# Acly/dlimgedit

Hardware: AMD Instinct MI355X
Metric: images/sec encode+mask @1024x1024 (higher is better)
Workload: dtype f16; 1 GPU; SAM vit_b encoder + 1 point prompt, 1 image(s)/GPU/step, 1024x1024 RGBA, inputs and masks resident in HBM; timed through the extension entry point dlimg_amd_encode_and_mask (device pointers in and out) -- the drop-in table itself, host buffers in and out, is `abi_path`; weights=seeded synthetic, lanes_per_gpu=4, lanes_fed_by_the_step_queue=3, requests_coalesced_per_pass=4, passes_queued_per_lane=2

## Files before the change

__graft_entry__.py:

```python
from __future__ import annotations

import sys
import tempfile
from pathlib import Path

ROOT = Path(__file__).resolve().parent
if str(ROOT) not in sys.path:
    sys.path.insert(0, str(ROOT))


def build() -> None:
    from dlimgedit_amd.build import build as build_lib
    lib = build_lib(verbose=True)
    import dlimgedit_amd
    from dlimgedit_amd import api
    handle = api.library()
    assert handle.dlimg_init() is not None
    for name in api.ext.EXPORTS:
        getattr(handle, name)
    hooks = api.hooks_library()
    assert hooks.dlimg_init() is not None
    for name in api.ext.HOOK_EXPORTS:
        getattr(hooks, name)
    from oracle import sam_oracle
    from oracle.build_ref import build_abi_consumer
    ref = build_abi_consumer()
    print(f"ok: {lib}; oracle/_ref: {ref if ref else 'reference tree absent, nothing prebuilt'}")


def smoke() -> None:
    import numpy as np
    from dlimgedit_amd import api, weights as W
    from dlimgedit_amd.sam_config import get_config
    from oracle import sam_oracle as O

    assert api.Environment.is_supported(api.Backend.gpu), "no gfx950 device: the HIP path cannot run"
    cfg = get_config("vit_test")
    with tempfile.TemporaryDirectory() as d:
        params = W.write_synthetic_model_dir(d, cfg, seed=7)
        env = api.Environment(api.Options(api.Backend.gpu, d))
        rng = np.random.default_rng(0)
        yy, xx = np.mgrid[0:1024, 0:1024].astype(np.float32)
        img = np.zeros((1024, 1024, 4), np.uint8)
        for c in range(3):
            img[:, :, c] = np.clip(128 + 60 * np.sin(xx * 0.01 * (c + 1)) * np.cos(yy * 0.013) +
                                   rng.uniform(-8, 8, (1024, 1024)), 0, 255).astype(np.uint8)
        img[:, :, 3] = 255
        seg = api.Segmentation.process(api.ImageView(img, api.Channels.rgba), env)
        mask = seg.compute_mask(api.Point(512, 512))
        ora = O.OracleSegmentation(params, cfg).process(img, O.CH_RGBA)
        want = ora.compute_mask(point=(512, 512))
        inter = np.logical_and(mask > 0, want > 0).sum()
        union = np.logical_or(mask > 0, want > 0).sum()
        iou = 1.0 if union == 0 else inter / union
        emb_err = float(np.abs(api.ext.get_embedding(seg) - ora.embedding).max())
        print(f"smoke: embedding max-abs err {emb_err:.4f}, mask IoU vs oracle {iou:.4f}")
        assert emb_err < 0.05 and iou >= 0.98
        seg.close()
        env.close()


if __name__ == "__main__":
    build()
    if "--smoke" in sys.argv:
        smoke()
```

dlimgedit_amd/api.py:

```python
from __future__ import annotations

import ctypes as C
import os
import enum
from dataclasses import dataclass, field
from pathlib import Path
from typing import Optional, Sequence, Tuple

import numpy as np

LIB_PATH = Path(__file__).resolve().parent / "lib" / "libdlimgedit.so"
HOOKS_LIB_PATH = LIB_PATH.with_name("libdlimgedit_test.so")
if os.environ.get("DLIMGEDIT_TUNING_LIB") == "1":
    LIB_PATH = HOOKS_LIB_PATH = LIB_PATH.with_name("libdlimgedit_tuning.so")
elif os.environ.get("DLIMGEDIT_TUNING_LIB"):
    LIB_PATH = HOOKS_LIB_PATH = LIB_PATH.with_name(os.environ["DLIMGEDIT_TUNING_LIB"])


class Error(RuntimeError):
    """dlimg::Exception."""


class Backend(enum.IntEnum):
    cpu = 0
    gpu = 1


class Channels(enum.IntEnum):
    mask = 1
    rgb = 3
    rgba = 4
    bgra = 5
    argb = 6


def count(channels: Channels) -> int:
    return 4 if int(channels) > 4 else int(channels)


@dataclass(frozen=True)
class Extent:
    width: int = 0
    height: int = 0


@dataclass(frozen=True)
class Point:
    x: int = 0
    y: int = 0


@dataclass(frozen=True)
class Region:
    top_left: Point = Point()
    bottom_right: Point = Point()

    @staticmethod
    def from_origin(origin: Point, extent: Extent) -> "Region":
        return Region(origin, Point(origin.x + extent.width, origin.y + extent.height))



class _ImageView(C.Structure):
    _fields_ = [("width", C.c_int), ("height", C.c_int), ("channels", C.c_int), ("stride", C.c_int),
                ("pixels", C.c_void_p)]


class _Options(C.Structure):
    _fields_ = [("backend", C.c_int), ("model_directory", C.c_char_p)]


_u8pp = C.POINTER(C.c_void_p)

_API_FIELDS = [
    ("is_backend_supported", C.CFUNCTYPE(C.c_int, C.c_int)),
    ("create_environment", C.CFUNCTYPE(C.c_int, C.POINTER(C.c_void_p), C.POINTER(_Options))),
    ("destroy_environment", C.CFUNCTYPE(None, C.c_void_p)),
    ("process_image_for_segmentation", C.CFUNCTYPE(C.c_int, C.POINTER(C.c_void_p), C.POINTER(_ImageView), C.c_void_p)),
    ("get_segmentation_mask", C.CFUNCTYPE(C.c_int, C.c_void_p, C.POINTER(C.c_int), C.POINTER(C.c_int), _u8pp,
                                          C.POINTER(C.c_float))),
    ("get_segmentation_extent", C.CFUNCTYPE(None, C.c_void_p, C.POINTER(C.c_int))),
    ("destroy_segmentation", C.CFUNCTYPE(None, C.c_void_p)),
    ("segment_objects", C.CFUNCTYPE(C.c_int, C.POINTER(_ImageView), C.c_void_p, C.c_void_p)),
    ("load_image", C.CFUNCTYPE(C.c_int, C.c_char_p, C.POINTER(C.c_int), C.POINTER(C.c_int), _u8pp)),
    ("save_image", C.CFUNCTYPE(C.c_int, C.POINTER(_ImageView), C.c_char_p)),
    ("create_image", C.CFUNCTYPE(C.c_void_p, C.c_int, C.c_int, C.c_int)),
    ("destroy_image", C.CFUNCTYPE(None, C.c_void_p)),
    ("last_error", C.CFUNCTYPE(C.c_char_p)),
    ("process_images_for_segmentation", C.CFUNCTYPE(C.c_int, C.POINTER(C.c_void_p), C.POINTER(_ImageView), C.c_int,
                                                    C.c_void_p)),
    ("get_segmentation_masks", C.CFUNCTYPE(C.c_int, C.POINTER(C.c_void_p), C.c_int, C.POINTER(C.c_int),
                                           C.POINTER(C.c_int), _u8pp)),
]

REFERENCE_SLOTS = 13


class _Api(C.Structure):
    _fields_ = _API_FIELDS


_lib = None
_api = None


def library() -> C.CDLL:
    global _lib
    if _lib is None:
        if not LIB_PATH.exists():
            raise Error(f"{LIB_PATH} not found: build it with `python -m dlimgedit_amd.build` "
                        "(the HIP library is the product; there is no Python fallback)")
        _lib = C.CDLL(str(LIB_PATH))
        _lib.dlimg_init.restype = C.POINTER(_Api)
        _lib.dlimg_init.argtypes = []
    return _lib


_hooks_lib = None


def hooks_library() -> C.CDLL:
    global _hooks_lib
    if _hooks_lib is None:
        if HOOKS_LIB_PATH == LIB_PATH:
            _hooks_lib = library()
        else:
            if not HOOKS_LIB_PATH.exists():
                raise Error(f"{HOOKS_LIB_PATH} not found: build it with `python -m dlimgedit_amd.build`")
            _hooks_lib = C.CDLL(str(HOOKS_LIB_PATH))
            _hooks_lib.dlimg_init.restype = C.POINTER(_Api)
            _hooks_lib.dlimg_init.argtypes = []
    return _hooks_lib


def _check_hook(result: int) -> None:
    if result != 0:
        msg = hooks_library().dlimg_init().contents.last_error()
        raise Error(msg.decode("utf-8", "replace") if msg else "Unknown error")


def api() -> _Api:
    global _api
    if _api is None:
        _api = library().dlimg_init().contents
    return _api


def _check(result: int) -> None:
    if result != 0:
        msg = api().last_error()
        raise Error(msg.decode("utf-8", "replace") if msg else "Unknown error")



class ImageView:

    def __init__(self, pixels: np.ndarray, channels: Channels = Channels.rgba, stride: Optional[int] = None):
        if pixels.dtype != np.uint8:
            raise TypeError("pixels must be uint8")
        if pixels.ndim == 2:
            pixels = pixels[:, :, None]
        h, w, c = pixels.shape
        if c != count(channels):
            raise ValueError(f"array has {c} channels, {channels!r} needs {count(channels)}")
        if stride is None:
            pixels = np.ascontiguousarray(pixels)
            stride = w * c
        self._array = pixels
        self.extent = Extent(w, h)
        self.channels = Channels(channels)
        self.stride = int(stride)

    def _c(self) -> _ImageView:
        return _ImageView(self.extent.width, self.extent.height, int(self.channels), self.stride,
                          self._array.ctypes.data)


class Image:

    def __init__(self, extent: Extent, channels: Channels = Channels.rgba):
        self._extent, self._channels = extent, Channels(channels)
        self._ptr = api().create_image(extent.width, extent.height, count(channels))
        if not self._ptr:
            raise Error("create_image failed")

    def extent(self) -> Extent:
        return self._extent

    def channels(self) -> Channels:
        return self._channels

    def size(self) -> int:
        return self._extent.width * self._extent.height * count(self._channels)

    def pixels(self) -> np.ndarray:
        buf = (C.c_uint8 * self.size()).from_address(self._ptr)
        buf._owner = self
        return np.frombuffer(buf, dtype=np.uint8).reshape(self._extent.height, self._extent.width, count(self._channels))

    def view(self) -> ImageView:
        return ImageView(self.pixels(), self._channels)

    @staticmethod
    def load(filepath) -> "Image":
        ext = (C.c_int * 2)()
        ch = C.c_int()
        px = C.c_void_p()
        _check(api().load_image(str(filepath).encode(), ext, C.byref(ch), C.byref(px)))
        img = Image.__new__(Image)
        img._extent, img._channels, img._ptr = Extent(ext[0], ext[1]), Channels(ch.value), px.value
        return img

    @staticmethod
    def save(img: ImageView, filepath) -> None:
        v = img._c()
        _check(api().save_image(C.byref(v), str(filepath).encode()))

    def __del__(self):
        ptr, self._ptr = getattr(self, "_ptr", None), None
        if ptr and _api is not None:
            _api.destroy_image(ptr)


def _mask_image(extent: Extent) -> np.ndarray:
    return Image(extent, Channels.mask).pixels().reshape(extent.height, extent.width)



@dataclass
class Options:
    backend: Backend = Backend.cpu
    model_directory: str = "models"


class Environment:

    @staticmethod
    def is_supported(backend: Backend) -> bool:
        return api().is_backend_supported(int(backend)) != 0

    def __init__(self, options: Options = Options()):
        self._handle = C.c_void_p()
        self._dir = str(options.model_directory).encode()
        opts = _Options(int(options.backend), self._dir)
        _check(api().create_environment(C.byref(self._handle), C.byref(opts)))

    def handle(self) -> C.c_void_p:
        return self._handle

    def close(self) -> None:
        h, self._handle = self._handle, C.c_void_p()
        if h and _api is not None:
            _api.destroy_environment(h)

    def __del__(self):
        self.close()

    def __enter__(self):
        return self

    def __exit__(self, *exc):
        self.close()


@dataclass
class Mask:
    image: np.ndarray
    accuracy: float = 0.0


MAX_CLICKS = 8
TOKEN_ROWS_MAX = 112
EMPTY_REGION = (0, 0, -1, -1)
REFINE_MARK = 4


@dataclass
class ClickEntries:
    heads: list
    points: list
    regions: list
    prompt_heads: list
    token_rows: list
    stage_clicks: list = field(default_factory=list)

    def _staged(self, j) -> bool:
        return j < len(self.stage_clicks) and len(self.stage_clicks[j]) > 1

    @property
    def launches(self) -> list:
        out = []
        plain = [j for j in range(len(self.token_rows)) if not self._staged(j)]
        for t in dict.fromkeys(self.token_rows[j] for j in plain):
            group = [j for j in plain if self.token_rows[j] == t]
            cut = TOKEN_ROWS_MAX // t
            out += [(t, group[k:k + cut]) for k in range(0, len(group), cut)]
        for j in range(len(self.token_rows)):
            if self._staged(j):
                box_rows = self.token_rows[j] - self.stage_clicks[j][-1]
                out += [(box_rows + k, [j]) for k in self.stage_clicks[j]]
        return out


def pack_clicks(clicks, labels, region=None):
    clicks, labels = _checked_clicks(clicks, labels)
    pts = [(c.x, c.y) for c in clicks]
    labs = list(labels)
    if region is not None:
        pts += [(region.top_left.x, region.top_left.y), (region.bottom_right.x, region.bottom_right.y)]
        labs += [2, 3]
    else:
        pts.append((0, 0))
        labs.append(-1)
    return pts, labs


def _checked_clicks(clicks, labels):
    clicks = list(clicks)
    labels = [1] * len(clicks) if labels is None else [int(v) for v in labels]
    if not clicks:
        raise Error("a prompt needs at least one click")
    if len(clicks) > MAX_CLICKS:
        raise Error(f"a prompt takes at most {MAX_CLICKS} clicks, not {len(clicks)}")
    if len(labels) != len(clicks):
        raise Error(f"{len(clicks)} clicks but {len(labels)} labels")
    if any(v not in (0, 1) for v in labels):
        raise Error("the label of a click is 1 (foreground) or 0 (background)")
    if labels[0] != 1:
        raise Error("the first click of a prompt is a foreground click: it travels in the head entry, which has no label")
    return clicks, labels


def _checked_marks(n_clicks: int, refine_after) -> list:
    if refine_after is None:
        return []
    if isinstance(refine_after, str):
        if refine_after != "each":
            raise Error('refine_after is a sequence of click counts or "each"')
        return list(range(1, n_clicks))
    ks = [int(k) for k in refine_after]
    if any(k < 1 or k >= n_clicks for k in ks):
        raise Error(f"refine_after: a mark goes behind the first k clicks, 1 <= k < {n_clicks} (every stage adds at least one click)")
    if any(b <= a for a, b in zip(ks, ks[1:])):
        raise Error("refine_after: the click counts are strictly increasing (no mark directly after another)")
    return ks


def click_entries(clicks, labels=None, regions=None, refine_after=None) -> ClickEntries:
    n = len(clicks)
    labels = [None] * n if labels is None else list(labels)
    regions = [None] * n if regions is None else list(regions)
    refine_after = [refine_after] * n if refine_after is None or isinstance(refine_after, str) else list(refine_after)
    if len(labels) != n or len(regions) != n or len(refine_after) != n:
        raise Error("one list of labels, one region (or None) and one refine_after (or None) per prompt")
    out = ClickEntries([], [], [], [], [])
    for j in range(n):
        cs, ls = _checked_clicks(clicks[j], labels[j])
        marks = _checked_marks(len(cs), refine_after[j])
        r = regions[j]
        out.prompt_heads.append(len(out.heads))
        out.token_rows.append(5 + len(cs) + (2 if r is not None else 1))
        out.stage_clicks.append(marks + [len(cs)])
        for k, (c, lab) in enumerate(zip(cs, ls)):
            if k in marks:
                out.heads.append(None)
                out.points.append((0, 0))
                out.regions.append((REFINE_MARK, 0, 0, 0))
            out.heads.append(j if k == 0 else None)
            out.points.append((c.x, c.y))
            if k:
                out.regions.append((lab, 0, 0, 0))
            else:
                out.regions.append(EMPTY_REGION if r is None else (r.top_left.x, r.top_left.y, r.bottom_right.x, r.bottom_right.y))
    return out


def _entry_calls(entries: ClickEntries) -> list:
    n = len(entries.heads)
    if any(h is None for h in entries.heads):
        return [(list(range(n)), True)]
    plain = [i for i in range(n) if entries.regions[i] == EMPTY_REGION]
    boxed = [i for i in range(n) if entries.regions[i] != EMPTY_REGION]
    return [(sel, given) for sel, given in ((plain, False), (boxed, True)) if sel]


def _entry_arrays(segs, entries: ClickEntries, sel, regions_given: bool):
    n = len(sel)
    handles = (C.c_void_p * n)(*[None if entries.heads[i] is None else segs[entries.heads[i]]._handle for i in sel])
    p = (C.c_int * (2 * n))(*[v for i in sel for v in entries.points[i]])
    r = (C.c_int * (4 * n))(*[v for i in sel for v in entries.regions[i]]) if regions_given else None
    return n, handles, p, r


class Segmentation:

    def __init__(self, handle: C.c_void_p, env: Environment):
        self._handle, self._env = handle, env

    @staticmethod
    def process(img: ImageView, env: Environment) -> "Segmentation":
        seg = Segmentation(C.c_void_p(), env)
        v = img._c()
        _check(api().process_image_for_segmentation(C.byref(seg._handle), C.byref(v), env.handle()))
        return seg

    @staticmethod
    def process_batch(imgs: Sequence[ImageView], env: Environment) -> list:
        n = len(imgs)
        handles = (C.c_void_p * n)()
        views = (_ImageView * n)(*[i._c() for i in imgs])
        segs = []
        try:
            _check(api().process_images_for_segmentation(handles, views, n, env.handle()))
        finally:
            segs = [Segmentation(C.c_void_p(h), env) for h in handles if h]
        return segs

    def extent(self) -> Extent:
        out = (C.c_int * 2)()
        api().get_segmentation_extent(self._handle, out)
        return Extent(out[0], out[1])

    def _query(self, point, region, n_masks, out=None):
        e = self.extent()
        masks = [_mask_image(e) for _ in range(n_masks)] if out is None else list(out)
        assert len(masks) == n_masks and all(m.shape == (e.height, e.width) and m.dtype == np.uint8 and
                                              m.flags.c_contiguous for m in masks)
        ptrs = (C.c_void_p * 3)(*([m.ctypes.data for m in masks] + [None] * (3 - n_masks)))
        acc = (C.c_float * 3)(0.0, 0.0, 0.0)
        p = (C.c_int * 2)(point.x, point.y) if point is not None else None
        r = (C.c_int * 4)(region.top_left.x, region.top_left.y, region.bottom_right.x, region.bottom_right.y) \
            if region is not None else None
        _check(api().get_segmentation_mask(self._handle, p, r, ptrs, acc))
        return masks, list(acc)

# ... 170 lines not shown
               "dlimg_amd_bench_gemm_stamps")

    @staticmethod
    def _ptr(a: Optional[np.ndarray]):
        return None if a is None else a.ctypes.data

    @classmethod
    def device_count(cls) -> int:
        return cls._l().dlimg_amd_device_count()

    @classmethod
    def model_geometry(cls, env: Environment) -> Tuple[int, int, int, int]:
        out = (C.c_int * 4)()
        _check(cls._l().dlimg_amd_model_geometry(env.handle(), out))
        return tuple(out)

    @classmethod
    def get_embedding(cls, seg: Segmentation) -> np.ndarray:
        out = np.empty((4096, 256), dtype=np.float32)
        _check(cls._l().dlimg_amd_get_embedding(seg._handle, out.ctypes.data))
        return out

    @classmethod
    def get_logits(cls, seg: Segmentation, point: Optional[Point] = None, region: Optional[Region] = None):
        logits = np.empty((4, 256, 256), dtype=np.float32)
        iou = np.empty(4, dtype=np.float32)
        p = (C.c_int * 2)(point.x, point.y) if point is not None else None
        r = (C.c_int * 4)(region.top_left.x, region.top_left.y, region.bottom_right.x, region.bottom_right.y) \
            if region is not None else None
        _check(cls._l().dlimg_amd_get_logits(seg._handle, p, r, logits.ctypes.data, iou.ctypes.data))
        return logits, iou

    @classmethod
    def decoder_state(cls, seg: Segmentation, point: Point):
        buf = C.create_string_buffer(1024)
        _check(cls._l().dlimg_amd_decoder_state(seg._handle, (C.c_int * 2)(point.x, point.y), None, 0, buf, 1024))
        parts = [(n, int(c)) for n, c in (item.split(":") for item in buf.value.decode().strip(",").split(","))]
        out = np.empty(sum(c for _, c in parts), dtype=np.float32)
        _check(cls._l().dlimg_amd_decoder_state(seg._handle, (C.c_int * 2)(point.x, point.y), out.ctypes.data, out.size, None, 0))
        res, off = {}, 0
        for n, c in parts:
            res[n] = out[off:off + c]
            off += c
        return res

    @classmethod
    def mask_pieces(cls, mask_bytes, extra_bytes: int = 0):
        n = len(mask_bytes)
        sizes = (C.c_longlong * max(1, n))(*mask_bytes)
        ends = (C.c_longlong * 8)()
        cap = 8 * (n + 1)
        copies = (C.c_longlong * (5 * cap))()
        pieces = C.c_int(0)
        got = cls._h().dlimg_amd_test_mask_pieces(n, sizes, extra_bytes, ends, 8, copies, cap, C.byref(pieces))
        if got < 0:
            _check_hook(1)
        return [ends[i] for i in range(pieces.value)], [tuple(copies[5 * k + j] for j in range(5)) for k in range(got)]

    @classmethod
    def plan_steps(cls, passes_in_flight, images_in_flight, cursor: int, pending: int, width: int, depth: int, all_: bool):
        lanes = len(passes_in_flight)
        p = (C.c_int * lanes)(*passes_in_flight)
        i = (C.c_int * lanes)(*images_in_flight)
        cur = C.c_int(cursor)
        cap = pending + lanes + 1
        out_lane, out_images = (C.c_int * cap)(), (C.c_int * cap)()
        n = cls._h().dlimg_amd_test_plan_steps(lanes, p, i, C.byref(cur), pending, width, depth, int(all_), out_lane, out_images, cap)
        if n < 0:
            _check_hook(1)
        return [(out_lane[k], out_images[k]) for k in range(n)], list(p), list(i), cur.value

    @classmethod
    def parse_cpu_list(cls, text: str) -> list:
        out = (C.c_int * 4096)()
        n = cls._h().dlimg_amd_test_parse_cpu_list(text.encode(), out, 4096)
        if n < 0:
            _check_hook(1)
        return list(out[:n])

    @classmethod
    def device_alloc(cls, env, nbytes: int) -> int:
        out = C.c_void_p()
        _check(cls._l().dlimg_amd_device_alloc(env.handle(), nbytes, C.byref(out)))
        return out.value

    @classmethod
    def device_free(cls, env, ptr: int) -> None:
        _check(cls._l().dlimg_amd_device_free(env.handle(), ptr))

    @classmethod
    def copy_to_device(cls, env, dst: int, src: np.ndarray) -> None:
        src = np.ascontiguousarray(src)
        _check(cls._l().dlimg_amd_copy_to_device(env.handle(), dst, src.ctypes.data, src.nbytes))

    @classmethod
    def copy_to_host(cls, env, dst: np.ndarray, src: int) -> None:
        _check(cls._l().dlimg_amd_copy_to_host(env.handle(), dst.ctypes.data, src, dst.nbytes))

    @staticmethod
    def device_views(ptrs, width, height, channels=Channels.rgba, stride=None):
        n = len(ptrs)

        def per_view(value):
            return list(value) if isinstance(value, (list, tuple)) else [value] * n

        ws, hs, cs, ss = per_view(width), per_view(height), per_view(channels), per_view(stride)
        return (_ImageView * n)(*[_ImageView(ws[i], hs[i], int(cs[i]), ws[i] * count(cs[i]) if ss[i] is None else ss[i], ptrs[i])
                                  for i in range(n)])

    @classmethod
    def encode_and_mask(cls, env, views, points, mask_ptrs) -> None:
        n = len(views)
        p = (C.c_int * (2 * n))(*[v for q in points for v in (q.x, q.y)])
        m = (C.c_void_p * n)(*mask_ptrs)
        _check(cls._l().dlimg_amd_encode_and_mask(env.handle(), views, n, p, m))

    @classmethod
    def encode_only(cls, env, views) -> None:
        _check(cls._l().dlimg_amd_encode_only(env.handle(), views, len(views)))

    @classmethod
    def synchronize(cls, env) -> None:
        _check(cls._l().dlimg_amd_synchronize(env.handle()))

    @classmethod
    def lane_count(cls, env) -> int:
        return cls._l().dlimg_amd_lane_count(env.handle())

    @classmethod
    def queue_config(cls, env) -> dict:
        out = (C.c_int * 6)()
        _check(cls._l().dlimg_amd_queue_config(env.handle(), out))
        return {"coalesce": out[0], "step_depth": out[1], "lanes": out[2], "lanes_in_use": out[3],
                "one_image_passes": out[4], "one_image_passes_alone": out[5]}

    @classmethod
    def image_memory_is_pinned(cls, array: np.ndarray) -> bool:
        out = C.c_int(0)
        _check(cls._l().dlimg_amd_image_memory(array.ctypes.data, array.nbytes, C.byref(out)))
        return bool(out.value)

    @classmethod
    def replica_count(cls, env) -> int:
        return cls._l().dlimg_amd_replica_count(env.handle())

    @classmethod
    def segmentation_device(cls, seg) -> Tuple[int, int]:
        r, d = C.c_int(), C.c_int()
        _check(cls._l().dlimg_amd_segmentation_device(seg._handle, C.byref(r), C.byref(d)))
        return r.value, d.value

    @classmethod
    def compute_mask_batch_device(cls, segs, dev_out: int, points=None, regions=None, root_device: int = 0, clicks=None,
                                  labels=None, refine_after=None) -> list:
        if refine_after is not None and clicks is None:
            raise Error("compute_mask_batch_device: refine_after goes with `clicks`")
        if clicks is not None:
            if points is not None:
                raise Error("compute_mask_batch_device: `points` or `clicks`, not both")
            if len(clicks) != len(segs):
                raise Error("compute_mask_batch_device: one list of clicks per segmentation")
            entries = click_entries(clicks, labels, regions, refine_after)
            calls = _entry_calls(entries)
            if len(calls) > 1:
                calls = [([i], entries.regions[i] != EMPTY_REGION) for i in range(len(entries.heads))]
            result, base = [], 0
            for sel, given in calls:
                n, handles, p, r = _entry_arrays(segs, entries, sel, given)
                offsets = (C.c_size_t * n)()
                _check(cls._l().dlimg_amd_get_segmentation_masks_device(handles, n, p, r, root_device, dev_out + base, offsets))
                result += [base + offsets[k] for k, i in enumerate(sel) if entries.heads[i] is not None]
                e = segs[entries.heads[sel[0]]].extent()
                base += e.width * e.height if len(calls) > 1 else 0
            return result
        n = len(segs)
        handles = (C.c_void_p * n)(*[s._handle for s in segs])
        p = r = None
        if points is not None:
            p = (C.c_int * (2 * n))(*[v for q in points for v in (q.x, q.y)])
        if regions is not None:
            r = (C.c_int * (4 * n))(*[v for q in regions for v in (q.top_left.x, q.top_left.y, q.bottom_right.x,
                                                                  q.bottom_right.y)])
        offsets = (C.c_size_t * n)()
        _check(cls._l().dlimg_amd_get_segmentation_masks_device(handles, n, p, r, root_device, dev_out, offsets))
        return list(offsets)

    @classmethod
    def set_profiling(cls, env, on: bool) -> None:
        _check(cls._l().dlimg_amd_set_profiling(env.handle(), int(on)))

    @classmethod
    def take_stage_stats(cls, env) -> dict:
        n = len(STAGES)
        ms, work, launches = (C.c_double * n)(), (C.c_double * n)(), (C.c_long * n)()
        _check(cls._l().dlimg_amd_take_stage_stats(env.handle(), ms, work, launches))
        return {s: {"ms": ms[i], "work": work[i], "launches": launches[i]} for i, s in enumerate(STAGES)}

    @classmethod
    def test_preprocess(cls, pixels: np.ndarray, channels: Channels, stride: Optional[int] = None) -> np.ndarray:
        h, w = pixels.shape[:2]
        if stride is None:
            pixels = np.ascontiguousarray(pixels)
            stride = w * count(channels)
        out = np.empty((4096, 768), dtype=np.float16)
        _check_hook(cls._h().dlimg_amd_test_preprocess(pixels.ctypes.data, w, h, stride, int(channels), out.ctypes.data))
        return out

    @classmethod
    def test_postprocess(cls, planes: np.ndarray, out_w: int, out_h: int, iou: Optional[np.ndarray] = None) -> np.ndarray:
        planes = np.ascontiguousarray(planes, dtype=np.float32).reshape(-1, 256, 256)
        out = np.empty((out_h, out_w), dtype=np.uint8)
        iou = None if iou is None else np.ascontiguousarray(iou, dtype=np.float32)
        _check_hook(cls._h().dlimg_amd_test_postprocess(planes.ctypes.data, planes.shape[0], cls._ptr(iou), out_w, out_h,
                                                   out.ctypes.data))
        return out

    @classmethod
    def test_postprocess_batch(cls, planes: np.ndarray, out_w: int, out_h: int) -> np.ndarray:
        planes = np.ascontiguousarray(planes, dtype=np.float32).reshape(-1, 256, 256)
        out = np.empty((planes.shape[0], out_h, out_w), dtype=np.uint8)
        _check_hook(cls._h().dlimg_amd_test_postprocess_batch(planes.ctypes.data, planes.shape[0], out_w, out_h, out.ctypes.data))
        return out

    @classmethod
    def force_gemm_tile(cls, tile: int = -1, consumer_tile: int = -1) -> None:
        _check_hook(cls._h().dlimg_amd_test_force_gemm_tile(int(tile)))
        _check_hook(cls._h().dlimg_amd_test_force_gemm_consumer_tile(int(consumer_tile)))

    @classmethod
    def test_gemm(cls, A: np.ndarray, W: np.ndarray, bias=None, resid=None, act: int = 0, want_f16: bool = False):
        A = np.ascontiguousarray(A, dtype=np.float16)
        W = np.ascontiguousarray(W, dtype=np.float16)
        M, K = A.shape
        N = W.shape[0]
        bias = None if bias is None else np.ascontiguousarray(bias, dtype=np.float32)
        resid = None if resid is None else np.ascontiguousarray(resid, dtype=np.float32)
        out32 = np.empty((M, N), dtype=np.float32)
        out16 = np.empty((M, N), dtype=np.float16) if want_f16 else None
        _check_hook(cls._h().dlimg_amd_test_gemm(M, N, K, A.ctypes.data, W.ctypes.data, cls._ptr(bias), cls._ptr(resid),
                                            0 if resid is None else resid.shape[0], act, out32.ctypes.data,
                                            cls._ptr(out16)))
        return (out32, out16) if want_f16 else out32

    @classmethod
    def test_gemm_ln(cls, A1, W1, bias1, resid, W2, gamma, beta, bias2, eps: float, act: int = 0):
        A1 = np.ascontiguousarray(A1, dtype=np.float16)
        W1 = np.ascontiguousarray(W1, dtype=np.float16)
        M, K1 = A1.shape
        D = W1.shape[0]
        W2 = np.asarray(W2, dtype=np.float32)
        N = W2.shape[0]
        wg = np.ascontiguousarray((W2 * np.asarray(gamma, np.float32)[None, :]).astype(np.float16))
        colsum = np.ascontiguousarray(wg.astype(np.float64).sum(axis=1).astype(np.float32))
        b2 = np.ascontiguousarray((np.asarray(bias2, np.float64) + W2.astype(np.float64) @ np.asarray(beta, np.float64))
                                  .astype(np.float32))
        bias1 = None if bias1 is None else np.ascontiguousarray(bias1, dtype=np.float32)
        resid = None if resid is None else np.ascontiguousarray(resid, dtype=np.float32)
        x = np.empty((M, D), dtype=np.float32)
        xh = np.empty((M, D), dtype=np.float16)
        y = np.empty((M, N), dtype=np.float32)
        _check_hook(cls._h().dlimg_amd_test_gemm_ln(M, D, K1, N, A1.ctypes.data, W1.ctypes.data, cls._ptr(bias1),
                                               cls._ptr(resid), wg.ctypes.data, colsum.ctypes.data, b2.ctypes.data,
                                               eps, act, x.ctypes.data, xh.ctypes.data, y.ctypes.data))
        return x, xh, y

    @classmethod
    def test_lane_worker(cls, tasks: int, sleep_us: int = 0):
        order = np.full(tasks + 1, -1, dtype=np.int32)
        ran = cls._h().dlimg_amd_test_lane_worker(tasks, sleep_us, order.ctypes.data)
        if ran < 0:
            _check_hook(1)
        return order[:ran].tolist()

    @classmethod
    def test_gemm_stream(cls, A, W, bias, resid_hi, resid_lo, pair: bool):
        A = np.ascontiguousarray(A, dtype=np.float16)
        W = np.ascontiguousarray(W, dtype=np.float16)
        M, K = A.shape
        D = W.shape[0]
        bias = None if bias is None else np.ascontiguousarray(bias, dtype=np.float32)
        resid_hi = None if resid_hi is None else np.ascontiguousarray(resid_hi, dtype=np.float16)
        resid_lo = None if resid_lo is None else np.ascontiguousarray(resid_lo, dtype=np.float16)
        x = None if pair else np.empty((M, D), dtype=np.float32)
        hi = np.empty((M, D), dtype=np.float16)
        lo = np.empty((M, D), dtype=np.float16) if pair else None
        stats = np.empty((M * 48,), dtype=np.float32)
        _check_hook(cls._h().dlimg_amd_test_gemm_stream(M, D, K, A.ctypes.data, W.ctypes.data, cls._ptr(bias), cls._ptr(resid_hi),
                                                   cls._ptr(resid_lo), int(pair), cls._ptr(x), hi.ctypes.data,
                                                   cls._ptr(lo), stats.ctypes.data))
        return x, hi, lo, stats

    @classmethod
    def test_layernorm(cls, x, w, b, eps: float, act: int = 0):
        x = np.ascontiguousarray(x, dtype=np.float32)
        w = np.ascontiguousarray(w, dtype=np.float32)
        b = np.ascontiguousarray(b, dtype=np.float32)
        rows, dim = x.shape
        o32 = np.empty_like(x)
        o16 = np.empty(x.shape, dtype=np.float16)
        _check_hook(cls._h().dlimg_amd_test_layernorm(x.ctypes.data, w.ctypes.data, b.ctypes.data, eps, rows, dim, act,
                                                 o32.ctypes.data, o16.ctypes.data))
        return o32, o16

    @classmethod
    def test_attention(cls, is_global: bool, qkv, qkv_bias, rel_h, rel_w, batch: int, heads: int, hd: int):
        qkv = np.ascontiguousarray(qkv, dtype=np.float16)
        rel_h = np.ascontiguousarray(rel_h, dtype=np.float32)
        rel_w = np.ascontiguousarray(rel_w, dtype=np.float32)
        qkv_bias = None if qkv_bias is None else np.ascontiguousarray(qkv_bias, dtype=np.float32)
        out = np.empty((batch * 4096, heads * hd), dtype=np.float16)
        _check_hook(cls._h().dlimg_amd_test_attention(int(is_global), qkv.ctypes.data, cls._ptr(qkv_bias), rel_h.ctypes.data,
                                                 rel_w.ctypes.data, batch, heads, hd, out.ctypes.data))
        return out

    @classmethod
    def test_decode(cls, env: Environment, embeddings: np.ndarray, emb_index, coords, labels):
        emb = np.ascontiguousarray(embeddings, dtype=np.float32).reshape(-1, 4096, 256)
        idx = np.ascontiguousarray(emb_index, dtype=np.int32).reshape(-1)
        count = idx.size
        c = np.ascontiguousarray(coords, dtype=np.float32).reshape(count, 4)
        l = np.ascontiguousarray(labels, dtype=np.float32).reshape(count, 2)
        logits = np.empty((count, 4, 256, 256), dtype=np.float32)
        iou = np.empty((count, 4), dtype=np.float32)
        _check_hook(cls._h().dlimg_amd_test_decode(env.handle(), emb.shape[0], emb.ctypes.data, count, idx.ctypes.data,
                                                   c.ctypes.data, l.ctypes.data, logits.ctypes.data, iou.ctypes.data))
        return logits, iou

    @classmethod
    def test_decode_prompts(cls, env: Environment, embeddings: np.ndarray, emb_index, coords, labels, mask_planes=None,
                            mask_iou=None, want_state: bool = False):
        emb = np.ascontiguousarray(embeddings, dtype=np.float32).reshape(-1, 4096, 256)
        idx = np.ascontiguousarray(emb_index, dtype=np.int32).reshape(-1)
        count = idx.size
        l = np.ascontiguousarray(labels, dtype=np.float32).reshape(count, -1)
        points = l.shape[1]
        c = np.ascontiguousarray(coords, dtype=np.float32).reshape(count, points, 2)
        planes = None if mask_planes is None else np.ascontiguousarray(mask_planes, dtype=np.float32).reshape(count, 4, 256, 256)
        iou4 = None if mask_iou is None else np.ascontiguousarray(mask_iou, dtype=np.float32).reshape(count, 4)
        logits = np.empty((count, 4, 256, 256), dtype=np.float32)
        iou = np.empty((count, 4), dtype=np.float32)
        state = np.empty(1 << 18, dtype=np.float32) if want_state else None
        layout = C.create_string_buffer(1024)
        _check_hook(cls._h().dlimg_amd_test_decode_prompts(
            env.handle(), emb.shape[0], emb.ctypes.data, count, idx.ctypes.data, points, c.ctypes.data, l.ctypes.data,
            cls._ptr(planes), cls._ptr(iou4), logits.ctypes.data, iou.ctypes.data, cls._ptr(state),
            0 if state is None else state.size, layout, 1024))
        if not want_state:
            return logits, iou
        res, off = {}, 0
        for n, cnt in ((n, int(cnt)) for n, cnt in (item.split(":") for item in layout.value.decode().strip(",").split(","))):
            res[n] = state[off:off + cnt].copy()
            off += cnt
        return logits, iou, res

    @classmethod
    def test_resize(cls, pixels: np.ndarray, channels: Channels, out_w: int, out_h: int) -> np.ndarray:
        pixels = np.ascontiguousarray(pixels)
        h, w = pixels.shape[:2]
        c = count(channels)
        out = np.empty((out_h, out_w, c), dtype=np.uint8)
        _check_hook(cls._h().dlimg_amd_test_resize(pixels.ctypes.data, w, h, w * c, int(channels), out_w, out_h,
                                              out.ctypes.data))
        return out

    @classmethod
    def birefnet_prepare_image(cls, image: np.ndarray, channels: "Channels", mean, std) -> np.ndarray:
        image = np.ascontiguousarray(image, dtype=np.uint8)
        h, w = image.shape[:2]
        mean = np.ascontiguousarray(mean, dtype=np.float32)
        std = np.ascontiguousarray(std, dtype=np.float32)
        out = np.empty((1, 3, h, w), dtype=np.float32)
        _check(cls._l().dlimg_amd_birefnet_prepare_image(image.ctypes.data, w, h, image.strides[0], int(channels),
                                                         mean.ctypes.data, std.ctypes.data, out.ctypes.data))
        return out

    @classmethod
    def birefnet_process_mask(cls, logits: np.ndarray) -> np.ndarray:
        logits = np.ascontiguousarray(logits, dtype=np.float32)
        h, w = logits.shape
        out = np.empty((h, w), dtype=np.uint8)
        _check(cls._l().dlimg_amd_birefnet_process_mask(logits.ctypes.data, w, h, out.ctypes.data))
        return out

    @classmethod
    def resize_mask(cls, mask: np.ndarray, out_w: int, out_h: int) -> np.ndarray:
        mask = np.ascontiguousarray(mask, dtype=np.uint8)
        h, w = mask.shape
        out = np.empty((out_h, out_w), dtype=np.uint8)
        _check(cls._l().dlimg_amd_resize_mask(mask.ctypes.data, w, h, mask.strides[0], out_w, out_h, out.ctypes.data))
        return out

    @classmethod
    def bench_prepost(cls, batch: int = 16, iters: int = 50, working_set_mb: int = 768) -> Tuple[float, float]:
        pre, post = C.c_double(), C.c_double()
        _check_hook(cls._h().dlimg_amd_bench_prepost(batch, iters, working_set_mb, C.byref(pre), C.byref(post)))
        return pre.value, post.value

    @classmethod
    def bench_attention(cls, is_global: bool, heads: int = 12, hd: int = 64, batch: int = 1, iters: int = 50) -> float:
        ms = C.c_double()
        _check_hook(cls._h().dlimg_amd_bench_attention(int(is_global), batch, heads, hd, iters, C.byref(ms)))
        return ms.value

    @classmethod
    def bench_gemm(cls, M: int, N: int, K: int, act: int = 0, iters: int = 20, flavour: int = 0, tile: int = -1,
                   shared: bool = False, streams: int = 1) -> float:
        ms = C.c_double()
        _check_hook(cls._h().dlimg_amd_bench_gemm_streams(M, N, K, act, flavour, tile, int(shared), streams, iters,
                                                     C.byref(ms)))
        return ms.value

    @classmethod
    def bench_gemm_stamps(cls, M: int, N: int, K: int, act: int = 0, iters: int = 20, flavour: int = 0, tile: int = 9,
                          streams: int = 1, groups: int = 4096):
        ms = C.c_double()
        st = np.zeros((groups, 4), np.uint64)
        _check_hook(cls._h().dlimg_amd_bench_gemm_stamps(M, N, K, act, flavour, tile, 0, streams, iters, C.byref(ms),
                                                    st.ctypes.data, groups))
        return ms.value, st
```

dlimgedit_amd/build.py:

```python
from __future__ import annotations

import os
import shutil
import subprocess
import sys
from concurrent.futures import ThreadPoolExecutor
from pathlib import Path

PKG = Path(__file__).resolve().parent
ROOT = PKG.parent
CSRC = PKG / "csrc"
OBJ = CSRC / "_obj"
OBJ_TUNING = CSRC / "_obj_tuning"
LIB = PKG / "lib" / "libdlimgedit.so"
LIB_TEST = PKG / "lib" / "libdlimgedit_test.so"
LIB_TUNING = PKG / "lib" / "libdlimgedit_tuning.so"
ARCH = "gfx950"
SONAME = "libdlimgedit.so.1"
EXPORTS_MAP = CSRC / "exports.map"
EXPORTS_TEST_MAP = CSRC / "exports_test.map"
HOOK_SOURCES = ["test_hooks.cpp"]

SOURCES = [
    "kernels/gemm.hip",
    "kernels/elementwise.hip",
    "kernels/attention_window.hip",
    "kernels/attention_global.hip",
    "kernels/decoder.hip",
    "kernels/decoder_image.hip",
    "kernels/decoder_hq.hip",
    "kernels/postprocess.hip",
    "kernels/resize.hip",
    "kernels/objects.hip",
    "resize_tables.cpp",
    "gemm_plan.cpp",
    "image_io.cpp",
    "image_memory.cpp",
    "jpeg_decode.cpp",
    "weights.cpp",
    "lane_board.cpp",
    "stage_clock.cpp",
    "mask_transport.cpp",
    "sam_weights.cpp",
    "sam_model.cpp",
    "environment.cpp",
    "segmentation.cpp",
    "dlimgedit.cpp",
    "ext_api.cpp",
]


EXTRA_FLAGS = {
    "kernels/postprocess.hip": ["-ffp-contract=off"],
    "kernels/resize.hip": ["-ffp-contract=off"],
    "kernels/objects.hip": ["-ffp-contract=off"],
    "resize_tables.cpp": ["-ffp-contract=off"],
}


def hipcc() -> str:
    exe = shutil.which("hipcc") or "/opt/rocm/bin/hipcc"
    if not Path(exe).exists():
        raise RuntimeError("hipcc not found; the MI355X build of dlimgedit needs the ROCm toolchain")
    return exe


def _flags() -> list:
    return [f"--offload-arch={ARCH}", "-O3", "-std=c++17", "-fPIC", "-fvisibility=hidden", "-DDLIMGEDIT_EXPORTS",
            "-fno-slp-vectorize", "-Wall", "-Wno-unused-function", "-Wno-unused-result", f"-I{ROOT / 'include'}", f"-I{CSRC}"]


def _deps_mtime() -> float:
    hdrs = list(CSRC.rglob("*.hpp")) + list(CSRC.rglob("*.inc")) + list((ROOT / "include").rglob("*.h"))
    return max(p.stat().st_mtime for p in hdrs)


def _compile(src: str, force: bool, hdr_mtime: float, tuning: bool = False) -> Path:
    s = CSRC / src
    if not s.exists():
        raise FileNotFoundError(s)
    o = (OBJ_TUNING if tuning else OBJ) / (src.replace("/", "_") + ".o")
    if not force and o.exists() and o.stat().st_mtime > max(s.stat().st_mtime, hdr_mtime):
        return o
    cmd = [hipcc(), *_flags(), *(["-DDLIMG_TUNING", *os.environ.get("DLIMG_TUNING_DEFS", "").split()] if tuning else []), *EXTRA_FLAGS.get(src, []), "-x", "hip", "-c",
           str(s), "-o", str(o)]
    r = subprocess.run(cmd, capture_output=True, text=True)
    if r.returncode != 0:
        raise RuntimeError(f"hipcc failed for {src}:\n{r.stdout}\n{r.stderr}")
    if r.stderr.strip():
        sys.stderr.write(r.stderr)
    return o


LLVM_OBJDUMP = "/opt/rocm/lib/llvm/bin/llvm-objdump"
VALIDATED_HIPCC = "HIP 7.2.26015 / AMD clang 22.0.0git roc-7.2.0 (7b800a19)"


def disassemble_device_code(obj: Path) -> str:
    import tempfile
    with tempfile.TemporaryDirectory() as d:
        tmp = Path(d) / obj.name
        shutil.copy(obj, tmp)
        subprocess.run([LLVM_OBJDUMP, "--offloading", str(tmp)], capture_output=True, text=True, check=True)
        code = [f for f in Path(d).iterdir() if f.name.startswith(obj.name + ".") and "amdgcn" in f.name]
        if not code:
            raise RuntimeError(f"no gfx950 code object found in {obj}")
        return subprocess.run([LLVM_OBJDUMP, "-d", str(code[0])], capture_output=True, text=True, check=True).stdout


def check_packed_select_erratum(obj: Path) -> dict:
    import re
    counts, bad, name = {}, [], None
    for line in disassemble_device_code(obj).splitlines():
        m = re.match(r"^[0-9a-f]+ <(.+)>:$", line)
        if m:
            name = m.group(1)
            continue
        m = re.search(r"\b(v_pk_\w+)\s", line)
        if not (name and m):
            continue
        if m.group(1).endswith("_f32"):
            counts[name] = counts.get(name, 0) + 1
        sel = re.search(r"op_sel:\[([01]),([01])", line)
        if sel and sel.group(2) == "1":
            bad.append((name, line.strip().split("//")[0].strip()))
    if bad:
        listing = "\n".join(f"  {n}: {i}" for n, i in bad[:8])
        raise RuntimeError(f"{obj.name}: packed instruction with a src1 low-lane select (op_sel:[_,1,..]) -- reads 0.0 beside another "
                           f"wave's MFMA on gfx950 (DESIGN.md section 6; validated toolchain: {VALIDATED_HIPCC}):\n{listing}")
    return counts


def _link(out: Path, objs: list, exports: Path, soname: str = "") -> None:
    cmd = [hipcc(), f"--offload-arch={ARCH}", "-shared", "-fPIC", "-o", str(out), *map(str, objs),
           "-Wl,-rpath,/opt/rocm/lib", "-Wl,--no-undefined", *([f"-Wl,-soname,{soname}"] if soname else []),
           f"-Wl,--version-script={exports}", "-ldl", "-lz"]
    r = subprocess.run(cmd, capture_output=True, text=True)
    if r.returncode != 0:
        raise RuntimeError(f"link failed:\n{r.stdout}\n{r.stderr}")


def _stale(lib: Path, objs: list, force: bool) -> bool:
    return force or not lib.exists() or lib.stat().st_mtime < max(o.stat().st_mtime for o in objs)


def build(force: bool = False, verbose: bool = False, tuning: bool = False) -> Path:
    (OBJ_TUNING if tuning else OBJ).mkdir(parents=True, exist_ok=True)
    LIB.parent.mkdir(parents=True, exist_ok=True)
    hdr = _deps_mtime()
    workers = min(6, os.cpu_count() or 1)
    with ThreadPoolExecutor(workers) as ex:
        objs = list(ex.map(lambda s: _compile(s, force, hdr, tuning), SOURCES))
        hooks = list(ex.map(lambda s: _compile(s, force, hdr, tuning), HOOK_SOURCES))
    if tuning:
        if _stale(LIB_TUNING, objs + hooks, force):
            _link(LIB_TUNING, objs + hooks, EXPORTS_TEST_MAP)
        if verbose:
            print(f"built {LIB_TUNING} ({LIB_TUNING.stat().st_size / 1e6:.1f} MB)")
        return LIB_TUNING
    if _stale(LIB, objs, force) or _stale(LIB_TEST, objs + hooks, force):
        for o in objs:
            if o.name.startswith("kernels_"):
                check_packed_select_erratum(o)
        if _stale(LIB, objs, force):
            _link(LIB, objs, EXPORTS_MAP, SONAME)
        _link(LIB_TEST, objs + hooks, EXPORTS_TEST_MAP)
    link = LIB.parent / SONAME
    if not link.is_symlink() and not link.exists():
        link.symlink_to(LIB.name)
    if verbose:
        print(f"built {LIB} ({LIB.stat().st_size / 1e6:.1f} MB) and {LIB_TEST.name}")
    return LIB


if __name__ == "__main__":
    build(force="--force" in sys.argv, verbose=True, tuning="--tuning" in sys.argv)
```

dlimgedit_amd/csrc/kernels/gemm.hip:

```cpp
#include "device_common.hpp"
#include "kernels.hpp"
#include "gemm_plan.hpp"

#include <hip/hip_ext.h>

#include <mutex>
#include <cstdlib>
#include <type_traits>

namespace dlimg {
namespace {

#ifdef DLIMG_TUNING
#define DLIMG_STAMPS(a) ((a).stamps)
#else
#define DLIMG_STAMPS(a) (static_cast<unsigned long long*>(nullptr))
#endif

#if defined(DLIMG_TUNING) && defined(DLIMG_NO_RESID_READ)
constexpr bool kNoResidRead = true;
#else
constexpr bool kNoResidRead = false;
#endif
#if defined(DLIMG_TUNING) && defined(DLIMG_NO_COPY_WRITE)
constexpr bool kNoCopyWrite = true;
#else
constexpr bool kNoCopyWrite = false;
#endif

#if defined(DLIMG_TUNING) && defined(DLIMG_NO_STATS_MATH)
constexpr bool kNoStatsMath = true;
#else
constexpr bool kNoStatsMath = false;
#endif
#if defined(DLIMG_TUNING) && defined(DLIMG_NO_STREAM_STORE)
constexpr bool kNoStreamStore = true;
#else
constexpr bool kNoStreamStore = false;
#endif

#include "gemm_f16_tile.inc"

typedef float float4v __attribute__((ext_vector_type(4)));

template <int BM, int BN, int WGM, int WGN, int NSTAGE, int MINW, int ACT, int EPI>
__global__ __launch_bounds__(64 * WGM * WGN, MINW) void gemm16_f16_kernel(k::GemmArgs a) {
    constexpr int BKT = 32;
    constexpr int NW = WGM * WGN;
    constexpr int ROW_BYTES = BKT * 2;
    constexpr int WM = BM / WGM, WN = BN / WGN;
    constexpr int TM = WM / 16, TN = WN / 16;
    constexpr int A_BYTES = BM * ROW_BYTES, B_BYTES = BN * ROW_BYTES;
    constexpr int STAGE_BYTES = A_BYTES + B_BYTES;
    constexpr int LOADS = (BM + BN) * ROW_BYTES / 1024 / NW;
    constexpr int JG = ((WN / 32) % 3 == 0) ? 3 : (((WN / 32) % 2 == 0) ? 2 : 1);
    constexpr int CHUNKS = JG * 8;
    constexpr int OUT_BYTES = 32 * CHUNKS * 16;
    static_assert(NW * OUT_BYTES <= NSTAGE * STAGE_BYTES, "output staging must fit in the operand buffers");
    static_assert(TM % 2 == 0 && TN % 2 == 0, "wave tile must be a multiple of 32x32");
    extern __shared__ __attribute__((aligned(16))) char smem[];

    const int lane = lane_id();
    const int wave = wave_id();
    const int wr = wave / WGN, wc = wave % WGN;
    const int l15 = lane & 15, quad = lane >> 4;

    const int ntn = a.N / BN;
    const int tile = xcd_remap(blockIdx.x, gridDim.x);
    const int m0 = (tile / ntn) * BM;
    const int n0 = (tile % ntn) * BN;

    float4v acc[TM][TN];
#pragma unroll
    for (int i = 0; i < TM; ++i)
#pragma unroll
        for (int j = 0; j < TN; ++j) acc[i][j] = float4v{0.f, 0.f, 0.f, 0.f};

    float* rowstat = reinterpret_cast<float*>(smem + NSTAGE * STAGE_BYTES);
    float* colvec = rowstat + 2 * BM;
    const int nk = a.K / BKT;
    auto stage = [&](int kt) {
        char* dst = smem + (kt % NSTAGE) * STAGE_BYTES;
        stage_tile<BM, BKT, NW, 1>(a.A, a.lda, m0, kt * BKT, dst, wave, lane);
        stage_tile<BN, BKT, NW, 1>(a.W, a.ldw, n0, kt * BKT, dst + A_BYTES, wave, lane);
    };
    auto frag = [&](const char* lds, int row) {
        return *reinterpret_cast<const half8_t*>(lds + row * ROW_BYTES + ((quad ^ swz16(row)) << 4));
    };
    ColumnVectors<BM, BN, 64 * NW, EPI> column_vectors;
    RowStats<BM, 64 * NW, EPI> row_stats;
    column_vectors.issue(a, n0);
    row_stats.issue(a, m0);
#pragma unroll
    for (int t = 0; t < NSTAGE - 1; ++t)
        if (t < nk) stage(t);
    column_vectors.store(colvec);
    row_stats.finish(a, rowstat);

    static_assert(NSTAGE >= 3, "a tile is read one step before it is multiplied");
    constexpr int TH = TM / 2;
    half8_t fb[2][TN], fal[2][TH], fah[TH];
    auto wait_tile = [&](int newer) {
        static_assert((NSTAGE - 2) * LOADS < 64 && NSTAGE <= 8, "vmcnt is a 6-bit counter");
        if (newer >= 6) wait_dma<6 * LOADS>();
        else if (newer == 5) wait_dma<5 * LOADS>();
        else if (newer == 4) wait_dma<4 * LOADS>();
        else if (newer == 3) wait_dma<3 * LOADS>();
        else if (newer == 2) wait_dma<2 * LOADS>();
        else if (newer == 1) wait_dma<LOADS>();
        else wait_dma<0>();
    };
    auto read_next = [&](int buf, int kt) {
        const char* la = smem + (kt % NSTAGE) * STAGE_BYTES;
        const char* lb = la + A_BYTES;
#pragma unroll
        for (int j = 0; j < TN; ++j) fb[buf][j] = frag(lb, wc * WN + j * 16 + l15);
#pragma unroll
        for (int i = 0; i < TH; ++i) fal[buf][i] = frag(la, wr * WM + i * 16 + l15);
    };
    auto step = [&](int kt, auto cur_tag, auto steady_tag) {
        constexpr int cur = decltype(cur_tag)::value;
        constexpr bool STEADY = decltype(steady_tag)::value;
        const char* la = smem + (kt % NSTAGE) * STAGE_BYTES;
#pragma unroll
        for (int i = 0; i < TH; ++i) fah[i] = frag(la, wr * WM + (TH + i) * 16 + l15);
        if (STEADY) {
            wait_dma<(NSTAGE - 3) * LOADS>();
            __builtin_amdgcn_s_barrier();
            read_next(cur ^ 1, kt + 1);
            stage(kt + NSTAGE - 1);
        } else if (kt + 1 < nk) {
            wait_tile(min(NSTAGE - 3, nk - 2 - kt));
            __builtin_amdgcn_s_barrier();
            read_next(cur ^ 1, kt + 1);
            if (kt + NSTAGE - 1 < nk) stage(kt + NSTAGE - 1);
        }
        __builtin_amdgcn_sched_barrier(0);
#pragma unroll
        for (int i = 0; i < TH; ++i)
#pragma unroll
            for (int j = 0; j < TN; ++j)
                acc[i][j] = __builtin_amdgcn_mfma_f32_16x16x32_f16(fb[cur][j], fal[cur][i], acc[i][j], 0, 0, 0);
#pragma unroll
        for (int i = 0; i < TH; ++i)
#pragma unroll
            for (int j = 0; j < TN; ++j)
                acc[TH + i][j] = __builtin_amdgcn_mfma_f32_16x16x32_f16(fb[cur][j], fah[i], acc[TH + i][j], 0, 0, 0);
    };
    wait_tile(min(NSTAGE - 2, nk - 1));
    __builtin_amdgcn_s_barrier();
    read_next(0, 0);
    __builtin_amdgcn_s_waitcnt(0xC07F);
    using Even = std::integral_constant<int, 0>;
    using Odd = std::integral_constant<int, 1>;
    int kt = 0;
    for (; kt + 2 + (NSTAGE - 1) <= nk; kt += 2) {
        step(kt, Even{}, std::true_type{});
        step(kt + 1, Odd{}, std::true_type{});
    }
    for (; kt < nk; kt += 2) {
        step(kt, Even{}, std::false_type{});
        if (kt + 1 < nk) step(kt + 1, Odd{}, std::false_type{});
    }

    __syncthreads();
    char* slab = smem + wave * OUT_BYTES;
    float2_t* rowpart = reinterpret_cast<float2_t*>(smem + NW * OUT_BYTES);
    static_assert(NW * OUT_BYTES + BM * (BN / 32) * 8 <= NSTAGE * STAGE_BYTES, "tile statistics must fit behind the slabs");
    const int resid_row0 = a.resid ? m0 % a.resid_mod : 0;
    constexpr int NIT = 32 * CHUNKS / 64;
    constexpr int NJ = (WN / 32) / JG, NSLAB = (TM / 2) * NJ;
    constexpr int RV_BUFS = (MINW >= 4 && NIT > 4) ? 1 : 2;
    float4_t rv[RV_BUFS][NIT];
    if (RV_BUFS == 2) {
        const int pf_row_base = wr * WM, pf_col_base = wc * WN;
        float4_t(&pf_dst)[NIT] = rv[0];
#include "gemm_epilogue_prefetch.inc"
    }
#pragma unroll
    for (int band = 0; band < TM / 2; ++band) {
#pragma unroll
        for (int jg = 0; jg < NJ; ++jg) {
            const int sl = band * NJ + jg;
#pragma unroll
            for (int ii = 0; ii < 2; ++ii) {
                const int row = ii * 16 + l15;
#pragma unroll
                for (int jj = 0; jj < JG * 2; ++jj) {
                    const int chunk = jj * 4 + quad;
                    *reinterpret_cast<float4v*>(slab + (row * CHUNKS + (chunk ^ (row & 7))) * 16) =
                        acc[band * 2 + ii][jg * JG * 2 + jj];
                }
            }
            if (sl + RV_BUFS - 1 < NSLAB) {
                constexpr int AHEAD = RV_BUFS - 1;
                const int pf_row_base = wr * WM + ((sl + AHEAD) / NJ) * 32;
                const int pf_col_base = wc * WN + ((sl + AHEAD) % NJ) * JG * 32;
                float4_t(&pf_dst)[NIT] = rv[(sl + AHEAD) % RV_BUFS];
#include "gemm_epilogue_prefetch.inc"
            }
            const int row_local_base = wr * WM + band * 32, col_local_base = wc * WN + jg * JG * 32;
            float4_t(&rv_cur)[NIT] = rv[sl % RV_BUFS];
#include "gemm_epilogue.inc"
        }
    }
    if (EPI == EPI_STATS) {
        __syncthreads();
        write_tile_stats<BM, BN>(a, rowpart, m0, n0);
    }
}


constexpr int kPPHalfBytes = 128 * 128;
constexpr int kPPBufBytes = 4 * kPPHalfBytes;
constexpr int pp_aux_bytes(int bm) { return bm * 8 + 2 * 256 * 4 + (bm * 4 * 8 > kPPStatGroups * bm * 8 ? bm * 4 * 8 : kPPStatGroups * bm * 8); }
constexpr int kPPAuxBytes = pp_aux_bytes(256);
constexpr int kPPLds = 2 * kPPBufBytes + kPPAuxBytes;
static_assert(kPPLds <= 160 * 1024, "gemm_pp_kernel: LDS");

DLIMG_DEVICE void pp_barrier_after_reads() {
    __builtin_amdgcn_sched_barrier(0);
    asm volatile("s_waitcnt lgkmcnt(0)\n\ts_barrier" ::: "memory");
    __builtin_amdgcn_sched_barrier(0);
}
DLIMG_DEVICE void pp_barrier() {
    __builtin_amdgcn_sched_barrier(0);
    asm volatile("s_barrier" ::: "memory");
    __builtin_amdgcn_sched_barrier(0);
}

struct HiLo4 { half4_t h, l; };
DLIMG_DEVICE float4_t hilo_pack(half4_t h, half4_t l) { return __builtin_bit_cast(float4_t, HiLo4{h, l}); }
template <bool HIGH> DLIMG_DEVICE float mix_sum(uint32_t hi, uint32_t lo) {
    float r;
    if (HIGH) asm("v_fma_mix_f32 %0, %1, 1.0, %2 op_sel:[1,0,1] op_sel_hi:[1,0,1]" : "=v"(r) : "v"(hi), "v"(lo));
    else asm("v_fma_mix_f32 %0, %1, 1.0, %2 op_sel:[0,0,0] op_sel_hi:[1,0,1]" : "=v"(r) : "v"(hi), "v"(lo));
    return r;
}
template <bool HIGH> DLIMG_DEVICE float mix_rest(float v, uint32_t hi) {
    float r;
    if (HIGH) asm("v_fma_mix_f32 %0, %1, -1.0, %2 op_sel:[1,0,0] op_sel_hi:[1,0,0]" : "=v"(r) : "v"(hi), "v"(v));
    else asm("v_fma_mix_f32 %0, %1, -1.0, %2 op_sel:[0,0,0] op_sel_hi:[1,0,0]" : "=v"(r) : "v"(hi), "v"(v));
    return r;
}
DLIMG_DEVICE float4_t hilo_value(float4_t packed) {
    const uint4_t x = __builtin_bit_cast(uint4_t, packed);
    return float4_t{mix_sum<false>(x[0], x[2]), mix_sum<true>(x[0], x[2]), mix_sum<false>(x[1], x[3]), mix_sum<true>(x[1], x[3])};
}
DLIMG_DEVICE HiLo4 hilo_split(float4_t v) {
    HiLo4 out;
    out.h = __builtin_convertvector(v, half4_t);
    const uint2_t hb = __builtin_bit_cast(uint2_t, out.h);
    const float4_t rest = {mix_rest<false>(v[0], hb[0]), mix_rest<true>(v[1], hb[0]), mix_rest<false>(v[2], hb[1]), mix_rest<true>(v[3], hb[1])};
    out.l = __builtin_convertvector(rest, half4_t);
    return out;
}
DLIMG_DEVICE float4_t hilo_load(const half_t* hi, const half_t* lo, size_t offset) {
    return hilo_pack(*reinterpret_cast<const half4_t*>(hi + offset), *reinterpret_cast<const half4_t*>(lo + offset));
}

template <int BM, int EPI>
struct PPAux {
    static constexpr int BN = 256;
    static constexpr int TPR = 512 / BM;
    static constexpr int GP = BM * 8 > 1024 ? BM * 8 / 1024 : 1;
    static DLIMG_DEVICE void issue(const k::GemmArgs& a, int m0, int n0, float* colvec, float2_t* raw, int wave, int lane) {
        if (wave == 0) {
            if (a.bias) glds16(a.bias + n0 + lane * 4, colvec);
            else *reinterpret_cast<float4_t*>(colvec + lane * 4) = float4_t{0.f, 0.f, 0.f, 0.f};
        }
        if (EPI != EPI_NORM) return;
        if (wave == 1) glds16(a.ln_colsum + n0 + lane * 4, colvec + BN);
        const int pieces = a.ln_groups * GP;
        for (int p = wave; p < pieces + 2; p += 8) {
            if (p < 2) continue;
            const int g = (p - 2) / GP, h = (p - 2) % GP;
            const float2_t* src = reinterpret_cast<const float2_t*>(a.ln_stats) + (size_t)g * a.M + m0 + h * 128 + lane * 2;
            if (BM * 8 >= 1024 || lane < BM / 2) glds16(src, raw + g * BM + h * 128);
        }
    }
    static DLIMG_DEVICE void merge(const k::GemmArgs& a, const float2_t* raw, float* rowstat) {
        if (EPI != EPI_NORM) return;
        const int r = threadIdx.x / TPR, sub = threadIdx.x % TPR;
        float s1 = 0.f;
        for (int g = sub; g < a.ln_groups; g += TPR) s1 += raw[g * BM + r][0];
#pragma unroll
        for (int o = 1; o < TPR; o <<= 1) s1 += __shfl_xor(s1, o, 64);
        const float n_g = (float)(a.K / a.ln_groups), inv_n_g = 1.0f / n_g;
        const float mean = s1 / (float)a.K;
        float m2 = 0.f;
        for (int g = sub; g < a.ln_groups; g += TPR) {
            const float2_t q = raw[g * BM + r];
            const float dm = q[0] * inv_n_g - mean;
            m2 += q[1] + n_g * dm * dm;
        }
#pragma unroll
        for (int o = 1; o < TPR; o <<= 1) m2 += __shfl_xor(m2, o, 64);
        if (sub == 0) reinterpret_cast<float2_t*>(rowstat)[r] = float2_t{mean, rsqrtf(m2 / (float)a.K + a.ln_eps)};
        __syncthreads();
    }
};

template <int NI, int ACT, int EPI, bool PRE = false>
DLIMG_DEVICE void pp_epilogue(const k::GemmArgs& a, float4v (&acc)[NI][4], char* smem, const float* rowstat, const float* colvec,
                              float2_t* rowpart, int m0, int n0, int row_base, int wc, int wave, int lane,
                              float4_t (*pre)[4] = nullptr) {
    constexpr int BN = 256;
    const int l15 = lane & 15, quad = lane >> 4;
    const int col_base = wc * 64 + quad * 4;
    float4_t bias4[4], csum4[4];
#pragma unroll
    for (int j = 0; j < 4; ++j) {
        bias4[j] = *reinterpret_cast<const float4_t*>(colvec + col_base + j * 16);
        if (EPI == EPI_NORM) csum4[j] = *reinterpret_cast<const float4_t*>(colvec + BN + col_base + j * 16);
    }
    char* slab = smem + wave * 8192;
    const int resid_row0 = (a.resid || a.resid_h) ? m0 % a.resid_mod : 0;
    if (a.out_f32 == nullptr && a.out_l == nullptr) {
        const int rd_row = lane >> 3, rd_chunk = lane & 7;
#pragma unroll
        for (int i = 0; i < NI; ++i) {
            char* sl = slab + (i & 1) * 4096;
            float2_t st = float2_t{0.f, 1.f};
            if (EPI == EPI_NORM) st = reinterpret_cast<const float2_t*>(rowstat)[row_base + i * 16 + l15];
#pragma unroll
            for (int j = 0; j < 4; ++j) {
                float4_t v = float4_t{acc[i][j][0], acc[i][j][1], acc[i][j][2], acc[i][j][3]};
                if (EPI == EPI_NORM) v = (v - csum4[j] * st[0]) * st[1];
                v += bias4[j];
                if (ACT == k::ACT_GELU) v = gelu4(v);
                const half4_t h = {(half_t)v[0], (half_t)v[1], (half_t)v[2], (half_t)v[3]};
                const int piece = (j * 4 + quad) ^ ((l15 & 7) << 1);
                *reinterpret_cast<half4_t*>(sl + l15 * 128 + piece * 8) = h;
            }
            asm volatile("s_waitcnt lgkmcnt(0)" ::: "memory");
#pragma unroll
            for (int kk = 0; kk < 2; ++kk) {
                const int r = kk * 8 + rd_row;
                const float4_t piece16 = *reinterpret_cast<const float4_t*>(sl + r * 128 + ((rd_chunk ^ (r & 7)) << 4));
                const size_t m = (size_t)(m0 + row_base + i * 16 + r);
                half_t* const dst = a.out_h + m * a.ldc16 + n0 + wc * 64 + rd_chunk * 8;
                store16_result(dst, piece16);
            }
        }
    } else {
        auto fp32_bands = [&](auto resid_tag, auto h_tag) {
            constexpr int RESID = decltype(resid_tag)::value;
            constexpr int OUT = decltype(h_tag)::value;
            constexpr bool HAS_H = OUT == 1;
            const int rd_row = lane >> 3, rd_col = (lane & 7) * 8;
            float4_t rv[2][4];
            auto request_residual = [&](int i, float4_t (&dst)[4]) {
    #pragma unroll
                for (int kk = 0; kk < 2; ++kk) {
                    dst[kk * 2] = dst[kk * 2 + 1] = float4_t{0.f, 0.f, 0.f, 0.f};
                    const int r = kk * 8 + rd_row;
                    if (RESID == 1 && !kNoResidRead) {
                        const float* src = a.resid + (size_t)(resid_row0 + row_base + i * 16 + r) * a.ldr + n0 + wc * 64 + rd_col;
                        dst[kk * 2] = *reinterpret_cast<const float4_t*>(src);
                        dst[kk * 2 + 1] = *reinterpret_cast<const float4_t*>(src + 4);
                    }
                    if (RESID == 2 && !kNoResidRead) {
                        const size_t off = (size_t)(resid_row0 + row_base + i * 16 + r) * a.ldrs + n0 + wc * 64 + rd_col;
                        dst[kk * 2] = *reinterpret_cast<const float4_t*>(a.resid_h + off);
                        dst[kk * 2 + 1] = *reinterpret_cast<const float4_t*>(a.resid_l + off);
                    }
                }
            };
            if (!PRE) request_residual(0, rv[0]);
    #pragma unroll
            for (int i = 0; i < NI; ++i) {
                char* sl = slab + (i & 1) * 4096;
                float2_t st = float2_t{0.f, 1.f};
                if (EPI == EPI_NORM) st = reinterpret_cast<const float2_t*>(rowstat)[row_base + i * 16 + l15];
    #pragma unroll
                for (int j = 0; j < 4; ++j) {
                    float4_t v = float4_t{acc[i][j][0], acc[i][j][1], acc[i][j][2], acc[i][j][3]};
                    if (EPI == EPI_NORM) v = (v - csum4[j] * st[0]) * st[1];
                    v += bias4[j];
                    if (ACT == k::ACT_GELU) v = gelu4(v);
                    *reinterpret_cast<float4_t*>(sl + l15 * 256 + (((j * 4 + quad) ^ (l15 & 7)) << 4)) = v;
                }
                if (!PRE && i + 1 < NI) request_residual(i + 1, rv[(i + 1) & 1]);
                asm volatile("s_waitcnt lgkmcnt(0)" ::: "memory");
    #pragma unroll
                for (int kk = 0; kk < 2; ++kk) {
                    const int r = kk * 8 + rd_row;
                    const int slot = (lane & 7) * 2;
                    float4_t v0 = *reinterpret_cast<const float4_t*>(sl + r * 256 + ((slot ^ (r & 7)) << 4));
                    float4_t v1 = *reinterpret_cast<const float4_t*>(sl + r * 256 + (((slot + 1) ^ (r & 7)) << 4));
                    const float4_t ra = PRE ? pre[i][kk * 2] : rv[i & 1][kk * 2], rb = PRE ? pre[i][kk * 2 + 1] : rv[i & 1][kk * 2 + 1];
                    if (RESID == 1) {
                        v0 += ra;
                        v1 += rb;
                    } else if (RESID == 2) {
                        const uint4_t xa = __builtin_bit_cast(uint4_t, ra), xb = __builtin_bit_cast(uint4_t, rb);
                        v0 += hilo_value(__builtin_bit_cast(float4_t, uint4_t{xa[0], xa[1], xb[0], xb[1]}));
                        v1 += hilo_value(__builtin_bit_cast(float4_t, uint4_t{xa[2], xa[3], xb[2], xb[3]}));
                    }
                    const size_t m = (size_t)(m0 + row_base + i * 16 + r);
                    const int col = n0 + wc * 64 + rd_col;
                    if (kNoStreamStore) {
                        if (v0[0] + v1[3] == 123.456f) a.out_h[0] = (half_t)1.f;
                    } else if (OUT == 2) {
                        const HiLo4 p0 = hilo_split(v0), p1 = hilo_split(v1);
                        const uint2_t h0 = __builtin_bit_cast(uint2_t, p0.h), h1 = __builtin_bit_cast(uint2_t, p1.h);
                        const uint2_t l0 = __builtin_bit_cast(uint2_t, p0.l), l1 = __builtin_bit_cast(uint2_t, p1.l);
                        store16_result(a.out_h + m * a.ldc16 + col, uint4_t{h0[0], h0[1], h1[0], h1[1]});
                        store16_result(a.out_l + m * a.ldc16 + col, uint4_t{l0[0], l0[1], l1[0], l1[1]});
                    } else {
                        store16_result(a.out_f32 + m * a.ldc32 + col, v0);
                        store16_result(a.out_f32 + m * a.ldc32 + col + 4, v1);
                    }
                    if (HAS_H && !kNoCopyWrite) {
                        const half8_t h = {(half_t)v0[0], (half_t)v0[1], (half_t)v0[2], (half_t)v0[3],
                                           (half_t)v1[0], (half_t)v1[1], (half_t)v1[2], (half_t)v1[3]};
                        store16_result(a.out_h + m * a.ldc16 + col, h);
                    }
                    if (EPI == EPI_STATS) {
                        float s1 = ((v0[0] + v0[1]) + (v0[2] + v0[3])) + ((v1[0] + v1[1]) + (v1[2] + v1[3]));
                        if (kNoStatsMath) { if ((lane & 7) == 0) rowpart[(row_base + i * 16 + r) * 4 + wc] = float2_t{s1, s1}; continue; }
                        s1 = sum_over_8_lanes(s1);
                        const float4_t d0 = v0 - s1 * (1.0f / 64.0f), d1 = v1 - s1 * (1.0f / 64.0f);
                        float m2 = ((d0[0] * d0[0] + d0[1] * d0[1]) + (d0[2] * d0[2] + d0[3] * d0[3])) +
                                   ((d1[0] * d1[0] + d1[1] * d1[1]) + (d1[2] * d1[2] + d1[3] * d1[3]));
                        m2 = sum_over_8_lanes(m2);
                        if ((lane & 7) == 0) rowpart[(row_base + i * 16 + r) * 4 + wc] = float2_t{s1, m2};
                    }
                }
            }

        };
        using I0 = std::integral_constant<int, 0>;
        using I1 = std::integral_constant<int, 1>;
        using I2 = std::integral_constant<int, 2>;
        if (a.out_l) {
            if (a.resid_h) fp32_bands(I2{}, I2{});
            else if (a.resid) fp32_bands(I1{}, I2{});
            else fp32_bands(I0{}, I2{});
        } else if (a.resid) {
            if (a.out_h) fp32_bands(I1{}, I1{});
            else fp32_bands(I1{}, I0{});
        } else {
            if (a.out_h) fp32_bands(I0{}, I1{});
            else fp32_bands(I0{}, I0{});
        }
    }
    if (EPI == EPI_STATS) {
        __syncthreads();
        for (int r = threadIdx.x; r < NI * 32; r += 512) {
            float s1 = 0.f;
#pragma unroll
            for (int g = 0; g < 4; ++g) s1 += rowpart[r * 4 + g][0];
            const float mean = s1 * (1.0f / (float)BN);
            float m2 = 0.f;
#pragma unroll
            for (int g = 0; g < 4; ++g) {
                const float dm = rowpart[r * 4 + g][0] * (1.0f / 64.0f) - mean;
                m2 += rowpart[r * 4 + g][1] + 64.0f * dm * dm;
            }
            reinterpret_cast<float2_t*>(a.stats_out)[(size_t)(n0 / BN) * a.M + m0 + r] = float2_t{s1, m2};
        }
    }
}

template <int ACT, int EPI>
__global__ __launch_bounds__(512, 2) void gemm_pp_kernel(k::GemmArgs a) {
    constexpr int BM = 256, BN = 256;
    extern __shared__ __attribute__((aligned(16))) char smem[];
    const int lane = lane_id();
    const int wave = wave_id();
    const int wr = wave >> 2, wc = wave & 3;
    const int l15 = lane & 15, quad = lane >> 4;

    const int ntn = a.N / BN;
    const int tile = xcd_remap(blockIdx.x, gridDim.x);
    const int m0 = (tile / ntn) * BM;
    const int n0 = (tile % ntn) * BN;
    const int nk = a.K / 64;

    float* rowstat = reinterpret_cast<float*>(smem + 2 * kPPBufBytes);
    float* colvec = rowstat + 2 * BM;
    float2_t* rowpart = reinterpret_cast<float2_t*>(colvec + 2 * BN);

    float4v acc[8][4];
#pragma unroll
    for (int i = 0; i < 8; ++i)
#pragma unroll
        for (int j = 0; j < 4; ++j) acc[i][j] = float4v{0.f, 0.f, 0.f, 0.f};

    const half_t* src_a[2];
    const half_t* src_w[2];
#pragma unroll
    for (int q = 0; q < 2; ++q) {
        const int row = (wave * 2 + q) * 8 + (lane >> 3);
        const int chunk = (lane & 7) ^ ((row >> 1) & 7);
        src_a[q] = a.A + (size_t)(m0 + row) * a.lda + chunk * 8;
        src_w[q] = a.W + (size_t)(n0 + row) * a.ldw + chunk * 8;
    }
    const size_t a_half = (size_t)128 * a.lda, w_half = (size_t)128 * a.ldw;
    auto stage = [&](int t, int H) {
        char* dst = smem + (t & 1) * kPPBufBytes + H * kPPHalfBytes + wave * 2048;
#pragma unroll
        for (int q = 0; q < 2; ++q) {
            const half_t* g = (H < 2 ? src_a[q] + (H & 1) * a_half : src_w[q] + (H & 1) * w_half) + (size_t)t * 64;
            glds16(g, dst + q * 1024);
        }
    };

    const int sw = (l15 >> 1) & 7;
    const int off0 = l15 * 128 + ((quad ^ sw) << 4);
    const int off1 = l15 * 128 + (((quad ^ sw) ^ 4) << 4);
    const char* a_base = smem + wr * kPPHalfBytes;
    const char* w_base = smem + (2 + (wc >> 1)) * kPPHalfBytes + (wc & 1) * 64 * 128;
    auto frag = [&](const char* p) { return *reinterpret_cast<const half8_t*>(p); };

    const unsigned long long t_start = DLIMG_STAMPS(a) ? __builtin_amdgcn_s_memtime() : 0ull;
    const unsigned long long r_start = DLIMG_STAMPS(a) ? __builtin_amdgcn_s_memrealtime() : 0ull;
    PPAux<BM, EPI>::issue(a, m0, n0, colvec, rowpart, wave, lane);
    stage(0, 0); stage(0, 1); stage(0, 2); stage(0, 3);
    if (nk > 1) { stage(1, 2); stage(1, 3); }
    if (nk > 1) wait_dma<4>(); else wait_dma<0>();
    pp_barrier();
    if (wr == 1) pp_barrier();

    half8_t fa[4][2], fw[2][2][2];
    auto mfma_quadrant = [&](int mh, int nh) {
        __builtin_amdgcn_s_setprio(1);
#pragma unroll
        for (int ks = 0; ks < 2; ++ks)
#pragma unroll
            for (int i = 0; i < 4; ++i)
#pragma unroll
                for (int j = 0; j < 2; ++j)
                    acc[mh * 4 + i][nh * 2 + j] =
                        __builtin_amdgcn_mfma_f32_16x16x32_f16(fw[nh][j][ks], fa[i][ks], acc[mh * 4 + i][nh * 2 + j], 0, 0, 0);
        __builtin_amdgcn_s_setprio(0);
    };
    auto read_a = [&](int buf, int mh) {
        const char* p = a_base + buf * kPPBufBytes + mh * 64 * 128;
#pragma unroll
        for (int i = 0; i < 4; ++i) {
            fa[i][0] = frag(p + i * 2048 + off0);
            fa[i][1] = frag(p + i * 2048 + off1);
        }
    };
    auto read_w = [&](int buf, int nh) {
        const char* p = w_base + buf * kPPBufBytes + nh * 32 * 128;
#pragma unroll
        for (int j = 0; j < 2; ++j) {
            fw[nh][j][0] = frag(p + j * 2048 + off0);
            fw[nh][j][1] = frag(p + j * 2048 + off1);
        }
    };
    auto step = [&](int t, auto buf_tag, auto steady_tag) {
        constexpr int buf = decltype(buf_tag)::value;
        constexpr bool STEADY = decltype(steady_tag)::value;
        read_w(buf, 0);
        read_w(buf, 1);
        read_a(buf, 0);
        if (STEADY || t + 1 < nk) { stage(t + 1, 0); stage(t + 1, 1); }
        pp_barrier_after_reads();
        mfma_quadrant(0, 0);
        mfma_quadrant(0, 1);
        pp_barrier();
        read_a(buf, 1);
        if (STEADY || t + 2 < nk) {
            stage(t + 2, 2);
            stage(t + 2, 3);
            wait_dma<4>();
        } else {
            wait_dma<0>();
        }
        pp_barrier_after_reads();
        mfma_quadrant(1, 1);
        mfma_quadrant(1, 0);
        pp_barrier();
    };
    using Even = std::integral_constant<int, 0>;
    using Odd = std::integral_constant<int, 1>;
    const unsigned long long t_loop = DLIMG_STAMPS(a) ? __builtin_amdgcn_s_memtime() : 0ull;
    const unsigned long long r_loop = DLIMG_STAMPS(a) ? __builtin_amdgcn_s_memrealtime() : 0ull;
    int t = 0;
    for (; t + 3 < nk; t += 2) {
        step(t, Even{}, std::true_type{});
        step(t + 1, Odd{}, std::true_type{});
    }
    for (; t < nk; t += 2) {
        step(t, Even{}, std::false_type{});
        if (t + 1 < nk) step(t + 1, Odd{}, std::false_type{});
    }
    if (wr == 0) pp_barrier();
    const unsigned long long t_loop_end = DLIMG_STAMPS(a) ? __builtin_amdgcn_s_memtime() : 0ull;
    const unsigned long long r_loop_end = DLIMG_STAMPS(a) ? __builtin_amdgcn_s_memrealtime() : 0ull;

    PPAux<BM, EPI>::merge(a, rowpart, rowstat);
    pp_epilogue<8, ACT, EPI>(a, acc, smem, rowstat, colvec, rowpart, m0, n0, wr * 128, wc, wave, lane);
    if (DLIMG_STAMPS(a) && threadIdx.x == 0) {
        asm volatile("s_waitcnt vmcnt(0)" ::: "memory");
        unsigned long long* d = DLIMG_STAMPS(a) + (size_t)blockIdx.x * 4;
        d[0] = t_loop_end - t_loop;
        d[1] = r_loop_end - r_loop;
        d[2] = ((t_loop - t_start) << 32) | ((__builtin_amdgcn_s_memtime() - t_loop_end) & 0xffffffffull);
        d[3] = __builtin_amdgcn_s_memrealtime() - r_start;
    }
}


constexpr int pp128_a_bytes(int bm) { return bm * 128; }
constexpr int pp128_w_base(int bm) { return 3 * pp128_a_bytes(bm); }
constexpr int pp128_operands(int bm) { return 3 * pp128_a_bytes(bm) + 3 * 2 * kPPHalfBytes; }
constexpr int pp128_lds(int bm) { return pp128_operands(bm) + pp_aux_bytes(bm); }
static_assert(pp128_lds(128) <= 160 * 1024 && pp128_lds(64) <= 160 * 1024, "gemm_pp128_kernel: LDS");

template <int BM, int ACT, int EPI>
__global__ __launch_bounds__(512, 2) void gemm_pp128_kernel(k::GemmArgs a) {
    static_assert(BM == 128 || BM == 64, "128 or 64 rows per tile");
    constexpr int BN = 256;
    constexpr int NI = BM / 32;
    constexpr int APIECES = BM / 64;
    constexpr int LOADS = 4 + APIECES;
    extern __shared__ __attribute__((aligned(16))) char smem[];
    const int lane = lane_id();
    const int wave = wave_id();
    const int wr = wave >> 2, wc = wave & 3;
    const int l15 = lane & 15, quad = lane >> 4;

    const int ntn = a.N / BN;
    const int tile = xcd_remap(blockIdx.x, gridDim.x);
    const int m0 = (tile / ntn) * BM;
    const int n0 = (tile % ntn) * BN;
    const int nk = a.K / 64;

    float* rowstat = reinterpret_cast<float*>(smem + pp128_operands(BM));
    float* colvec = rowstat + 2 * BM;
    float2_t* rowpart = reinterpret_cast<float2_t*>(colvec + 2 * BN);

    float4v acc[NI][4];
#pragma unroll
    for (int i = 0; i < NI; ++i)
#pragma unroll
        for (int j = 0; j < 4; ++j) acc[i][j] = float4v{0.f, 0.f, 0.f, 0.f};

    const half_t* src_a[APIECES];
    const half_t* src_w[2];
#pragma unroll
    for (int q = 0; q < 2; ++q) {
        const int row = (wave * 2 + q) * 8 + (lane >> 3);
        const int chunk = (lane & 7) ^ ((row >> 1) & 7);
        src_w[q] = a.W + (size_t)(n0 + row) * a.ldw + chunk * 8;
    }
#pragma unroll
    for (int q = 0; q < APIECES; ++q) {
        const int row = (wave * APIECES + q) * 8 + (lane >> 3);
        const int chunk = (lane & 7) ^ ((row >> 1) & 7);
        src_a[q] = a.A + (size_t)(m0 + row) * a.lda + chunk * 8;
    }
    const size_t w_half = (size_t)128 * a.ldw;
    auto stage_a = [&](int t, int abuf) {
        char* dst = smem + abuf * pp128_a_bytes(BM) + wave * (APIECES * 1024);
#pragma unroll
        for (int q = 0; q < APIECES; ++q) glds16(src_a[q] + (size_t)t * 64, dst + q * 1024);
    };
    auto stage_w = [&](int t, int wbuf, int h) {
        char* dst = smem + pp128_w_base(BM) + (wbuf * 2 + h) * kPPHalfBytes + wave * 2048;
#pragma unroll
        for (int q = 0; q < 2; ++q) glds16(src_w[q] + h * w_half + (size_t)t * 64, dst + q * 1024);
    };

    const int sw = (l15 >> 1) & 7;
    const int off0 = l15 * 128 + ((quad ^ sw) << 4);
    const int off1 = l15 * 128 + (((quad ^ sw) ^ 4) << 4);
    const char* a_base = smem + wr * (BM / 2) * 128;
    const char* w_base = smem + pp128_w_base(BM) + (wc >> 1) * kPPHalfBytes + (wc & 1) * 64 * 128;
    auto frag = [&](const char* p) { return *reinterpret_cast<const half8_t*>(p); };

    PPAux<BM, EPI>::issue(a, m0, n0, colvec, rowpart, wave, lane);
    stage_a(0, 0); stage_w(0, 0, 0); stage_w(0, 0, 1);
    if (nk > 1) { stage_a(1, 1); stage_w(1, 1, 0); stage_w(1, 1, 1); }
    if (nk > 1) wait_dma<LOADS>(); else wait_dma<0>();
    constexpr bool PRE = EPI == EPI_STATS;
    float4_t rpre[NI][4];
    if (PRE) {
#pragma unroll
        for (int i = 0; i < NI; ++i)
#pragma unroll
            for (int kk = 0; kk < 4; ++kk) rpre[i][kk] = float4_t{0.f, 0.f, 0.f, 0.f};
        if (a.resid && !kNoResidRead) {
            const int resid_row0 = m0 % a.resid_mod;
#pragma unroll
            for (int i = 0; i < NI; ++i)
#pragma unroll
                for (int kk = 0; kk < 2; ++kk) {
                    const float* src = a.resid + (size_t)(resid_row0 + wr * (BM / 2) + i * 16 + kk * 8 + (lane >> 3)) * a.ldr + n0 + wc * 64 + (lane & 7) * 8;
                    rpre[i][kk * 2] = *reinterpret_cast<const float4_t*>(src);
                    rpre[i][kk * 2 + 1] = *reinterpret_cast<const float4_t*>(src + 4);
                }
        } else if (a.resid_h) {
            const int resid_row0 = m0 % a.resid_mod;
#pragma unroll
            for (int i = 0; i < NI; ++i)
#pragma unroll
                for (int kk = 0; kk < 2; ++kk) {
                    const size_t off = (size_t)(resid_row0 + wr * (BM / 2) + i * 16 + kk * 8 + (lane >> 3)) * a.ldrs + n0 + wc * 64 + (lane & 7) * 8;
                    rpre[i][kk * 2] = *reinterpret_cast<const float4_t*>(a.resid_h + off);
                    rpre[i][kk * 2 + 1] = *reinterpret_cast<const float4_t*>(a.resid_l + off);
                }
        }
    }
    pp_barrier();
    if (wr == 1) pp_barrier();

    half8_t fa[NI][2], fw[4][2];
    auto mfma_tile = [&] {
        __builtin_amdgcn_s_setprio(1);
#pragma unroll
        for (int ks = 0; ks < 2; ++ks)
#pragma unroll
            for (int i = 0; i < NI; ++i)
#pragma unroll
                for (int j = 0; j < 4; ++j)
                    acc[i][j] = __builtin_amdgcn_mfma_f32_16x16x32_f16(fw[j][ks], fa[i][ks], acc[i][j], 0, 0, 0);
        __builtin_amdgcn_s_setprio(0);
    };
    int buf3 = 0;
    auto step = [&](int t, auto steady_tag) {
        constexpr bool STEADY = decltype(steady_tag)::value;
        const char* ab = a_base + buf3 * pp128_a_bytes(BM);
        const char* wb = w_base + buf3 * 2 * kPPHalfBytes;
        const int next2 = buf3 == 0 ? 2 : buf3 - 1;
#pragma unroll
        for (int j = 0; j < 4; ++j) {
            fw[j][0] = frag(wb + j * 2048 + off0);
            fw[j][1] = frag(wb + j * 2048 + off1);
        }
#pragma unroll
        for (int i = 0; i < NI; ++i) {
            fa[i][0] = frag(ab + i * 2048 + off0);
            fa[i][1] = frag(ab + i * 2048 + off1);
        }
        if (STEADY || t + 2 < nk) {
            stage_w(t + 2, next2, 0);
            stage_w(t + 2, next2, 1);
            stage_a(t + 2, next2);
            __builtin_amdgcn_sched_barrier(0);
            asm volatile("s_waitcnt lgkmcnt(0) vmcnt(%0)\n\ts_barrier" ::"n"(LOADS) : "memory");
        } else {
            __builtin_amdgcn_sched_barrier(0);
            asm volatile("s_waitcnt lgkmcnt(0) vmcnt(0)\n\ts_barrier" ::: "memory");
        }
        __builtin_amdgcn_sched_barrier(0);
        mfma_tile();
        pp_barrier();
        buf3 = buf3 == 2 ? 0 : buf3 + 1;
    };
    const unsigned long long t_loop = DLIMG_STAMPS(a) ? __builtin_amdgcn_s_memtime() : 0ull;
    const unsigned long long r_loop = DLIMG_STAMPS(a) ? __builtin_amdgcn_s_memrealtime() : 0ull;
    int t = 0;
    for (; t + 2 < nk; ++t) step(t, std::true_type{});
    for (; t < nk; ++t) step(t, std::false_type{});
    if (wr == 0) pp_barrier();
    const unsigned long long t_loop_end = DLIMG_STAMPS(a) ? __builtin_amdgcn_s_memtime() : 0ull;
    const unsigned long long r_loop_end = DLIMG_STAMPS(a) ? __builtin_amdgcn_s_memrealtime() : 0ull;

    PPAux<BM, EPI>::merge(a, rowpart, rowstat);
    pp_epilogue<NI, ACT, EPI, PRE>(a, acc, smem, rowstat, colvec, rowpart, m0, n0, wr * (BM / 2), wc, wave, lane, PRE ? rpre : nullptr);
    if (DLIMG_STAMPS(a) && threadIdx.x == 0) {
        asm volatile("s_waitcnt vmcnt(0)" ::: "memory");
        unsigned long long* d = DLIMG_STAMPS(a) + (size_t)blockIdx.x * 4;
        d[0] = t_loop_end - t_loop;
        d[1] = r_loop_end - r_loop;
        d[2] = (__builtin_amdgcn_s_memtime() - t_loop_end) & 0xffffffffull;
        d[3] = 0;
    }
}

typedef void (*GemmKernel)(k::GemmArgs);

struct Timing { hipEvent_t start = nullptr, stop = nullptr; };

void launch_flavour(GemmKernel const (&kernels)[5], k::LdsOptIn (&opt_in)[5], const k::GemmArgs& a, int grid,
                    int threads, size_t lds, hipStream_t s, Timing t) {
    const int index = a.stats_out ? 4 : (a.ln_stats ? 2 : 0) + (a.act == k::ACT_GELU ? 1 : 0);
    if (lds > 48 * 1024)
        opt_in[index].ensure((const void*)kernels[index], lds, "gemm: the device refuses the LDS size of this tile configuration");
    if (t.start && t.stop)
        hipExtLaunchKernelGGL(kernels[index], dim3(grid), dim3(threads), lds, s, t.start, t.stop, 0, a);
    else
        hipLaunchKernelGGL(kernels[index], dim3(grid), dim3(threads), lds, s, a);
}

template <int TILE>
constexpr bool tile_row_is(int bm, int bn, int threads, size_t lds, k::TileFamily family, int stat_capacity) {
    constexpr k::GemmTile row = k::kGemmTiles[TILE];
    return row.bm == bm && row.bn == bn && row.threads == threads && (size_t)row.lds == lds && row.family == family &&
           row.pair_stream == (family == k::TileFamily::pingpong) && row.stat_groups <= stat_capacity &&
           row.lds * row.per_cu <= 160 * 1024;
}
template <int TILE>
void launch_tile(GemmKernel const (&kernels)[5], k::LdsOptIn (&opt_in)[5], const k::GemmArgs& a, hipStream_t s, Timing t) {
    constexpr k::GemmTile row = k::kGemmTiles[TILE];
    launch_flavour(kernels, opt_in, a, (a.M / row.bm) * (a.N / row.bn), row.threads, row.lds, s, t);
}

template <int TILE, int BM, int BN, int WGM, int WGN, int NSTAGE, int MINW>
void launch16(const k::GemmArgs& a, hipStream_t s, Timing t) {
    static_assert(tile_row_is<TILE>(BM, BN, 64 * WGM * WGN, (size_t)NSTAGE * (BM + BN) * 64 + aux_bytes(BM, BN), k::TileFamily::ring16,
                                    kStatRegs * (64 * WGM * WGN / BM)), "gemm16_f16_kernel: the kernel and its row of k::kGemmTiles disagree");
    static const GemmKernel kernels[5] = {
        gemm16_f16_kernel<BM, BN, WGM, WGN, NSTAGE, MINW, k::ACT_NONE, EPI_PLAIN>,
        gemm16_f16_kernel<BM, BN, WGM, WGN, NSTAGE, MINW, k::ACT_GELU, EPI_PLAIN>,
        gemm16_f16_kernel<BM, BN, WGM, WGN, NSTAGE, MINW, k::ACT_NONE, EPI_NORM>,
        gemm16_f16_kernel<BM, BN, WGM, WGN, NSTAGE, MINW, k::ACT_GELU, EPI_NORM>,
        gemm16_f16_kernel<BM, BN, WGM, WGN, NSTAGE, MINW, k::ACT_NONE, EPI_STATS>,
    };
    static k::LdsOptIn attr_once[5];
    launch_tile<TILE>(kernels, attr_once, a, s, t);
}

template <int TILE, int BM, int BN, int WGM, int WGN, int BKT, int NSTAGE, int MINW>
void launch(const k::GemmArgs& a, hipStream_t s, Timing t) {
    static_assert(tile_row_is<TILE>(BM, BN, 64 * WGM * WGN, (size_t)NSTAGE * (BM + BN) * BKT * 2 + aux_bytes(BM, BN), k::TileFamily::ring32,
                                    kStatRegs * (64 * WGM * WGN / BM)), "gemm_f16_kernel: the kernel and its row of k::kGemmTiles disagree");
#ifdef DLIMG_TUNING
    static const int ablate = [] { const char* e = std::getenv("DLIMGEDIT_GEMM_ABLATE"); return e ? std::atoi(e) : 0; }();
#endif
    static const GemmKernel kernels[5] = {
#ifdef DLIMG_TUNING
        ablate == 1   ? gemm_f16_kernel<BM, BN, WGM, WGN, BKT, NSTAGE, MINW, k::ACT_NONE, EPI_PLAIN, 1>
        : ablate == 2 ? gemm_f16_kernel<BM, BN, WGM, WGN, BKT, NSTAGE, MINW, k::ACT_NONE, EPI_PLAIN, 2> :
#endif
        gemm_f16_kernel<BM, BN, WGM, WGN, BKT, NSTAGE, MINW, k::ACT_NONE, EPI_PLAIN>,
        gemm_f16_kernel<BM, BN, WGM, WGN, BKT, NSTAGE, MINW, k::ACT_GELU, EPI_PLAIN>,
        gemm_f16_kernel<BM, BN, WGM, WGN, BKT, NSTAGE, MINW, k::ACT_NONE, EPI_NORM>,
        gemm_f16_kernel<BM, BN, WGM, WGN, BKT, NSTAGE, MINW, k::ACT_GELU, EPI_NORM>,
        gemm_f16_kernel<BM, BN, WGM, WGN, BKT, NSTAGE, MINW, k::ACT_NONE, EPI_STATS>,
    };
    static k::LdsOptIn attr_once[5];
    launch_tile<TILE>(kernels, attr_once, a, s, t);
}

template <int TILE>
void launch_pp(const k::GemmArgs& a, hipStream_t s, Timing t) {
    static_assert(tile_row_is<TILE>(256, 256, 512, kPPLds, k::TileFamily::pingpong, kPPStatGroups), "gemm_pp_kernel: the kernel and its row of k::kGemmTiles disagree");
    static const GemmKernel kernels[5] = {
        gemm_pp_kernel<k::ACT_NONE, EPI_PLAIN>, gemm_pp_kernel<k::ACT_GELU, EPI_PLAIN>, gemm_pp_kernel<k::ACT_NONE, EPI_NORM>,
        gemm_pp_kernel<k::ACT_GELU, EPI_NORM>,  gemm_pp_kernel<k::ACT_NONE, EPI_STATS>,
    };
    static k::LdsOptIn attr_once[5];
    launch_tile<TILE>(kernels, attr_once, a, s, t);
}

template <int TILE, int BM>
void launch_pp128(const k::GemmArgs& a, hipStream_t s, Timing t) {
    static_assert(tile_row_is<TILE>(BM, 256, 512, pp128_lds(BM), k::TileFamily::pingpong, kPPStatGroups), "gemm_pp128_kernel: the kernel and its row of k::kGemmTiles disagree");
    static const GemmKernel kernels[5] = {
        gemm_pp128_kernel<BM, k::ACT_NONE, EPI_PLAIN>, gemm_pp128_kernel<BM, k::ACT_GELU, EPI_PLAIN>,
        gemm_pp128_kernel<BM, k::ACT_NONE, EPI_NORM>,  gemm_pp128_kernel<BM, k::ACT_GELU, EPI_NORM>,
        gemm_pp128_kernel<BM, k::ACT_NONE, EPI_STATS>,
    };
    static k::LdsOptIn attr_once[5];
    launch_tile<TILE>(kernels, attr_once, a, s, t);
}

typedef void (*TileLauncher)(const k::GemmArgs&, hipStream_t, Timing);
constexpr TileLauncher kLaunchers[k::kGemmNumTiles] = {
    launch<0, 128, 384, 2, 2, 64, 2, 1>, launch<1, 128, 288, 4, 1, 64, 3, 1>, launch<2, 128, 128, 2, 2, 64, 2, 4>,
    launch<3, 128, 96, 4, 1, 64, 4, 1>,  launch<4, 128, 64, 2, 2, 64, 2, 3>,  launch<5, 64, 64, 2, 2, 64, 2, 4>,
    launch<6, 256, 256, 2, 4, 32, 4, 2>, launch16<7, 256, 256, 2, 4, 4, 2>,   launch16<8, 128, 128, 2, 2, 4, 2>,
    launch_pp<9>,                        launch_pp128<10, 128>,               launch_pp128<11, 64>,
};

}

namespace k {

void gemm(const GemmArgs& a, hipStream_t s, hipEvent_t start, hipEvent_t stop) {
    if (const char* err = gemm_check(a)) throw_error(err);
    const int tile = gemm_pick_tile(a);
    if (tile < 0) gemm_no_tile(a);
    kLaunchers[tile](a, s, Timing{start, stop});
}

}
}
```

dlimgedit_amd/csrc/kernels/kernels.hpp:

```cpp
#pragma once

#include <hip/hip_runtime.h>
#include <stdint.h>

namespace dlimg {

typedef _Float16 half_t;

[[noreturn]] void throw_error(const char* msg);

namespace k {

class LdsOptIn {
  public:
    static constexpr int kMaxDevices = 64;
    void ensure(const void* kernel, size_t bytes, const char* refused_message) {
        int dev = 0;
        if (hipGetDevice(&dev) != hipSuccess || dev < 0 || dev >= kMaxDevices) throw_error("kernel launch: no current HIP device");
        int st = __atomic_load_n(&state_[dev], __ATOMIC_ACQUIRE);
        if (st == 0) {
            st = hipFuncSetAttribute(kernel, hipFuncAttributeMaxDynamicSharedMemorySize, (int)bytes) == hipSuccess ? 1 : -1;
            if (st < 0) (void)hipGetLastError();
            __atomic_store_n(&state_[dev], st, __ATOMIC_RELEASE);
        }
        if (st < 0) throw_error(refused_message);
    }

  private:
    int state_[kMaxDevices] = {};
};

enum Act { ACT_NONE = 0, ACT_GELU = 1 };

struct GemmArgs {
    const half_t* A = nullptr;  int lda = 0;
    const half_t* W = nullptr;  int ldw = 0;
    const float* bias = nullptr;
    const float* resid = nullptr; int ldr = 0; int resid_mod = 1;
    float* out_f32 = nullptr;   int ldc32 = 0;
    half_t* out_h = nullptr;    int ldc16 = 0;
    const half_t* resid_h = nullptr; const half_t* resid_l = nullptr; int ldrs = 0;
    half_t* out_l = nullptr;
    int M = 0, N = 0, K = 0;
    int act = ACT_NONE;
    float* stats_out = nullptr;
    const float* ln_stats = nullptr;
    int ln_groups = 0;
    const float* ln_colsum = nullptr;
    float ln_eps = 0.f;
    bool shared_gpu = false;
    bool alone = false;
    int tile = -1;
    int unit_rows = 0;
    unsigned long long* stamps = nullptr;
};
const char* gemm_check(const GemmArgs&);
bool gemm_tile_fits(const GemmArgs&, int tile);
int gemm_pick_tile(const GemmArgs&);
int gemm_choose_tile(GemmArgs&);
void gemm(const GemmArgs&, hipStream_t, hipEvent_t start = nullptr, hipEvent_t stop = nullptr);

void layernorm(const float* x, const float* w, const float* b, float eps, int rows, int D, int act,
               float* out_f32, half_t* out_h, hipStream_t, int* nonfinite = nullptr);

void preprocess(const uint8_t* img, int w, int h, int stride, int channels, half_t* patches, hipStream_t);
struct PreImage { const uint8_t* img; int w, h, stride, channels; half_t* patches; };
void preprocess_batch(const PreImage* images, int count, hipStream_t);

struct ResizeAxis { const int* first; const int* count; const float* coef; int taps; int out; };
void resize_srgb(const uint8_t* src, int w, int h, int stride, int C, const ResizeAxis& ax, const ResizeAxis& ay,
                 const float* decode_lut, const uint32_t* encode_tab, float* tmp, uint8_t* dst, hipStream_t);

struct ResizeJob { const uint8_t* src; int w, h, stride, channels; ResizeAxis ax, ay; float* tmp; half_t* patches; };
size_t resize_preprocess_tmp_floats(int h, int rw, int channels);
void resize_preprocess_batch(const ResizeJob* jobs, int count, const float* decode_lut, const uint32_t* encode_tab,
                             hipStream_t);

void add_cast(const float* a, const float* b, size_t b_mod, size_t n, float* out_f32, half_t* out_h, hipStream_t);
void im2col3x3(const half_t* in, int B, int C, half_t* out, hipStream_t);
void cast_f16(const float* in, half_t* out, size_t n, hipStream_t);

void attention_window(const half_t* qkv, const half_t* qkv_pad, const half_t* rel_h, const half_t* rel_w,
                      half_t* out, int B, int heads, int hd, hipStream_t);
float attention_global_q_scale(int hd);
float attention_global_rel_scale(int hd);
void attention_global(const half_t* qkv, const half_t* rel_h, const half_t* rel_w, half_t* out, int B,
                      int heads, int hd, hipStream_t);

constexpr int kDecoderMaxRows = 112;
constexpr int kDecoderMaxPoints = 10;
constexpr int kDecoderMaxTokens = 5 + kDecoderMaxPoints;
constexpr bool decoder_tokens_supported(int T) { return T >= 7 && T <= kDecoderMaxTokens; }
constexpr int decoder_max_prompts(int T) { return kDecoderMaxRows / T; }
constexpr int decoder_prompt_slice(int T) { return T <= 8 ? 2 : 1; }
size_t token_to_image_scratch_floats(int P, int T);
struct TokenRows {
    const float* x = nullptr;
    const float* ln_w = nullptr;
    const float* ln_b = nullptr;
    float eps = 0.f;
    const float* add = nullptr;
};
struct TokenLinear {
    TokenRows in;
    int K = 0;
    const float* W = nullptr;
    const float* b = nullptr;
    TokenRows resid;
    float* Y = nullptr;
    int N = 0;
    int relu = 0;
};
constexpr int kDecoderMaxPrompts = 16;
struct DecoderPrompts {
    float coords[kDecoderMaxPrompts * kDecoderMaxPoints * 2];
    float labels[kDecoderMaxPrompts * kDecoderMaxPoints];
    const float* emb[kDecoderMaxPrompts];
};
constexpr int kMaskHidden = 16;
struct MaskBranch {
    const float* w1 = nullptr; const float* b1 = nullptr; const float* ln1_w = nullptr; const float* ln1_b = nullptr;
    const float* w2 = nullptr; const float* b2 = nullptr; const float* ln2_w = nullptr; const float* ln2_b = nullptr;
    const float* proj_w = nullptr; const float* proj_b = nullptr;
};
struct MaskSource { const float* logits4; const float* iou4; };
void mask_embed(const MaskSource* src, const MaskBranch& branch, float* h , int P, hipStream_t);
constexpr float kDecoderHqLabel = -1024.0f;
struct PromptEncoderWeights {
    const float* gauss = nullptr; const float* point_embed = nullptr; const float* not_a_point = nullptr;
    const float* iou_token = nullptr; const float* mask_tokens = nullptr;
};
struct DecoderStartInputs {
    DecoderPrompts prompts{};
    PromptEncoderWeights pe;
    float* tokens = nullptr;
    const TokenLinear* first = nullptr;
    int n_first = 0;
    float* keys = nullptr;
    half_t* keys_h = nullptr;
    const float* no_mask = nullptr;
    const float* const* mask_h = nullptr;
    const MaskBranch* mask = nullptr;
    const float* hq_token = nullptr;
};
void decoder_start(const DecoderStartInputs& in, int P, int T, hipStream_t s);
void token_linears(const TokenLinear* ops, int count, int rows, int T, hipStream_t);
void token_self_attention_out(const float* q, const float* k, const float* v, const TokenLinear& out, int P, int T, hipStream_t);
bool token_self_attention_out_with_gemm(const float* q, const float* k, const float* v, const TokenLinear& out, int P, int T,
                                        const GemmArgs& g, hipStream_t);
void token_to_image_partials(const float* q, const TokenLinear* q_proj, const half_t* K, int ldk, const half_t* V, int ldv,
                             float* scratch, int P, int T, hipStream_t);
void token_merge_linear(const float* scratch, const TokenLinear& out, const float* out_wt, const TokenLinear& next, int P,
                        int T, hipStream_t);
void image_update(const half_t* q, int ldq, const float* tk, const float* tv, const half_t* W, const float* bias,
                  const float* ln_w, const float* ln_b, float eps, float* keys, half_t* keys_h, int P, int T, hipStream_t);
void upscale_logits(const half_t* keys_h, const half_t* W1, const float* b1, const float* ln_w, const float* ln_b, float eps,
                    const half_t* W2, const float* b2, const float* hyper, float* logits, int P, hipStream_t, half_t* u_out = nullptr);
struct HeadWeights { const float* w[5][3]; const float* b[5][3]; };
struct HqHead { const float* w[3]; const float* b[3]; float* hyper_hq; };
void output_heads(const float* scratch, const TokenLinear& out, const float* out_wt, const TokenRows& norm ,
                  const HeadWeights& hw, float* hyper , float* iou , int P, int T, hipStream_t,
                  const HqHead* hq = nullptr);

void hq_features_finish(const float* vit, const float* emb, const float* b_vit, const float* b_emb, float* out, hipStream_t);
struct HqMaskWeights {
    const half_t* conv1_w = nullptr; const float* conv1_b = nullptr; const float* ln_w = nullptr; const float* ln_b = nullptr;
    const half_t* conv2_w = nullptr; const float* conv2_b = nullptr;
};
void hq_mask_path(const half_t* U, const HqMaskWeights& w, float eps, half_t* H, const float* const* features,
                  const float* hyper_hq, float* logits, int P, hipStream_t);

void birefnet_prepare_image(const uint8_t* pixels, int w, int h, int stride, int bytes_pp, const float mean[3],
                            const float std[3], float* out, hipStream_t s);
void birefnet_process_mask(const float* logits, int w, int h, uint8_t* out, hipStream_t s);

struct PostJob { const float* src; const float* select_iou; uint8_t* dst; int out_w, out_h, pre_w, pre_h; };
void postprocess_masks(const PostJob* jobs_host, int count, hipStream_t);

}
}
```

dlimgedit_amd/csrc/sam_model.cpp:

```cpp
#include "sam_model.hpp"
#include "gemm_plan.hpp"
#include "image_memory.hpp"

#include <algorithm>
#include <cmath>
#include <cstdlib>
#include <cstring>

namespace dlimg {

namespace {

constexpr float kLnEps = 1e-6f;
constexpr float kDecLnEps = 1e-5f;

hipStream_t make_lane_stream(int device, int lane_index) {
    HIP_CHECK(hipSetDevice(device));
    hipStream_t stream = nullptr;
    static const bool plain = [] {
        if (const char* e = std::getenv("DLIMGEDIT_PLAIN_STREAMS")) return std::atoi(e) != 0;
        return hardware_queues_trusted();
    }();
    if (plain) {
        HIP_CHECK(hipStreamCreateWithFlags(&stream, hipStreamNonBlocking));
    } else {
        int least = 0, greatest = 0;
        HIP_CHECK(hipDeviceGetStreamPriorityRange(&least, &greatest));
        const int prio = least + (greatest - least) * (lane_index % 3) / 2;
        HIP_CHECK(hipStreamCreateWithPriority(&stream, hipStreamNonBlocking, prio));
    }
    return stream;
}

}

SamModel::SamModel(std::shared_ptr<SamWeights const> weights, int lane_index, int lane_count, std::shared_ptr<LaneBoard> board)
    : device_(weights->device), shared_gpu_(lane_count > 1), board_(std::move(board)), lane_index_(lane_index),
      stream_(make_lane_stream(device_, lane_index)), weights_(std::move(weights)), clock_(stream_), done_events_(stream_),
      masks_(device_, stream_, clock_, board_.get(), lane_index_) {
    for (auto& st : stage_) HIP_CHECK(hipEventCreateWithFlags(&st.copied, hipEventDisableTiming));
    HIP_CHECK(hipEventCreateWithFlags(&caller_copied_, hipEventDisableTiming));
}

SamModel::~SamModel() {
    if (stream_) (void)hipStreamSynchronize(stream_);
    for (auto& d : flag_owner_) {
        try {
            if (d) d->settle();
        } catch (...) {
        }
    }
    for (auto& st : stage_)
        if (st.copied) (void)hipEventDestroy(st.copied);
    if (caller_copied_) (void)hipEventDestroy(caller_copied_);
    if (stream_) (void)hipStreamDestroy(stream_);
    if (pass_flags_) (void)hipHostFree(pass_flags_);
}

void SamModel::gemm(k::GemmArgs const& args, Stage shape) {
    k::GemmArgs a = args;
    plan_inputs(a, shared_gpu_, alone_);
    if (!clock_.profiling()) {
        k::gemm(a, stream_);
        return;
    }
    const Stage flavour = a.stats_out ? ST_GEMM_STATS : a.ln_stats ? (a.act == k::ACT_GELU ? ST_GEMM_NORM_GELU : ST_GEMM_NORM) : ST_GEMM_OTHER;
    const StageClock::Pending p = clock_.event_pair(ST_GEMM, 2.0 * a.M * a.N * a.K, flavour, shape);
    k::gemm(a, stream_, p.a, p.b);
    clock_.add(p);
}

void SamModel::synchronize() { HIP_CHECK(hipStreamSynchronize(stream_)); }

std::shared_ptr<SamModel::DeferredPass> SamModel::defer_last_pass() {
    DLIMG_ASSERT(pass_flag_ != nullptr);
    auto d = std::make_shared<DeferredPass>();
    d->lane = this;
    d->done_ = completion();
    d->flag_ = pass_flag_;
    flag_owner_[pass_flag_ - pass_flags_] = d;
    return d;
}

bool SamModel::DeferredPass::settle() {
    std::lock_guard<std::mutex> lock(mutex_);
    if (!settled_) {
        settled_ = true;
        lane->wait_and_recycle(done_);
        overflowed_ = *flag_ != 0;
        *const_cast<volatile int*>(flag_) = 0;
    }
    return overflowed_;
}


void SamModel::reserve_encoder(int batch) {
    SamWeights const& W = *weights_;
    if (batch <= enc_batch_) return;
    HIP_CHECK(hipStreamSynchronize(stream_));
    const size_t M = (size_t)batch * kTokens;
    const size_t D = W.geom_.embed_dim;
    const size_t wide = std::max<size_t>(W.geom_.mlp_dim, 9 * kEmbedDim);
    img_dev_.reserve((size_t)batch * kImageSize * kImageSize * 4);
    patches_.reserve(M * kPatchK);
    split_stream_ = W.fused_ln_ && shared_gpu_ && D % 256 == 0 && split_stream_allowed();
    if (split_stream_) xlo_.reserve(M * D);
    else x_.reserve(M * D);
    xn_.reserve(M * D);
    xstat_.reserve(M * k::kGemmMaxStatGroups * 2);
    qkv_.reserve(M * 3 * D);
    att_.reserve(M * std::max<size_t>(D, kEmbedDim));
    hid_.reserve(M * wide);
    neck_f32_.reserve(M * kEmbedDim);
    emb_.reserve(M * kEmbedDim);
    if (W.has_hq()) {
        hq_a_.reserve(M * 4 * kEmbedDim);
        hq_h_.reserve(M * 4 * kEmbedDim);
        hq_vit_.reserve(M * 4 * 128);
        hq_embf_.reserve(M * 4 * 128);
        emb_h_.reserve(M * kEmbedDim);
        hq_feat_.reserve((size_t)batch * kHqFeatureFloats);
    }
    enc_batch_ = batch;
}

bool SamModel::split_stream_allowed() {
    static const bool on = [] { const char* e = std::getenv("DLIMGEDIT_SPLIT_STREAM"); return !e || std::atoi(e) != 0; }();
    return on;
}

void SamModel::preprocess_device_image(int slot, int batch, uint8_t const* dev_pixels, int w, int h, int stride,
                                       int channels) {
    DLIMG_ASSERT(slot >= 0 && slot < batch);
    reserve_encoder(batch);
    forget_staged_resize(slot);
    const int bytes = channels > 4 ? 4 : channels;
    clock_.timed(ST_PRE, (double)w * h * bytes + (double)kTokens * kPatchK * 2, [&] {
        k::preprocess(dev_pixels, w, h, stride, channels, patches_.get() + (size_t)slot * kTokens * kPatchK, stream_);
    });
}

void SamModel::preprocess_device_images(dlimg_ImageView const* views, int const* resized_wh, int batch) {
    DLIMG_ASSERT(views != nullptr && resized_wh != nullptr && batch > 0);
    reserve_encoder(batch);
    staged_resizes_.clear();
    std::vector<k::PreImage> images;
    std::vector<ResizeRequest> resizes;
    double bytes = 0;
    for (int i = 0; i < batch; ++i) {
        dlimg_ImageView const& v = views[i];
        const int rw = resized_wh[i * 2], rh = resized_wh[i * 2 + 1];
        if (rw == v.width && rh == v.height) {
            const int px = v.channels > 4 ? 4 : v.channels;
            images.push_back(k::PreImage{v.pixels, v.width, v.height, v.stride, v.channels,
                                         patches_.get() + (size_t)i * kTokens * kPatchK});
            bytes += (double)v.width * v.height * px + (double)kTokens * kPatchK * 2;
        } else {
            resizes.push_back(ResizeRequest{v.pixels, v.width, v.height, v.stride, v.channels, rw, rh, i});
        }
    }
    if (!images.empty()) clock_.timed(ST_PRE, bytes, [&] { k::preprocess_batch(images.data(), (int)images.size(), stream_); });
    if (!resizes.empty()) resize_into_patches(resizes.data(), (int)resizes.size());
}

uint8_t* SamModel::stage_rows(uint8_t const* pixels, size_t row_bytes, int rows, int stride, hipEvent_t* copied) {
    ImageStage& st = stage_[stage_seq_++ % kStageRing];
    HIP_CHECK(hipEventSynchronize(st.copied));
    st.pin.reserve(row_bytes * rows);
    uint8_t* pin = static_cast<uint8_t*>(st.pin.get());
    if ((size_t)stride == row_bytes) {
        std::memcpy(pin, pixels, row_bytes * rows);
    } else {
        for (int y = 0; y < rows; ++y) std::memcpy(pin + y * row_bytes, pixels + (size_t)y * stride, row_bytes);
    }
    *copied = st.copied;
    return pin;
}

void SamModel::upload_image(int slot, int batch, uint8_t const* pixels, int w, int h, int stride, int channels) {
    DLIMG_ASSERT(slot >= 0 && slot < batch);
    DLIMG_ASSERT(w > 0 && h > 0 && w <= kImageSize && h <= kImageSize);
    reserve_encoder(batch);
    const int bytes = channels > 4 ? 4 : channels;
    const size_t row = (size_t)w * bytes;
    const size_t slot_bytes = (size_t)kImageSize * kImageSize * 4;
    uint8_t* dev = img_dev_.get() + slot * slot_bytes;
    if ((size_t)stride == row && image_memory_is_pinned(pixels, row * h)) {
        HIP_CHECK(hipMemcpyAsync(dev, pixels, row * h, hipMemcpyHostToDevice, stream_));
        HIP_CHECK(hipEventRecord(caller_copied_, stream_));
        caller_copy_pending_ = true;
        preprocess_device_image(slot, batch, dev, w, h, (int)row, channels);
        return;
    }
    ImageStage& st = stage_[stage_seq_++ % kStageRing];
    HIP_CHECK(hipEventSynchronize(st.copied));
    st.pin.reserve(row * h);
    uint8_t* pin = static_cast<uint8_t*>(st.pin.get());
    const int pieces = (int)std::min<size_t>(8, std::max<size_t>(1, row * h / (1u << 20)));
    for (int p = 0; p < pieces; ++p) {
        const int y0 = (int)((long)h * p / pieces), y1 = (int)((long)h * (p + 1) / pieces);
        if ((size_t)stride == row) {
            std::memcpy(pin + (size_t)y0 * row, pixels + (size_t)y0 * stride, row * (size_t)(y1 - y0));
        } else {
            for (int y = y0; y < y1; ++y) std::memcpy(pin + (size_t)y * row, pixels + (size_t)y * stride, row);
        }
        HIP_CHECK(hipMemcpyAsync(dev + (size_t)y0 * row, pin + (size_t)y0 * row, row * (size_t)(y1 - y0), hipMemcpyHostToDevice, stream_));
    }
    HIP_CHECK(hipEventRecord(st.copied, stream_));
    preprocess_device_image(slot, batch, dev, w, h, (int)row, channels);
}

void SamModel::wait_caller_copies() {
    if (!caller_copy_pending_) return;
    caller_copy_pending_ = false;
    HIP_CHECK(hipEventSynchronize(caller_copied_));
}

std::shared_ptr<SamModel::AxisDev const> SamModel::axis_table(int in_size, int out_size) {
    for (size_t i = 0; i < axis_cache_.size(); ++i)
        if (axis_cache_[i]->in_size == in_size && axis_cache_[i]->out_size == out_size) {
            std::rotate(axis_cache_.begin() + i, axis_cache_.begin() + i + 1, axis_cache_.end());
            return axis_cache_.back();
        }
    AxisTable t = make_axis_table(in_size, out_size);
    auto a = std::make_shared<AxisDev>();
    a->in_size = in_size;
    a->out_size = out_size;
    a->taps = t.taps;
    const size_t n_first = t.first.size() * sizeof(int), n_count = t.count.size() * sizeof(int);
    const size_t n_coef = t.coef.size() * sizeof(float);
    a->host.reserve(n_first + n_count + n_coef);
    a->dev.reserve(n_first + n_count + n_coef);
    uint8_t* host = static_cast<uint8_t*>(a->host.get());
    std::memcpy(host, t.first.data(), n_first);
    std::memcpy(host + n_first, t.count.data(), n_count);
    std::memcpy(host + n_first + n_count, t.coef.data(), n_coef);
    HIP_CHECK(hipMemcpyAsync(a->dev.get(), host, n_first + n_count + n_coef, hipMemcpyHostToDevice, stream_));
    a->first = reinterpret_cast<int const*>(a->dev.get());
    a->count = reinterpret_cast<int const*>(a->dev.get() + n_first);
    a->coef = reinterpret_cast<float const*>(a->dev.get() + n_first + n_count);
    if (axis_cache_.size() >= kAxisCacheEntries) {
        HIP_CHECK(hipStreamSynchronize(stream_));
        axis_cache_.erase(axis_cache_.begin());
    }
    axis_cache_.push_back(a);
    return a;
}

void SamModel::resize_into_patches(ResizeRequest const* requests, int count) {
    constexpr int kGroup = (int)(kAxisCacheEntries / 2);
    if (count > kGroup) {
        for (int base = 0; base < count; base += kGroup) resize_into_patches(requests + base, std::min(kGroup, count - base));
        return;
    }
    if (!srgb_decode_.get()) {
        float lut[256];
        srgb_decode_table(lut);
        srgb_decode_.reserve(256);
        srgb_encode_.reserve(104);
        HIP_CHECK(hipMemcpy(srgb_decode_.get(), lut, sizeof(lut), hipMemcpyHostToDevice));
        HIP_CHECK(hipMemcpy(srgb_encode_.get(), kSrgbEncodeTab4, sizeof(kSrgbEncodeTab4), hipMemcpyHostToDevice));
    }
    std::vector<std::shared_ptr<AxisDev const>> held((size_t)count * 2);
    std::vector<size_t> offset(count);
    size_t floats = 0;
    double bytes = 0;
    for (int i = 0; i < count; ++i) {
        ResizeRequest const& r = requests[i];
        DLIMG_ASSERT(r.slot >= 0 && r.slot < enc_batch_);
        DLIMG_ASSERT(r.w > 0 && r.h > 0 && r.rw > 0 && r.rh > 0 && r.rw <= kImageSize && r.rh <= kImageSize);
        held[i * 2] = axis_table(r.w, r.rw);
        held[i * 2 + 1] = axis_table(r.h, r.rh);
        offset[i] = floats;
        floats += k::resize_preprocess_tmp_floats(r.h, r.rw, r.channels);
        bytes += (double)r.w * r.h * (r.channels > 4 ? 4 : r.channels) + (double)kTokens * kPatchK * 2;
    }
    if (floats > resize_tmp_.capacity()) {
        HIP_CHECK(hipStreamSynchronize(stream_));
        resize_tmp_.reserve(floats);
    }
    std::vector<k::ResizeJob> jobs(count);
    for (int i = 0; i < count; ++i) {
        ResizeRequest const& r = requests[i];
        AxisDev const& ax = *held[i * 2];
        AxisDev const& ay = *held[i * 2 + 1];
        jobs[i] = k::ResizeJob{r.pixels, r.w, r.h, r.stride, r.channels,
                               k::ResizeAxis{ax.first, ax.count, ax.coef, ax.taps, r.rw},
                               k::ResizeAxis{ay.first, ay.count, ay.coef, ay.taps, r.rh},
                               resize_tmp_.get() + offset[i], patches_.get() + (size_t)r.slot * kTokens * kPatchK};
    }
    clock_.timed(ST_PRE, bytes, [&] {
        k::resize_preprocess_batch(jobs.data(), count, srgb_decode_.get(), srgb_encode_.get(), stream_);
    });
}

void SamModel::upload_and_resize_image(int slot, int batch, uint8_t const* pixels, int w, int h, int stride, int channels,
                                       int rw, int rh) {
    DLIMG_ASSERT(slot >= 0 && slot < batch);
    DLIMG_ASSERT(w > 0 && h > 0 && rw > 0 && rh > 0 && rw <= kImageSize && rh <= kImageSize);
    reserve_encoder(batch);
    const int bytes = channels > 4 ? 4 : channels;
    const size_t row = (size_t)w * bytes;
    forget_staged_resize(slot);
    if ((int)resize_src_.size() <= slot) resize_src_.resize(slot + 1);
    DeviceBuffer<uint8_t>& src = resize_src_[slot];
    if (row * h > src.capacity()) {
        HIP_CHECK(hipStreamSynchronize(stream_));
        src.reserve(row * h);
    }
    if ((size_t)stride == row && image_memory_is_pinned(pixels, row * h)) {
        HIP_CHECK(hipMemcpyAsync(src.get(), pixels, row * h, hipMemcpyHostToDevice, stream_));
        HIP_CHECK(hipEventRecord(caller_copied_, stream_));
        caller_copy_pending_ = true;
    } else {
        hipEvent_t copied = nullptr;
        uint8_t* pin = stage_rows(pixels, row, h, stride, &copied);
        HIP_CHECK(hipMemcpyAsync(src.get(), pin, row * h, hipMemcpyHostToDevice, stream_));
        HIP_CHECK(hipEventRecord(copied, stream_));
    }
    staged_resizes_.push_back(ResizeRequest{src.get(), w, h, (int)row, channels, rw, rh, slot});
}

void SamModel::forget_staged_resize(int slot) {
    staged_resizes_.erase(std::remove_if(staged_resizes_.begin(), staged_resizes_.end(),
                                         [slot](ResizeRequest const& r) { return r.slot == slot; }),
                          staged_resizes_.end());
}

void SamModel::run_staged_resizes(int batch) {
    if (staged_resizes_.empty()) return;
    std::vector<ResizeRequest> now;
    now.swap(staged_resizes_);
    now.erase(std::remove_if(now.begin(), now.end(), [batch](ResizeRequest const& r) { return r.slot >= batch; }), now.end());
    if (!now.empty()) resize_into_patches(now.data(), (int)now.size());
}

void SamModel::encode(int batch, float* const* emb_dst) {
    SamWeights const& W = *weights_;
    DLIMG_ASSERT(batch > 0 && batch <= enc_batch_);
    run_staged_resizes(batch);
    alone_ = batch == 1 && shared_gpu_ && board_ && board_->others_idle(lane_index_);
    if (board_ && batch == 1) board_->count_pass(alone_);
    begin_activity();
    struct EndOnExit {
        LaneBoard* board; int lane;
        ~EndOnExit() { if (board) board->end(lane); }
    } end_on_exit{board_.get(), lane_index_};
    const int D = W.geom_.embed_dim, H = W.geom_.num_heads, hd = W.geom_.head_dim(), mlp = W.geom_.mlp_dim;
    const int M = batch * kTokens;

    const bool fused = W.fused_ln_;
    int stat_groups = 0;
    const bool split = split_stream_;
    auto stream_residual = [&](k::GemmArgs& a) {
        if (split) { a.resid_h = xn_.get(); a.resid_l = xlo_.get(); a.ldrs = D; }
        else { a.resid = x_.get(); a.ldr = D; }
        a.resid_mod = M;
    };
    auto writes_stream = [&](k::GemmArgs& a) {
        a.M = M; a.N = D;
        if (split) { a.out_l = xlo_.get(); }
        else { a.out_f32 = x_.get(); a.ldc32 = D; }
        if (fused) {
            a.out_h = xn_.get(); a.ldc16 = D; a.stats_out = xstat_.get();
            plan_inputs(a, shared_gpu_, alone_);
            stat_groups = D / k::gemm_choose_tile(a);
        }
    };
    auto reads_stream = [&](k::GemmArgs& a, LinearH const& lin, NormW const& norm) {
        if (fused) {
            a.ln_stats = xstat_.get(); a.ln_groups = stat_groups; a.ln_colsum = lin.colsum.get(); a.ln_eps = kLnEps;
        } else {
            clock_.timed(ST_LAYERNORM, (double)M * D * 6, [&] {
                k::layernorm(x_.get(), norm.w.get(), norm.b.get(), kLnEps, M, D, k::ACT_NONE, nullptr, xn_.get(), stream_);
            });
        }
        a.A = xn_.get(); a.lda = D; a.W = lin.w.get(); a.ldw = D; a.bias = lin.b.get(); a.M = M; a.N = lin.out; a.K = D;
    };

    k::GemmArgs g;
    g.A = patches_.get(); g.lda = kPatchK; g.W = W.patch_.w.get(); g.ldw = kPatchK; g.bias = W.patch_.b.get();
    g.resid = W.pos_embed_.get(); g.ldr = D; g.resid_mod = kTokens; g.K = kPatchK;
    writes_stream(g);
    gemm(g, ST_GEMM_PATCH);

    int layer_index = 0, first_global = -1;
    for (int gi : W.geom_.global_attn_indexes)
        if (first_global < 0 || gi < first_global) first_global = gi;
    for (EncoderLayer const& L : W.layers_) {
        g = k::GemmArgs{};
        reads_stream(g, L.qkv, L.ln1);
        g.out_h = qkv_.get(); g.ldc16 = 3 * D;
        gemm(g);
        if (L.global) {
            const double fl = (double)batch * (4.0 * kTokens * (double)kTokens * D + 4.0 * kTokens * 64.0 * hd * H);
            clock_.timed(ST_ATTN_GLOBAL, fl, [&] {
                k::attention_global(qkv_.get(), L.rel_h16.get(), L.rel_w16.get(), att_.get(), batch, H, hd, stream_);
            });
        } else {
            const double fl = (double)batch * 25.0 * (4.0 * 196.0 * 196.0 * D + 4.0 * 196.0 * 14.0 * hd * H);
            clock_.timed(ST_ATTN_WINDOW, fl, [&] {
                k::attention_window(qkv_.get(), L.qkv_pad.get(), L.rel_h16.get(), L.rel_w16.get(), att_.get(), batch, H, hd,
                                    stream_);
            });
        }
        g = k::GemmArgs{};
        g.A = att_.get(); g.lda = D; g.W = L.proj.w.get(); g.ldw = D; g.bias = L.proj.b.get(); g.K = D;
        stream_residual(g);
        writes_stream(g);
        gemm(g, ST_GEMM_PROJ);
        g = k::GemmArgs{};
        reads_stream(g, L.fc1, L.ln2);
        g.act = k::ACT_GELU; g.out_h = hid_.get(); g.ldc16 = mlp;
        gemm(g);
        g = k::GemmArgs{};
        g.A = hid_.get(); g.lda = mlp; g.W = L.fc2.w.get(); g.ldw = mlp; g.bias = L.fc2.b.get(); g.K = mlp;
        stream_residual(g);
        writes_stream(g);
        gemm(g, ST_GEMM_FC2);
        if (W.has_hq() && layer_index == first_global) {
            if (!fused) {
                clock_.timed(ST_ENC_OTHER, (double)M * D * 6, [&] {
                    k::add_cast(x_.get(), nullptr, 0, (size_t)M * D, nullptr, xn_.get(), stream_);
                });
            }
            hq_gemm_pair(xn_.get(), D, W.hq_vit1_, W.hq_vit_ln_, W.hq_vit2_, M, hq_vit_.get());
        }
        ++layer_index;
    }

    if (!fused) {
        clock_.timed(ST_ENC_OTHER, (double)M * D * 6, [&] {
            k::add_cast(x_.get(), nullptr, 0, (size_t)M * D, nullptr, xn_.get(), stream_);
        });
    }
    g = k::GemmArgs{};
    g.A = xn_.get(); g.lda = D; g.W = W.neck1_.w.get(); g.ldw = D;
    g.out_f32 = neck_f32_.get(); g.ldc32 = kEmbedDim; g.M = M; g.N = kEmbedDim; g.K = D;
    gemm(g);
    clock_.timed(ST_LAYERNORM, (double)M * kEmbedDim * 6, [&] {
        k::layernorm(neck_f32_.get(), W.neck_ln1_.w.get(), W.neck_ln1_.b.get(), kLnEps, M, kEmbedDim, k::ACT_NONE, nullptr,
                     att_.get(), stream_);
    });
    clock_.timed(ST_ENC_OTHER, (double)M * kEmbedDim * 2 * 10, [&] {
        k::im2col3x3(att_.get(), batch, kEmbedDim, hid_.get(), stream_);
    });
    g = k::GemmArgs{};
    g.A = hid_.get(); g.lda = 9 * kEmbedDim; g.W = W.neck2_.w.get(); g.ldw = 9 * kEmbedDim;
    g.out_f32 = neck_f32_.get(); g.ldc32 = kEmbedDim; g.M = M; g.N = kEmbedDim; g.K = 9 * kEmbedDim;
    gemm(g);
    float* direct = (emb_dst && batch == 1 && emb_dst[0]) ? emb_dst[0] : nullptr;
    if (!pass_flags_) {
        HIP_CHECK(hipHostMalloc(reinterpret_cast<void**>(&pass_flags_), kPassFlags * sizeof(int), hipHostMallocDefault));
        std::memset(pass_flags_, 0, kPassFlags * sizeof(int));
    }
    const unsigned flag_slot = pass_counter_++ % kPassFlags;
    if (flag_owner_[flag_slot]) {
        flag_owner_[flag_slot]->settle();
        flag_owner_[flag_slot].reset();
    }
    pass_flag_ = pass_flags_ + flag_slot;
    *pass_flag_ = 0;
    clock_.timed(ST_LAYERNORM, (double)M * kEmbedDim * 8, [&] {
        k::layernorm(neck_f32_.get(), W.neck_ln2_.w.get(), W.neck_ln2_.b.get(), kLnEps, M, kEmbedDim, k::ACT_NONE,
                     direct ? direct : emb_.get(), W.has_hq() ? emb_h_.get() : nullptr, stream_, pass_flag_);
    });
    if (W.has_hq()) {
        hq_gemm_pair(emb_h_.get(), kEmbedDim, W.hq_emb1_, W.hq_emb_ln_, W.hq_emb2_, M, hq_embf_.get());
        clock_.timed(ST_ENC_OTHER, (double)batch * kHqFeatureFloats * 12, [&] {
            for (int i = 0; i < batch; ++i) {
                float* dst = (emb_dst && emb_dst[i]) ? emb_dst[i] + kEmbeddingFloats : hq_feat_.get() + (size_t)i * kHqFeatureFloats;
                const size_t off = (size_t)i * kTokens * 4 * 128;
                k::hq_features_finish(hq_vit_.get() + off, hq_embf_.get() + off, W.hq_vit2_.b.get(), W.hq_emb2_.b.get(), dst, stream_);
            }
        });
    }
    if (emb_dst && !direct) {
        const size_t n = (size_t)kTokens * kEmbedDim;
        for (int i = 0; i < batch; ++i)
            if (emb_dst[i])
                HIP_CHECK(hipMemcpyAsync(emb_dst[i], emb_.get() + i * n, n * sizeof(float), hipMemcpyDeviceToDevice, stream_));
    }
    HIP_CHECK(hipGetLastError());
    mark_activity();
}

void SamModel::hq_gemm_pair(half_t const* a, int K, LinearH const& conv1, NormW const& ln, LinearH const& conv2, int M, float* out) {
    const int C = conv1.out / 4;
    k::GemmArgs g;
    g.A = a; g.lda = K; g.W = conv1.w.get(); g.ldw = K; g.bias = conv1.b.get();
    g.out_f32 = hq_a_.get(); g.ldc32 = conv1.out; g.M = M; g.N = conv1.out; g.K = K;
    gemm(g);
    clock_.timed(ST_LAYERNORM, (double)M * conv1.out * 6, [&] {
        k::layernorm(hq_a_.get(), ln.w.get(), ln.b.get(), kLnEps, 4 * M, C, k::ACT_GELU, nullptr, hq_h_.get(), stream_);
    });
    g = k::GemmArgs{};
    g.A = hq_h_.get(); g.lda = C; g.W = conv2.w.get(); g.ldw = C;
    g.out_f32 = out; g.ldc32 = conv2.out; g.M = 4 * M; g.N = conv2.out; g.K = C;
    gemm(g);
}


void SamModel::reserve_decoder(int count) {
    if (count <= dec_count_) return;
    HIP_CHECK(hipStreamSynchronize(stream_));
    const size_t P = count, M = P * kTokens;
    keys_.reserve(M * 256);
    keys_h_.reserve(M * 256);
    kqv_h_.reserve(M * 384);
    logits_.reserve(P * 4 * kLowRes * kLowRes);
    iou_.reserve(P * 4);
    hyper_.reserve(P * 4 * 32);
    const size_t T = P * kDecMaxTokens;
    tokens_.reserve(T * 256);
    queries_.reserve(T * 256);
    tk_.reserve(T * 256);
    tv_.reserve(T * 256);
    sq_.reserve(T * 256);
    sk_.reserve(T * 256);
    sv_.reserve(T * 256);
    tsa_.reserve(T * 256);
    tt2i_.reserve(T * 256);
    t2i_part_.reserve(k::token_to_image_scratch_floats((int)P, kDecMaxTokens));
    tmlp_.reserve(T * 2048);
    if (weights_->has_hq()) {
        const size_t L = std::min<size_t>(P, k::decoder_max_prompts(8));
        hyper_hq_.reserve(P * 32);
        hq_u_.reserve(L * kLowRes * kLowRes * 32);
        hq_mid_.reserve(L * kLowRes * kLowRes * 64);
    }
    dec_count_ = count;
}

std::string SamModel::hq_refusal(int points) const {
    if (!has_hq() || points <= kHqMaxPoints) return {};
    return "a prompt of " + std::to_string(points) + " packed points (8 clicks and a box) is more than a SAM-HQ model takes: at most " +
           std::to_string(kHqMaxPoints) + " points, because the HQ token of the model file's dec.hq.* group travels as the 15th and last "
           "token row of the decoder";
}

void SamModel::decode(float const* const* emb, float const* coords, float const* labels, int count, int points,
                      k::MaskSource const* mask_input, bool handles) {
    DLIMG_ASSERT(count > 0);
    if (mask_input && !has_mask_branch()) throw Exception("a mask input needs the prompt encoder's mask branch: the model file has no pe.mask.* tensors");
    DLIMG_ASSERT(points >= 2 && points <= k::kDecoderMaxPoints);
    std::vector<float> hq_coords, hq_labels;
    if (has_hq()) {
        if (!handles)
            throw Exception("a SAM-HQ model (dec.hq.* in the model file) does not decode bare embeddings: the HQ features of the "
                            "image are part of the decode, and only a Segmentation handle holds them");
        const std::string why = hq_refusal(points);
        if (!why.empty()) throw Exception(why);
        const int np = points + 1;
        hq_coords.assign((size_t)count * np * 2, 0.f);
        hq_labels.assign((size_t)count * np, k::kDecoderHqLabel);
        for (int i = 0; i < count; ++i) {
            std::copy_n(coords + (size_t)i * points * 2, points * 2, hq_coords.data() + (size_t)i * np * 2);
            std::copy_n(labels + (size_t)i * points, points, hq_labels.data() + (size_t)i * np);
        }
        coords = hq_coords.data();
        labels = hq_labels.data();
        points = np;
    }
    static_assert(5 + k::kDecoderMaxPoints == kDecMaxTokens && k::decoder_tokens_supported(kDecTokens) &&
                  k::decoder_tokens_supported(kDecMaxTokens), "the kernels are built for these token counts");
    reserve_decoder(count);
    const int chunk = k::decoder_max_prompts(5 + points);
    if (mask_input) {
        DLIMG_ASSERT(count <= chunk);
        const size_t need = (size_t)count * kTokens * k::kMaskHidden;
        if (need > mask_h_.capacity()) {
            HIP_CHECK(hipStreamSynchronize(stream_));
            mask_h_.reserve(need);
        }
    }
    for (int c0 = 0; c0 < count; c0 += chunk)
        decode_chunk(emb + c0, coords + (size_t)c0 * points * 2, labels + (size_t)c0 * points, std::min(chunk, count - c0), c0,
                     points, mask_input ? mask_input + c0 : nullptr);
    mark_activity();
}

void SamModel::decode_chunk(float const* const* emb, float const* coords, float const* labels, int count, int first,
                            int points, k::MaskSource const* mask_input) {
    SamWeights const& W = *weights_;
    const int TOK = 5 + points;
    const bool hq = W.has_hq();
    const int P = count, M = P * kTokens, T = P * TOK;
    hipStream_t s = stream_;
    float* logits_out = logits_.get() + (size_t)first * 4 * kLowRes * kLowRes;
    float* iou_out = iou_.get() + (size_t)first * 4;

    auto body = [&] {
        k::DecoderStartInputs start;
        std::memcpy(start.prompts.coords, coords, (size_t)P * points * 2 * sizeof(float));
        std::memcpy(start.prompts.labels, labels, (size_t)P * points * sizeof(float));
        for (int i = 0; i < P; ++i) start.prompts.emb[i] = emb[i];

        float const* qpe = tokens_.get();
        k::TokenRows cur;
        auto rows_of = [&](k::TokenRows r, bool with_pe) { if (with_pe) r.add = qpe; return r; };
        auto lin = [&](k::TokenRows in, int K, LinearF const& l, k::TokenRows resid, float* Y, int relu) {
            k::TokenLinear op;
            op.in = in; op.K = K; op.W = l.w.get(); op.b = l.b.get(); op.resid = resid; op.Y = Y; op.N = l.out; op.relu = relu;
            return op;
        };
        auto plain = [&](float const* x) { k::TokenRows r; r.x = x; return r; };
        auto normed = [&](float const* x, NormW const& n) {
            k::TokenRows r; r.x = x; r.ln_w = n.w.get(); r.ln_b = n.b.get(); r.eps = kDecLnEps; return r;
        };
        auto img_gemm_args = [&](LinearH const& l, DeviceBuffer<float> const& pos) {
            k::GemmArgs g;
            g.A = keys_h_.get(); g.lda = 256; g.W = l.w.get(); g.ldw = 256; g.bias = l.b.get();
            g.resid = pos.get(); g.ldr = l.out; g.resid_mod = kTokens;
            g.out_h = kqv_h_.get(); g.ldc16 = l.out; g.M = M; g.N = l.out; g.K = 256;
            plan_inputs(g, shared_gpu_,  false);
            return g;
        };
        auto img_gemm = [&](LinearH const& l, DeviceBuffer<float> const& pos) { k::gemm(img_gemm_args(l, pos), s); };

        {
            DecoderLayer const& L = W.dec_[0];
            k::TokenLinear qkv[3] = {lin({}, 256, L.self_attn.q, {}, sq_.get(), 0), lin({}, 256, L.self_attn.k, {}, sk_.get(), 0),
                                     lin({}, 256, L.self_attn.v, {}, sv_.get(), 0)};
            start.pe = W.prompt_encoder();
            start.tokens = tokens_.get(); start.first = qkv; start.n_first = 3;
            start.keys = keys_.get(); start.keys_h = keys_h_.get();
            if (hq) start.hq_token = W.hq_token_.get();
            const k::MaskBranch branch = W.mask_branch();
            float const* h[k::kDecoderMaxPrompts];
            if (mask_input) {
                k::mask_embed(mask_input, branch, mask_h_.get(), P, s);
                for (int i = 0; i < P; ++i) h[i] = mask_h_.get() + (size_t)i * kTokens * k::kMaskHidden;
                start.mask_h = h; start.mask = &branch;
            } else {
                start.no_mask = W.pe_no_mask_.get();
            }
            k::decoder_start(start, P, TOK, s);
        }
        for (int i = 0; i < 2; ++i) {
            DecoderLayer const& L = W.dec_[i];
            const k::TokenLinear self_out = lin({}, 256, L.self_attn.o, i == 0 ? k::TokenRows{} : cur, tsa_.get(), 0);
            static const bool ride = [] { const char* e = std::getenv("DLIMGEDIT_DECODER_RIDE"); return !e || std::atoi(e) != 0; }();
            if (!ride || !k::token_self_attention_out_with_gemm(sq_.get(), sk_.get(), sv_.get(), self_out, P, TOK, img_gemm_args(L.img_kqv, L.pos_kqv), s)) {
                k::token_self_attention_out(sq_.get(), sk_.get(), sv_.get(), self_out, P, TOK, s);
                img_gemm(L.img_kqv, L.pos_kqv);
            }
            const k::TokenRows q1 = normed(tsa_.get(), L.ln1);
            const k::TokenLinear tq = lin(rows_of(q1, true), 256, L.t2i_q, {}, nullptr, 0);
            k::token_to_image_partials(nullptr, &tq, kqv_h_.get(), 384, kqv_h_.get() + 256, 384, t2i_part_.get(), P, TOK, s);
            const k::TokenRows q2 = normed(tt2i_.get(), L.ln2);
            k::token_merge_linear(t2i_part_.get(), lin({}, 128, L.t2i_o, q1, tt2i_.get(), 0), L.t2i_o_t.get(),
                                  lin(q2, 256, L.mlp1, {}, tmlp_.get(), 1), P, TOK, s);
            k::TokenLinear m2 = lin(plain(tmlp_.get()), 2048, L.mlp2, q2, queries_.get(), 0);
            k::token_linears(&m2, 1, T, TOK, s);
            const k::TokenRows q3 = normed(queries_.get(), L.ln3);
            k::TokenLinear kv[5] = {lin(rows_of(q3, true), 256, L.i2t_k, {}, tk_.get(), 0),
                                    lin(q3, 256, L.i2t_v, {}, tv_.get(), 0)};
            int n_ops = 2;
            if (i == 0) {
                DecoderLayer const& N = W.dec_[1];
                kv[n_ops++] = lin(rows_of(q3, true), 256, N.self_attn.q, {}, sq_.get(), 0);
                kv[n_ops++] = lin(rows_of(q3, true), 256, N.self_attn.k, {}, sk_.get(), 0);
                kv[n_ops++] = lin(q3, 256, N.self_attn.v, {}, sv_.get(), 0);
            } else {
                kv[n_ops++] = lin(rows_of(q3, true), 256, W.final_q_, {}, sq_.get(), 0);
            }
            k::token_linears(kv, n_ops, T, TOK, s);
            k::image_update(kqv_h_.get() + 128, 384, tk_.get(), tv_.get(), L.i2t_o.w.get(), L.i2t_o.b.get(), L.ln4.w.get(),
                            L.ln4.b.get(), kDecLnEps, keys_.get(), keys_h_.get(), P, TOK, s);
            cur = q3;
        }
        img_gemm(W.final_kv_, W.final_pos_kv_);
        k::token_to_image_partials(sq_.get(), nullptr, kqv_h_.get(), 256, kqv_h_.get() + 128, 256, t2i_part_.get(), P, TOK, s);

        k::HeadWeights hw;
        for (int m = 0; m < 5; ++m)
            for (int j = 0; j < 3; ++j) {
                hw.w[m][j] = W.heads_[m][j].w.get();
                hw.b[m][j] = W.heads_[m][j].b.get();
            }
        k::HqHead hq_head{};
        if (hq) {
            for (int j = 0; j < 3; ++j) {
                hq_head.w[j] = W.hq_mlp_[j].w.get();
                hq_head.b[j] = W.hq_mlp_[j].b.get();
            }
            hq_head.hyper_hq = hyper_hq_.get();
        }
        k::output_heads(t2i_part_.get(), lin({}, 128, W.final_o_, cur, nullptr, 0), W.final_o_t_.get(), normed(nullptr, W.ln_final_),
                        hw, hyper_.get(), iou_out, P, TOK, s, hq ? &hq_head : nullptr);
        k::upscale_logits(keys_h_.get(), W.up1_.w.get(), W.up1_.b.get(), W.up_ln_.w.get(), W.up_ln_.b.get(), kLnEps,
                          W.up2_.w.get(), W.up2_.b.get(), hyper_.get(), logits_out, P, s, hq ? hq_u_.get() : nullptr);
        if (hq) {
            float const* feat[k::kDecoderMaxPrompts];
            for (int i = 0; i < P; ++i) feat[i] = emb[i] + kEmbeddingFloats;
            k::hq_mask_path(hq_u_.get(), W.hq_mask_weights(), kLnEps, hq_mid_.get(), feat, hyper_hq_.get(), logits_out, P, s);
        }
    };
    clock_.timed(ST_DECODER, (hq ? 3.62e9 + 4.83e9 : 3.62e9) * P, body);
    HIP_CHECK(hipGetLastError());
}

std::vector<std::pair<const char*, size_t>> SamModel::decoder_state_layout() { return decoder_state_layout(kDecTokens); }

std::vector<std::pair<const char*, size_t>> SamModel::decoder_state_layout(int tokens, bool with_mask_h, bool with_hq) {
    DLIMG_ASSERT(k::decoder_tokens_supported(tokens));
    const size_t T = (size_t)tokens;
    std::vector<std::pair<const char*, size_t>> parts = {
        {"tokens", T * 256}, {"final_q", T * 128}, {"self_k", T * 256}, {"self_v", T * 256}, {"self_out", T * 256},
        {"t2i_out", T * 256}, {"mlp_hidden", T * 2048}, {"queries", T * 256}, {"i2t_k", T * 128}, {"i2t_v", T * 128},
        {"final_partials", k::token_to_image_scratch_floats(1, tokens)}, {"hyper", 4 * 32}, {"iou", 4}, {"keys_head", 4096}};
    if (with_mask_h) parts.push_back({"mask_h", (size_t)kTokens * k::kMaskHidden});
    if (with_hq) parts.push_back({"hyper_hq", 32});
    return parts;
}

void SamModel::decoder_state(float* out) const { decoder_state(out, kDecTokens); }

void SamModel::decoder_state(float* out, int tokens, bool with_mask_h, bool with_hq) const {
    std::vector<float const*> src = {tokens_.get(), sq_.get(), sk_.get(), sv_.get(), tsa_.get(), tt2i_.get(), tmlp_.get(), queries_.get(),
                                     tk_.get(), tv_.get(), t2i_part_.get(), hyper_.get(), iou_.get(), keys_.get()};
    if (with_mask_h) {
        DLIMG_ASSERT(mask_h_.capacity() >= (size_t)kTokens * k::kMaskHidden);
        src.push_back(mask_h_.get());
    }
    if (with_hq) {
        DLIMG_ASSERT(hyper_hq_.capacity() >= 32);
        src.push_back(hyper_hq_.get());
    }
    size_t off = 0, i = 0;
    for (auto const& part : decoder_state_layout(tokens, with_mask_h, with_hq)) {
        HIP_CHECK(hipMemcpy(out + off, src[i++], part.second * sizeof(float), hipMemcpyDeviceToHost));
        off += part.second;
    }
}

void SamModel::masks_on_device(k::PostJob const* jobs, int count) {
    if (count <= 0) return;
    double bytes = 0;
    for (int i = 0; i < count; ++i) bytes += (double)kLowRes * kLowRes * 4 + (double)jobs[i].out_w * jobs[i].out_h;
    clock_.timed(ST_POST, bytes, [&] { k::postprocess_masks(jobs, count, stream_); });
    mark_activity();
}

void SamModel::masks_to_host(k::PostJob const* jobs, int count) {
    MaskSlotLease lease(*this);
    enqueue_masks(lease.slot(), jobs, count, 0);
    finish_masks(lease.slot(), jobs, count, nullptr, 0);
}

}
```

dlimgedit_amd/csrc/sam_model.hpp:

```cpp
#pragma once

#include "common.hpp"

#include <dlimgedit/dlimgedit.h>
#include "completion_events.hpp"
#include "kernels/kernels.hpp"
#include "lane_board.hpp"
#include "mask_transport_exec.hpp"
#include "resize_tables.hpp"
#include "stage_clock.hpp"
#include "weights.hpp"

#include <array>
#include <memory>
#include <mutex>
#include <string>
#include <vector>

namespace dlimg {

constexpr int kTokens = 4096;
constexpr int kEmbedDim = 256;
constexpr int kPatchK = 768;
constexpr int kImageSize = 1024;
constexpr int kDecTokens = 7;
constexpr int kDecMaxTokens = 15;
constexpr int kLowRes = 256;

struct LinearH {
    DeviceBuffer<half_t> w;
    DeviceBuffer<float> b;
    int out = 0, in = 0;
    bool has_bias = false;
    DeviceBuffer<float> colsum;
};
struct LinearF {
    DeviceBuffer<float> w, b;
    int out = 0, in = 0;
};
struct NormW { DeviceBuffer<float> w, b; };

struct EncoderLayer {
    bool global = false;
    NormW ln1, ln2;
    LinearH qkv, proj, fc1, fc2;
    DeviceBuffer<half_t> qkv_pad;
    DeviceBuffer<half_t> rel_h16, rel_w16;
};

struct TokenAttention { LinearF q, k, v, o; };

struct DecoderLayer {
    TokenAttention self_attn;
    NormW ln1, ln2, ln3, ln4;
    LinearF t2i_q, t2i_o;
    DeviceBuffer<float> t2i_o_t;
    LinearH img_kqv;
    DeviceBuffer<float> pos_kqv;
    LinearF mlp1, mlp2;
    LinearF i2t_k, i2t_v;
    LinearH i2t_o;
};

struct SamWeights {
    explicit SamWeights(std::string const& weight_path, int device);
    SamWeights(SamWeights const&) = delete;
    SamWeights& operator=(SamWeights const&) = delete;

    int device = 0;
    SamGeometry geom_;
    bool fused_ln_ = true;
    LinearH patch_;
    DeviceBuffer<float> pos_embed_;
    std::vector<EncoderLayer> layers_;
    LinearH neck1_, neck2_;
    NormW neck_ln1_, neck_ln2_;
    DeviceBuffer<float> pe_gauss_, pe_point_, pe_not_a_point_, pe_no_mask_;
    k::PromptEncoderWeights prompt_encoder() const {
        return k::PromptEncoderWeights{pe_gauss_.get(), pe_point_.get(), pe_not_a_point_.get(), iou_token_.get(), mask_tokens_.get()};
    }
    bool has_mask_branch_ = false;
    DeviceBuffer<float> mask_w1_, mask_b1_, mask_w2_, mask_b2_, mask_proj_w_, mask_proj_b_;
    NormW mask_ln1_, mask_ln2_;
    k::MaskBranch mask_branch() const {
        k::MaskBranch b;
        b.w1 = mask_w1_.get(); b.b1 = mask_b1_.get(); b.ln1_w = mask_ln1_.w.get(); b.ln1_b = mask_ln1_.b.get();
        b.w2 = mask_w2_.get(); b.b2 = mask_b2_.get(); b.ln2_w = mask_ln2_.w.get(); b.ln2_b = mask_ln2_.b.get();
        b.proj_w = mask_proj_w_.get(); b.proj_b = mask_proj_b_.get();
        return b;
    }
    DeviceBuffer<float> iou_token_, mask_tokens_;
    std::array<DecoderLayer, 2> dec_;
    LinearF final_q_, final_o_;
    DeviceBuffer<float> final_o_t_;
    LinearH final_kv_;
    DeviceBuffer<float> final_pos_kv_;
    NormW ln_final_;
    LinearH up1_, up2_;
    NormW up_ln_;
    std::array<std::array<LinearF, 3>, 5> heads_;
    bool has_hq_ = false;
    bool has_hq() const { return has_hq_; }
    DeviceBuffer<float> hq_token_;
    std::array<LinearF, 3> hq_mlp_;
    LinearH hq_vit1_, hq_vit2_, hq_emb1_, hq_emb2_;
    NormW hq_vit_ln_, hq_emb_ln_, hq_mask_ln_;
    DeviceBuffer<half_t> hq_conv1_w_, hq_conv2_w_;
    DeviceBuffer<float> hq_conv1_b_, hq_conv2_b_;
    k::HqMaskWeights hq_mask_weights() const {
        k::HqMaskWeights w;
        w.conv1_w = hq_conv1_w_.get(); w.conv1_b = hq_conv1_b_.get(); w.ln_w = hq_mask_ln_.w.get(); w.ln_b = hq_mask_ln_.b.get();
        w.conv2_w = hq_conv2_w_.get(); w.conv2_b = hq_conv2_b_.get();
        return w;
    }
};

constexpr size_t kEmbeddingFloats = (size_t)kTokens * kEmbedDim;
constexpr size_t kHqFeatureFloats = (size_t)kLowRes * kLowRes * 32;
constexpr size_t handle_floats(bool hq) { return kEmbeddingFloats + (hq ? kHqFeatureFloats : 0); }
constexpr int kHqMaxPoints = 9;

class SamModel {
  public:
    explicit SamModel(std::shared_ptr<SamWeights const> weights, int lane_index = 0, int lane_count = 1,
                      std::shared_ptr<LaneBoard> board = nullptr);
    ~SamModel();
    SamModel(SamModel const&) = delete;
    SamModel& operator=(SamModel const&) = delete;

    SamGeometry const& geometry() const { return weights_->geom_; }
    hipStream_t stream() const { return stream_; }
    std::mutex& mutex() { return mutex_; }
    int device() const { return device_; }
    int lane_index() const { return lane_index_; }
    LaneBoard const* board() const { return board_.get(); }


    void upload_image(int slot, int batch, uint8_t const* pixels, int w, int h, int stride, int channels);
    void wait_caller_copies();
    void upload_and_resize_image(int slot, int batch, uint8_t const* pixels, int w, int h, int stride, int channels,
                                 int rw, int rh);
    void preprocess_device_image(int slot, int batch, uint8_t const* dev_pixels, int w, int h, int stride, int channels);
    void preprocess_device_images(dlimg_ImageView const* views, int const* resized_wh, int batch);
    void encode(int batch, float* const* emb_dst = nullptr);
    bool has_hq() const { return weights_->has_hq_; }
    float const* embeddings() const { return emb_.get(); }

    void decode(float const* const* emb, float const* coords, float const* labels, int count, int points = 2,
                k::MaskSource const* mask_input = nullptr, bool handles = false);
    std::string hq_refusal(int points) const;
    bool has_mask_branch() const { return weights_->has_mask_branch_; }
    float const* logits() const { return logits_.get(); }
    static std::vector<std::pair<const char*, size_t>> decoder_state_layout();
    void decoder_state(float* out) const;
    static std::vector<std::pair<const char*, size_t>> decoder_state_layout(int tokens, bool with_mask_h = false, bool with_hq = false);
    void decoder_state(float* out, int tokens, bool with_mask_h = false, bool with_hq = false) const;
    float const* iou() const { return iou_.get(); }

    using MaskSlot = dlimg::MaskSlot;
    MaskSlot& acquire_mask_slot() { return masks_.acquire(); }
    void release_mask_slot(MaskSlot& s) { masks_.release(s); }
    void enqueue_masks(MaskSlot& slot, k::PostJob const* jobs, int count, int iou_count) { masks_.enqueue(slot, jobs, count, iou_.get(), iou_count); }
    void finish_masks(MaskSlot& slot, k::PostJob const* jobs, int count, float* iou_out, int iou_count) { masks_.finish(slot, jobs, count, iou_out, iou_count); }
    void enqueue_masks_device(MaskSlot& slot, k::PostJob const* jobs, int count, int dst_device) { masks_.enqueue_device(slot, jobs, count, dst_device); }
    void wait_masks(MaskSlot& slot) { masks_.wait(slot); }
    void masks_to_host(k::PostJob const* jobs, int count);
    void masks_on_device(k::PostJob const* jobs, int count);

    void synchronize();
    hipEvent_t completion() { return done_events_.record(); }
    static constexpr int kPassFlags = 64;
    const volatile int* last_pass_flag() const { return pass_flag_; }
    struct DeferredPass {
        SamModel* lane = nullptr;
        bool settle();
      private:
        friend class SamModel;
        std::mutex mutex_;
        hipEvent_t done_ = nullptr;
        const volatile int* flag_ = nullptr;
        bool settled_ = false, overflowed_ = false;
    };
    std::shared_ptr<DeferredPass> defer_last_pass();
    void wait_and_recycle(hipEvent_t e) { done_events_.wait_and_recycle(e); }
    bool poll_and_recycle(hipEvent_t e) { return done_events_.poll_and_recycle(e); }

    static void plan_inputs(k::GemmArgs& a, bool shared_gpu, bool alone) { a.shared_gpu = shared_gpu; a.alone = alone; a.unit_rows = kTokens; }

    void set_profiling(bool on) { clock_.set_profiling(on); }
    StageStats take_stats() { return clock_.take_stats(); }

  private:
    void reserve_encoder(int batch);
    void reserve_decoder(int count);
    void decode_chunk(float const* const* emb, float const* coords, float const* labels, int count, int first, int points,
                      k::MaskSource const* mask_input);
    void hq_gemm_pair(half_t const* a, int K, LinearH const& conv1, NormW const& ln, LinearH const& conv2, int M, float* out);
    void gemm(k::GemmArgs const& a, Stage shape = ST_COUNT);

    int device_ = 0;
    bool shared_gpu_ = false;
    std::shared_ptr<LaneBoard> board_;
    int lane_index_ = 0;
    bool alone_ = false;
    void mark_activity() { if (board_) board_->mark(lane_index_, stream_); }
    void begin_activity() { if (board_) board_->begin(lane_index_); }
    hipStream_t stream_ = nullptr;
    std::mutex mutex_;

    std::shared_ptr<SamWeights const> weights_;

    int enc_batch_ = 0;
    DeviceBuffer<uint8_t> img_dev_;
    static constexpr int kStageRing = 4;
    struct ImageStage { PinnedBuffer pin; hipEvent_t copied = nullptr; };
    ImageStage stage_[kStageRing];
    unsigned stage_seq_ = 0;
    hipEvent_t caller_copied_ = nullptr;
    bool caller_copy_pending_ = false;
    uint8_t* stage_rows(uint8_t const* pixels, size_t row_bytes, int rows, int stride, hipEvent_t* copied);
    DeviceBuffer<half_t> patches_, xn_, xlo_, qkv_, att_, hid_;
    DeviceBuffer<float> x_, xstat_, neck_f32_, emb_;
    DeviceBuffer<float> hq_a_, hq_vit_, hq_embf_, hq_feat_;
    DeviceBuffer<half_t> hq_h_, emb_h_;
    bool split_stream_ = false;
    static bool split_stream_allowed();

    struct AxisDev {
        int in_size = 0, out_size = 0, taps = 0;
        PinnedBuffer host;
        DeviceBuffer<uint8_t> dev;
        int const* first = nullptr;
        int const* count = nullptr;
        float const* coef = nullptr;
    };
    std::shared_ptr<AxisDev const> axis_table(int in_size, int out_size);
    static constexpr size_t kAxisCacheEntries = 64;
    std::vector<std::shared_ptr<AxisDev const>> axis_cache_;
    DeviceBuffer<float> srgb_decode_;
    DeviceBuffer<uint32_t> srgb_encode_;
    std::vector<DeviceBuffer<uint8_t>> resize_src_;
    DeviceBuffer<float> resize_tmp_;
    struct ResizeRequest { uint8_t const* pixels; int w, h, stride, channels, rw, rh, slot; };
    void resize_into_patches(ResizeRequest const* requests, int count);
    std::vector<ResizeRequest> staged_resizes_;
    void forget_staged_resize(int slot);
    void run_staged_resizes(int batch);

    int dec_count_ = 0;
    DeviceBuffer<float> keys_, logits_, iou_, hyper_;
    DeviceBuffer<float> hyper_hq_;
    DeviceBuffer<half_t> hq_u_, hq_mid_;
    DeviceBuffer<float> mask_h_;
    DeviceBuffer<half_t> keys_h_, kqv_h_;
    DeviceBuffer<float> tokens_, queries_, tk_, tv_, sq_, sk_, sv_, tsa_, tt2i_, tmlp_, t2i_part_;

    int* pass_flags_ = nullptr;
    int* pass_flag_ = nullptr;
    unsigned pass_counter_ = 0;
    std::shared_ptr<DeferredPass> flag_owner_[kPassFlags];

    StageClock clock_;
    CompletionEvents done_events_;
    MaskTransport masks_;
};

class MaskSlotLease {
  public:
    explicit MaskSlotLease(SamModel& model) : model_(&model), slot_(&model.acquire_mask_slot()) {}
    MaskSlotLease(MaskSlotLease&& o) noexcept : model_(o.model_), slot_(o.slot_) { o.slot_ = nullptr; }
    MaskSlotLease& operator=(MaskSlotLease&& o) noexcept {
        if (this != &o) {
            release();
            model_ = o.model_;
            slot_ = o.slot_;
            o.slot_ = nullptr;
        }
        return *this;
    }
    ~MaskSlotLease() { release(); }
    void release() noexcept {
        if (slot_) model_->release_mask_slot(*slot_);
        slot_ = nullptr;
    }
    bool held() const { return slot_ != nullptr; }
    SamModel& model() const { return *model_; }
    SamModel::MaskSlot& slot() const { return *slot_; }

  private:
    SamModel* model_;
    SamModel::MaskSlot* slot_;
};

}
```

dlimgedit_amd/csrc/sam_weights.cpp:

```cpp
#include "sam_model.hpp"

#include <cmath>
#include <cstdlib>
#include <cstring>

namespace dlimg {

namespace {

struct Loader {
    WeightFile const& file;
    hipStream_t stream;
    DeviceBuffer<float> staging;

    void f32(std::string const& name, std::vector<int64_t> const& dims, DeviceBuffer<float>& dst) {
        HostTensor const& t = file.get(name, dims);
        dst.reserve(t.numel());
        HIP_CHECK(hipMemcpy(dst.get(), t.data, t.numel() * 4, hipMemcpyHostToDevice));
    }
    void f32_host(std::vector<float> const& v, DeviceBuffer<float>& dst) {
        dst.reserve(v.size());
        HIP_CHECK(hipMemcpy(dst.get(), v.data(), v.size() * 4, hipMemcpyHostToDevice));
    }
    void f16_host(float const* src, size_t n, DeviceBuffer<half_t>& dst, std::string const& what) {
        for (size_t i = 0; i < n; ++i)
            if (!(std::fabs(src[i]) <= 65504.0f))
                throw Exception("'" + file.path() + "': " + what + " holds " + std::to_string(src[i]) + " (element " +
                                std::to_string(i) + "), outside the f16 range of this build's MFMA operands");
        staging.reserve(n);
        dst.reserve(n);
        HIP_CHECK(hipMemcpy(staging.get(), src, n * 4, hipMemcpyHostToDevice));
        k::cast_f16(staging.get(), dst.get(), n, stream);
        HIP_CHECK(hipStreamSynchronize(stream));
    }
    void linear_h(std::string const& prefix, int out, int in, bool bias, LinearH& l, int head_rows = 0, float head_scale = 1.f) {
        HostTensor const& w = file.get(prefix + ".w", {out, in});
        if (head_rows > 0) {
            std::vector<float> ws(w.data, w.data + w.numel());
            for (size_t i = 0; i < (size_t)head_rows * in; ++i) ws[i] *= head_scale;
            f16_host(ws.data(), ws.size(), l.w, prefix + ".w");
        } else {
            f16_host(w.data, w.numel(), l.w, prefix + ".w");
        }
        l.out = out;
        l.in = in;
        l.has_bias = bias;
        if (bias && head_rows > 0) {
            HostTensor const& b = file.get(prefix + ".b", {out});
            std::vector<float> bs(b.data, b.data + out);
            for (int i = 0; i < head_rows; ++i) bs[i] *= head_scale;
            f32_host(bs, l.b);
        } else if (bias) {
            f32(prefix + ".b", {out}, l.b);
        }
    }
    void linear_ln_h(std::string const& prefix, std::string const& norm, int out, int in, LinearH& l, int head_rows = 0,
                     float head_scale = 1.f) {
        HostTensor const& w = file.get(prefix + ".w", {out, in});
        HostTensor const& b = file.get(prefix + ".b", {out});
        HostTensor const& gamma = file.get(norm + ".w", {in});
        HostTensor const& beta = file.get(norm + ".b", {in});
        std::vector<float> wg((size_t)out * in), colsum(out), bias(out);
        for (int n = 0; n < out; ++n) {
            const float rs = n < head_rows ? head_scale : 1.f;
            double sum = 0, shift = 0;
            for (int i = 0; i < in; ++i) {
                const float v = rs * w.data[(size_t)n * in + i] * gamma.data[i];
                wg[(size_t)n * in + i] = v;
                sum += (double)(float)(half_t)v;
                shift += (double)rs * w.data[(size_t)n * in + i] * beta.data[i];
            }
            colsum[n] = (float)sum;
            bias[n] = (float)((double)rs * b.data[n] + shift);
        }
        f16_host(wg.data(), wg.size(), l.w, prefix + ".w scaled by " + norm + ".w");
        f32_host(bias, l.b);
        f32_host(colsum, l.colsum);
        l.out = out;
        l.in = in;
        l.has_bias = true;
    }
    void linear_f(std::string const& prefix, int out, int in, LinearF& l) {
        f32(prefix + ".w", {out, in}, l.w);
        f32(prefix + ".b", {out}, l.b);
        l.out = out;
        l.in = in;
    }
    void transposed_f(std::string const& prefix, int out, int in, DeviceBuffer<float>& dst) {
        HostTensor const& w = file.get(prefix + ".w", {out, in});
        std::vector<float> t((size_t)out * in);
        for (int n = 0; n < out; ++n)
            for (int i = 0; i < in; ++i) t[(size_t)i * out + n] = w.data[(size_t)n * in + i];
        f32_host(t, dst);
    }
    void norm(std::string const& prefix, int dim, NormW& n) {
        f32(prefix + ".w", {dim}, n.w);
        f32(prefix + ".b", {dim}, n.b);
    }
    void attention(std::string const& prefix, int dim, int inner, TokenAttention& a) {
        linear_f(prefix + ".q", inner, dim, a.q);
        linear_f(prefix + ".k", inner, dim, a.k);
        linear_f(prefix + ".v", inner, dim, a.v);
        linear_f(prefix + ".o", dim, inner, a.o);
    }
    void fused_h(std::vector<std::string> const& parts, int out_each, int in, LinearH& l) {
        const size_t n = parts.size();
        std::vector<float> w(n * (size_t)out_each * in), b(n * (size_t)out_each);
        for (size_t i = 0; i < n; ++i) {
            HostTensor const& wi = file.get(parts[i] + ".w", {out_each, in});
            HostTensor const& bi = file.get(parts[i] + ".b", {out_each});
            std::memcpy(w.data() + i * wi.numel(), wi.data, wi.numel() * 4);
            std::memcpy(b.data() + i * out_each, bi.data, bi.numel() * 4);
        }
        f16_host(w.data(), w.size(), l.w, parts[0] + ".w (fused with its siblings)");
        f32_host(b, l.b);
        l.out = int(n) * out_each;
        l.in = in;
        l.has_bias = true;
    }
    void conv_transpose_h(std::string const& prefix, int ci_n, int co_n, LinearH& l) {
        HostTensor const& w = file.get(prefix + ".w", {ci_n, co_n, 2, 2});
        HostTensor const& b = file.get(prefix + ".b", {co_n});
        std::vector<float> g((size_t)4 * co_n * ci_n), gb((size_t)4 * co_n);
        for (int s = 0; s < 4; ++s)
            for (int co = 0; co < co_n; ++co) {
                gb[(size_t)s * co_n + co] = b.data[co];
                for (int ci = 0; ci < ci_n; ++ci)
                    g[((size_t)s * co_n + co) * ci_n + ci] = w.data[((size_t)ci * co_n + co) * 4 + s];
            }
        f16_host(g.data(), g.size(), l.w, prefix + ".w");
        f32_host(gb, l.b);
        l.out = 4 * co_n;
        l.in = ci_n;
        l.has_bias = true;
    }
};

}

SamWeights::SamWeights(std::string const& weight_path, int device_index) : device(device_index) {
    WeightFile file(weight_path);
    geom_ = file.geometry();
    const int D = geom_.embed_dim, hd = geom_.head_dim();
    if (D % 64 || geom_.mlp_dim % 64) throw Exception("SAM encoder width must be a multiple of 64");
    if (D != hd * geom_.num_heads || (hd != 64 && hd != 80))
        throw Exception("SAM encoder head dimension must be 64 or 80");
    if (const char* e = std::getenv("DLIMGEDIT_FUSED_LN")) fused_ln_ = std::atoi(e) != 0;

    HIP_CHECK(hipSetDevice(device));
    hipStream_t stream_ = nullptr;
    HIP_CHECK(hipStreamCreateWithFlags(&stream_, hipStreamNonBlocking));
    Loader ld{file, stream_, {}};

    ld.linear_h("enc.patch", D, kPatchK, true, patch_);
    ld.f32("enc.pos", {kTokens, D}, pos_embed_);
    layers_.resize(geom_.depth);
    for (int i = 0; i < geom_.depth; ++i) {
        EncoderLayer& L = layers_[i];
        const std::string p = "enc.L" + std::to_string(i);
        L.global = geom_.is_global(i);
        const int span = L.global ? 64 : 14;
        if (!L.global) {
            HostTensor const& qb = file.get(p + ".qkv.b", {3 * D});
            ld.f16_host(qb.data, qb.numel(), L.qkv_pad, p + ".qkv.b");
        }
        const int q_rows = L.global ? D : 0;
        const float q_scale = L.global ? k::attention_global_q_scale(hd) : 1.f;
        if (fused_ln_) {
            ld.linear_ln_h(p + ".qkv", p + ".ln1", 3 * D, D, L.qkv, q_rows, q_scale);
            ld.linear_ln_h(p + ".fc1", p + ".ln2", geom_.mlp_dim, D, L.fc1);
        } else {
            ld.norm(p + ".ln1", D, L.ln1);
            ld.norm(p + ".ln2", D, L.ln2);
            ld.linear_h(p + ".qkv", 3 * D, D, true, L.qkv, q_rows, q_scale);
            ld.linear_h(p + ".fc1", geom_.mlp_dim, D, true, L.fc1);
        }
        HostTensor const& rh = file.get(p + ".rel_h", {2 * span - 1, hd});
        HostTensor const& rw = file.get(p + ".rel_w", {2 * span - 1, hd});
        if (L.global) {
            std::vector<float> rhs(rh.data, rh.data + rh.numel()), rws(rw.data, rw.data + rw.numel());
            const float rel_scale = k::attention_global_rel_scale(hd);
            for (auto& v : rhs) v *= rel_scale;
            for (auto& v : rws) v *= rel_scale;
            ld.f16_host(rhs.data(), rhs.size(), L.rel_h16, p + ".rel_h");
            ld.f16_host(rws.data(), rws.size(), L.rel_w16, p + ".rel_w");
        } else {
            ld.f16_host(rh.data, rh.numel(), L.rel_h16, p + ".rel_h");
            ld.f16_host(rw.data, rw.numel(), L.rel_w16, p + ".rel_w");
        }
        ld.linear_h(p + ".proj", D, D, true, L.proj);
        ld.linear_h(p + ".fc2", D, geom_.mlp_dim, true, L.fc2);
    }
    ld.linear_h("enc.neck.conv1", kEmbedDim, D, false, neck1_);
    ld.norm("enc.neck.ln1", kEmbedDim, neck_ln1_);
    {
        HostTensor const& w = file.get("enc.neck.conv2.w", {kEmbedDim, kEmbedDim, 3, 3});
        std::vector<float> g(w.numel());
        for (int co = 0; co < kEmbedDim; ++co)
            for (int ci = 0; ci < kEmbedDim; ++ci)
                for (int t = 0; t < 9; ++t)
                    g[((size_t)co * 9 + t) * kEmbedDim + ci] = w.data[((size_t)co * kEmbedDim + ci) * 9 + t];
        ld.f16_host(g.data(), g.size(), neck2_.w, "enc.neck.conv2.w");
        neck2_.out = kEmbedDim;
        neck2_.in = 9 * kEmbedDim;
    }
    ld.norm("enc.neck.ln2", kEmbedDim, neck_ln2_);

    DeviceBuffer<half_t> pe_h;
    ld.f32("pe.gauss", {2, 128}, pe_gauss_);
    ld.f32("pe.point", {4, 256}, pe_point_);
    ld.f32("pe.not_a_point", {256}, pe_not_a_point_);
    ld.f32("pe.no_mask", {256}, pe_no_mask_);
    {
        static const char* const names[] = {"pe.mask.down1.w", "pe.mask.down1.b", "pe.mask.ln1.w", "pe.mask.ln1.b", "pe.mask.down2.w",
                                            "pe.mask.down2.b", "pe.mask.ln2.w",   "pe.mask.ln2.b", "pe.mask.proj.w", "pe.mask.proj.b"};
        int present = 0;
        const char* absent = nullptr;
        for (const char* n : names) {
            if (file.has(n)) ++present;
            else absent = n;
        }
        if (present != 0 && absent)
            throw Exception("'" + file.path() + "': the mask branch pe.mask.* is all or nothing: " + std::to_string(present) +
                            " of its 10 tensors are there, '" + absent + "' is not");
        has_mask_branch_ = present != 0;
        if (has_mask_branch_) {
            ld.f32("pe.mask.down1.w", {4, 1, 2, 2}, mask_w1_);
            ld.f32("pe.mask.down1.b", {4}, mask_b1_);
            ld.norm("pe.mask.ln1", 4, mask_ln1_);
            ld.f32("pe.mask.down2.w", {16, 4, 2, 2}, mask_w2_);
            ld.f32("pe.mask.down2.b", {16}, mask_b2_);
            ld.norm("pe.mask.ln2", 16, mask_ln2_);
            ld.f32("pe.mask.proj.w", {256, 16}, mask_proj_w_);
            ld.f32("pe.mask.proj.b", {256}, mask_proj_b_);
        }
    }
    {
        HostTensor const& g = file.get("pe.gauss", {2, 128});
        std::vector<float> pe((size_t)kTokens * 256);
        for (int y = 0; y < 64; ++y)
            for (int x = 0; x < 64; ++x) {
                const float cx = 2.0f * ((x + 0.5f) / 64.0f) - 1.0f, cy = 2.0f * ((y + 0.5f) / 64.0f) - 1.0f;
                float* row = pe.data() + ((size_t)y * 64 + x) * 256;
                for (int kf = 0; kf < 128; ++kf) {
                    const float v = 6.283185307179586f * (cx * g.data[kf] + cy * g.data[128 + kf]);
                    row[kf] = std::sin(v);
                    row[128 + kf] = std::cos(v);
                }
            }
        ld.f16_host(pe.data(), pe.size(), pe_h, "the dense positional encoding");
    }
    auto pos_term = [&](LinearH const& l, int with_pos, DeviceBuffer<float>& dst) {
        dst.reserve((size_t)kTokens * l.out);
        HIP_CHECK(hipMemsetAsync(dst.get(), 0, (size_t)kTokens * l.out * sizeof(float), stream_));
        k::GemmArgs g;
        g.A = pe_h.get(); g.lda = 256; g.W = l.w.get(); g.ldw = 256;
        g.out_f32 = dst.get(); g.ldc32 = l.out; g.M = kTokens; g.N = with_pos; g.K = 256;
        SamModel::plan_inputs(g,  false,  false);
        k::gemm(g, stream_);
    };
    ld.f32("dec.iou_token", {256}, iou_token_);
    ld.f32("dec.mask_tokens", {4, 256}, mask_tokens_);
    for (int i = 0; i < 2; ++i) {
        DecoderLayer& L = dec_[i];
        const std::string p = "dec.L" + std::to_string(i);
        ld.attention(p + ".self", 256, 256, L.self_attn);
        ld.norm(p + ".ln1", 256, L.ln1);
        ld.norm(p + ".ln2", 256, L.ln2);
        ld.norm(p + ".ln3", 256, L.ln3);
        ld.norm(p + ".ln4", 256, L.ln4);
        ld.linear_f(p + ".t2i.q", 128, 256, L.t2i_q);
        ld.linear_f(p + ".t2i.o", 256, 128, L.t2i_o);
        ld.transposed_f(p + ".t2i.o", 256, 128, L.t2i_o_t);
        ld.fused_h({p + ".t2i.k", p + ".i2t.q", p + ".t2i.v"}, 128, 256, L.img_kqv);
        pos_term(L.img_kqv, 256, L.pos_kqv);
        ld.linear_f(p + ".mlp.fc1", 2048, 256, L.mlp1);
        ld.linear_f(p + ".mlp.fc2", 256, 2048, L.mlp2);
        ld.linear_f(p + ".i2t.k", 128, 256, L.i2t_k);
        ld.linear_f(p + ".i2t.v", 128, 256, L.i2t_v);
        ld.linear_h(p + ".i2t.o", 256, 128, true, L.i2t_o);
    }
    ld.linear_f("dec.final.q", 128, 256, final_q_);
    ld.linear_f("dec.final.o", 256, 128, final_o_);
    ld.transposed_f("dec.final.o", 256, 128, final_o_t_);
    ld.fused_h({"dec.final.k", "dec.final.v"}, 128, 256, final_kv_);
    pos_term(final_kv_, 128, final_pos_kv_);
    ld.norm("dec.ln_final", 256, ln_final_);
    ld.conv_transpose_h("dec.up1", 256, 64, up1_);
    ld.norm("dec.up_ln", 64, up_ln_);
    ld.conv_transpose_h("dec.up2", 64, 32, up2_);
    for (int m = 0; m < 5; ++m) {
        const std::string p = m < 4 ? "dec.hyper" + std::to_string(m) : std::string("dec.iou");
        const int last = m < 4 ? 32 : 4;
        ld.linear_f(p + ".0", 256, 256, heads_[m][0]);
        ld.linear_f(p + ".1", 256, 256, heads_[m][1]);
        ld.linear_f(p + ".2", last, 256, heads_[m][2]);
    }
    {
        static const char* const names[] = {
            "dec.hq.token", "dec.hq.mlp.0.w", "dec.hq.mlp.0.b", "dec.hq.mlp.1.w", "dec.hq.mlp.1.b", "dec.hq.mlp.2.w", "dec.hq.mlp.2.b",
            "dec.hq.vit.conv1.w", "dec.hq.vit.conv1.b", "dec.hq.vit.ln.w", "dec.hq.vit.ln.b", "dec.hq.vit.conv2.w", "dec.hq.vit.conv2.b",
            "dec.hq.emb.conv1.w", "dec.hq.emb.conv1.b", "dec.hq.emb.ln.w", "dec.hq.emb.ln.b", "dec.hq.emb.conv2.w", "dec.hq.emb.conv2.b",
            "dec.hq.mask.conv1.w", "dec.hq.mask.conv1.b", "dec.hq.mask.ln.w", "dec.hq.mask.ln.b", "dec.hq.mask.conv2.w", "dec.hq.mask.conv2.b"};
        int present = 0;
        const char* absent = nullptr;
        for (const char* n : names) {
            if (file.has(n)) ++present;
            else absent = n;
        }
        if (present != 0 && absent)
            throw Exception("'" + file.path() + "': the SAM-HQ group dec.hq.* is all or nothing: " + std::to_string(present) +
                            " of its 25 tensors are there, '" + absent + "' is not");
        has_hq_ = present != 0;
        if (has_hq_ && geom_.global_attn_indexes.empty())
            throw Exception("'" + file.path() + "': the SAM-HQ group needs an encoder with a global-attention block (its early feature)");
        if (has_hq_) {
            ld.f32("dec.hq.token", {256}, hq_token_);
            ld.linear_f("dec.hq.mlp.0", 256, 256, hq_mlp_[0]);
            ld.linear_f("dec.hq.mlp.1", 256, 256, hq_mlp_[1]);
            ld.linear_f("dec.hq.mlp.2", 32, 256, hq_mlp_[2]);
            ld.conv_transpose_h("dec.hq.vit.conv1", D, 256, hq_vit1_);
            ld.norm("dec.hq.vit.ln", 256, hq_vit_ln_);
            ld.conv_transpose_h("dec.hq.vit.conv2", 256, 32, hq_vit2_);
            ld.conv_transpose_h("dec.hq.emb.conv1", 256, 64, hq_emb1_);
            ld.norm("dec.hq.emb.ln", 64, hq_emb_ln_);
            ld.conv_transpose_h("dec.hq.emb.conv2", 64, 32, hq_emb2_);
            auto conv3x3 = [&](std::string const& prefix, int co_n, int ci_n, DeviceBuffer<half_t>& w16, DeviceBuffer<float>& b) {
                HostTensor const& w = file.get(prefix + ".w", {co_n, ci_n, 3, 3});
                std::vector<float> g(w.numel());
                for (int co = 0; co < co_n; ++co)
                    for (int ci = 0; ci < ci_n; ++ci)
                        for (int t = 0; t < 9; ++t)
                            g[((size_t)t * co_n + co) * ci_n + ci] = w.data[((size_t)co * ci_n + ci) * 9 + t];
                ld.f16_host(g.data(), g.size(), w16, prefix + ".w");
                ld.f32(prefix + ".b", {co_n}, b);
            };
            conv3x3("dec.hq.mask.conv1", 64, 32, hq_conv1_w_, hq_conv1_b_);
            ld.norm("dec.hq.mask.ln", 64, hq_mask_ln_);
            conv3x3("dec.hq.mask.conv2", 32, 64, hq_conv2_w_, hq_conv2_b_);
        }
    }
    HIP_CHECK(hipStreamSynchronize(stream_));
    HIP_CHECK(hipStreamDestroy(stream_));
}

}
```

Baseline: 900.4 images/s.

## Fuse neck convolutions with their LayerNorm2d and implicit 3x3 im2col

```diff
diff --git a/__graft_entry__.py b/__graft_entry__.py
--- a/__graft_entry__.py
+++ b/__graft_entry__.py
@@ -22,6 +22,9 @@
     assert hooks.dlimg_init() is not None
     for name in api.ext.HOOK_EXPORTS:
         getattr(hooks, name)
+    neck = api.neck_hooks_library()
+    for name in api.NECK_HOOK_EXPORTS:
+        getattr(neck, name)
     from oracle import sam_oracle
     from oracle.build_ref import build_abi_consumer
     ref = build_abi_consumer()
diff --git a/dlimgedit_amd/api.py b/dlimgedit_amd/api.py
--- a/dlimgedit_amd/api.py
+++ b/dlimgedit_amd/api.py
@@ -131,6 +131,33 @@
             _hooks_lib.dlimg_init.restype = C.POINTER(_Api)
             _hooks_lib.dlimg_init.argtypes = []
     return _hooks_lib
+
+
+_neck_hooks_lib = None
+NECK_HOOKS_LIB_PATH = LIB_PATH.with_name("libdlimgedit_neck_test.so")
+NECK_HOOK_EXPORTS = ("dlimg_amd_test_neck_conv1x1_ln", "dlimg_amd_test_neck_conv3x3_ln")
+
+
+def neck_hooks_library() -> C.CDLL:
+    global _neck_hooks_lib
+    if _neck_hooks_lib is None:
+        if not NECK_HOOKS_LIB_PATH.exists():
+            raise Error(f"{NECK_HOOKS_LIB_PATH} not found: build it with `python -m dlimgedit_amd.build`")
+        lib = C.CDLL(str(NECK_HOOKS_LIB_PATH))
+        lib.dlimg_init.restype = C.POINTER(_Api)
+        lib.dlimg_init.argtypes = []
+        vp, ci, cf = C.c_void_p, C.c_int, C.c_float
+        lib.dlimg_amd_test_neck_conv1x1_ln.argtypes = [vp, ci, ci, vp, vp, vp, cf, vp, vp, vp, C.POINTER(ci)]
+        lib.dlimg_amd_test_neck_conv3x3_ln.argtypes = [vp, ci, vp, vp, vp, cf, vp, vp, vp, C.POINTER(ci)]
+        lib.dlimg_amd_test_neck_conv1x1_ln.restype = lib.dlimg_amd_test_neck_conv3x3_ln.restype = ci
+        _neck_hooks_lib = lib
+    return _neck_hooks_lib
+
+
+def _check_neck_hook(result: int) -> None:
+    if result != 0:
+        msg = neck_hooks_library().dlimg_init().contents.last_error()
+        raise Error(msg.decode("utf-8", "replace") if msg else "Unknown error")
 
 
 def _check_hook(result: int) -> None:
@@ -907,6 +934,67 @@
                                                  o32.ctypes.data, o16.ctypes.data))
         return o32, o16
 
+    NECK_GUARD = 256
+    NECK_GUARD_BYTE = 0xA5
+
+    @classmethod
+    def test_neck_conv_ln(cls, env: Environment, x, w, gamma, beta, eps: float, want_f16: bool = True, want_f32: bool = True,
+                          own_buffer=None):
+        x = np.ascontiguousarray(x, dtype=np.float16)
+        w = np.ascontiguousarray(w, dtype=np.float16)
+        gamma = np.ascontiguousarray(gamma, dtype=np.float32)
+        beta = np.ascontiguousarray(beta, dtype=np.float32)
+        conv3 = x.ndim == 4
+        B = x.shape[0] if conv3 else x.shape[0] // 4096
+        K = 2304 if conv3 else x.shape[1]
+        assert x.size == B * 4096 * (256 if conv3 else K) and w.shape == (256, K) and gamma.shape == beta.shape == (256,)
+        own = [False] * B if own_buffer is None else [bool(o) for o in own_buffer]
+        assert len(own) == B and (want_f32 or not any(own))
+        img_bytes, G = 4096 * 256 * 4, cls.NECK_GUARD
+        held = []
+
+        def dev(a=None, nbytes=0):
+            ptr = cls.device_alloc(env, a.nbytes if a is not None else nbytes)
+            held.append(ptr)
+            if a is not None:
+                cls.copy_to_device(env, ptr, a)
+            return ptr
+
+        try:
+            d_x, d_w, d_g, d_b = dev(x), dev(w), dev(gamma), dev(beta)
+            d_h = dev(nbytes=B * 4096 * 256 * 2) if want_f16 else None
+            d_ws = dev(nbytes=B * img_bytes) if want_f32 else None
+            ptrs = (C.c_void_p * B)()
+            fill = np.full(img_bytes + 2 * G, cls.NECK_GUARD_BYTE, np.uint8)
+            for i in range(B):
+                ptrs[i] = dev(fill) + G if own[i] else None
+            flag = C.c_int(-1)
+            h = neck_hooks_library()
+            if conv3:
+                rc = h.dlimg_amd_test_neck_conv3x3_ln(d_x, B, d_w, d_g, d_b, eps, d_h, ptrs if any(own) else None, d_ws, C.byref(flag))
+            else:
+                rc = h.dlimg_amd_test_neck_conv1x1_ln(d_x, B, K, d_w, d_g, d_b, eps, d_h, ptrs if any(own) else None, d_ws,
+                                                      C.byref(flag))
+            _check_neck_hook(rc)
+            out16 = out32 = None
+            guards = [None] * B
+            if want_f16:
+                out16 = np.empty((B * 4096, 256), np.float16)
+                cls.copy_to_host(env, out16, d_h)
+            if want_f32:
+                out32 = np.empty((B * 4096, 256), np.float32)
+                cls.copy_to_host(env, out32, d_ws)
+                for i in range(B):
+                    if own[i]:
+                        whole = np.empty(img_bytes + 2 * G, np.uint8)
+                        cls.copy_to_host(env, whole, ptrs[i] - G)
+                        guards[i] = (whole[:G].copy(), whole[-G:].copy())
+                        out32[i * 4096:(i + 1) * 4096] = whole[G:-G].view(np.float32).reshape(4096, 256)
+            return out16, out32, flag.value, guards
+        finally:
+            for ptr in held:
+                cls.device_free(env, ptr)
+
     @classmethod
     def test_attention(cls, is_global: bool, qkv, qkv_bias, rel_h, rel_w, batch: int, heads: int, hd: int):
         qkv = np.ascontiguousarray(qkv, dtype=np.float16)
diff --git a/dlimgedit_amd/build.py b/dlimgedit_amd/build.py
--- a/dlimgedit_amd/build.py
+++ b/dlimgedit_amd/build.py
@@ -15,11 +15,14 @@
 LIB = PKG / "lib" / "libdlimgedit.so"
 LIB_TEST = PKG / "lib" / "libdlimgedit_test.so"
 LIB_TUNING = PKG / "lib" / "libdlimgedit_tuning.so"
+LIB_NECK_TEST = PKG / "lib" / "libdlimgedit_neck_test.so"
 ARCH = "gfx950"
 SONAME = "libdlimgedit.so.1"
 EXPORTS_MAP = CSRC / "exports.map"
 EXPORTS_TEST_MAP = CSRC / "exports_test.map"
+EXPORTS_NECK_TEST_MAP = CSRC / "exports_neck_test.map"
 HOOK_SOURCES = ["test_hooks.cpp"]
+NECK_HOOK_SOURCES = ["neck_test_hooks.cpp"]
 
 SOURCES = [
     "kernels/gemm.hip",
@@ -152,6 +155,7 @@
     with ThreadPoolExecutor(workers) as ex:
         objs = list(ex.map(lambda s: _compile(s, force, hdr, tuning), SOURCES))
         hooks = list(ex.map(lambda s: _compile(s, force, hdr, tuning), HOOK_SOURCES))
+        neck_hooks = [] if tuning else list(ex.map(lambda s: _compile(s, force, hdr), NECK_HOOK_SOURCES))
     if tuning:
         if _stale(LIB_TUNING, objs + hooks, force):
             _link(LIB_TUNING, objs + hooks, EXPORTS_TEST_MAP)
@@ -165,11 +169,13 @@
         if _stale(LIB, objs, force):
             _link(LIB, objs, EXPORTS_MAP, SONAME)
         _link(LIB_TEST, objs + hooks, EXPORTS_TEST_MAP)
+    if _stale(LIB_NECK_TEST, objs + neck_hooks, force):
+        _link(LIB_NECK_TEST, objs + neck_hooks, EXPORTS_NECK_TEST_MAP)
     link = LIB.parent / SONAME
     if not link.is_symlink() and not link.exists():
         link.symlink_to(LIB.name)
     if verbose:
-        print(f"built {LIB} ({LIB.stat().st_size / 1e6:.1f} MB) and {LIB_TEST.name}")
+        print(f"built {LIB} ({LIB.stat().st_size / 1e6:.1f} MB), {LIB_TEST.name} and {LIB_NECK_TEST.name}")
     return LIB
 
 
diff --git a/dlimgedit_amd/csrc/kernels/gemm.hip b/dlimgedit_amd/csrc/kernels/gemm.hip
--- a/dlimgedit_amd/csrc/kernels/gemm.hip
+++ b/dlimgedit_amd/csrc/kernels/gemm.hip
@@ -5,6 +5,7 @@
 #include <hip/hip_ext.h>
 
 #include <mutex>
+#include <string>
 #include <cstdlib>
 #include <type_traits>
 
@@ -40,6 +41,8 @@
 #endif
 
 #include "gemm_f16_tile.inc"
+
+constexpr int EPI_LN2D = 3;
 
 typedef float float4v __attribute__((ext_vector_type(4)));
 
@@ -265,6 +268,11 @@
     static constexpr int TPR = 512 / BM;
     static constexpr int GP = BM * 8 > 1024 ? BM * 8 / 1024 : 1;
     static DLIMG_DEVICE void issue(const k::GemmArgs& a, int m0, int n0, float* colvec, float2_t* raw, int wave, int lane) {
+        if (EPI == EPI_LN2D) {
+            if (wave == 0) glds16(a.ln2d_w + lane * 4, colvec);
+            if (wave == 1) glds16(a.ln2d_b + lane * 4, colvec + BN);
+            return;
+        }
         if (wave == 0) {
             if (a.bias) glds16(a.bias + n0 + lane * 4, colvec);
             else *reinterpret_cast<float4_t*>(colvec + lane * 4) = float4_t{0.f, 0.f, 0.f, 0.f};
@@ -301,11 +309,85 @@
     }
 };
 
+template <int NI>
+DLIMG_DEVICE void pp_epilogue_ln2d(const k::GemmArgs& a, float4v (&acc)[NI][4], char* smem, const float* colvec,
+                                   float2_t* rowpart, int m0, int row_base, int wc, int wave, int lane) {
+    constexpr int BN = 256;
+    const int l15 = lane & 15, quad = lane >> 4;
+    const int rd_row = lane >> 3, rd_col = (lane & 7) * 8;
+    char* slab = smem + wave * 8192;
+    float4_t v[NI][2][2];
+#pragma unroll
+    for (int i = 0; i < NI; ++i) {
+        char* sl = slab + (i & 1) * 4096;
+#pragma unroll
+        for (int j = 0; j < 4; ++j)
+            *reinterpret_cast<float4_t*>(sl + l15 * 256 + (((j * 4 + quad) ^ (l15 & 7)) << 4)) =
+                float4_t{acc[i][j][0], acc[i][j][1], acc[i][j][2], acc[i][j][3]};
+        asm volatile("s_waitcnt lgkmcnt(0)" ::: "memory");
+#pragma unroll
+        for (int kk = 0; kk < 2; ++kk) {
+            const int r = kk * 8 + rd_row;
+            const int slot = (lane & 7) * 2;
+            const float4_t v0 = *reinterpret_cast<const float4_t*>(sl + r * 256 + ((slot ^ (r & 7)) << 4));
+            const float4_t v1 = *reinterpret_cast<const float4_t*>(sl + r * 256 + (((slot + 1) ^ (r & 7)) << 4));
+            float s1 = ((v0[0] + v0[1]) + (v0[2] + v0[3])) + ((v1[0] + v1[1]) + (v1[2] + v1[3]));
+            s1 = sum_over_8_lanes(s1);
+            const float4_t d0 = v0 - s1 * (1.0f / 64.0f), d1 = v1 - s1 * (1.0f / 64.0f);
+            float m2 = ((d0[0] * d0[0] + d0[1] * d0[1]) + (d0[2] * d0[2] + d0[3] * d0[3])) +
+                       ((d1[0] * d1[0] + d1[1] * d1[1]) + (d1[2] * d1[2] + d1[3] * d1[3]));
+            m2 = sum_over_8_lanes(m2);
+            if ((lane & 7) == 0) rowpart[(row_base + i * 16 + r) * 4 + wc] = float2_t{s1, m2};
+            v[i][kk][0] = v0;
+            v[i][kk][1] = v1;
+        }
+    }
+    __syncthreads();
+    const int col = wc * 64 + rd_col;
+    const float4_t g0 = *reinterpret_cast<const float4_t*>(colvec + col), g1 = *reinterpret_cast<const float4_t*>(colvec + col + 4);
+    const float4_t b0 = *reinterpret_cast<const float4_t*>(colvec + BN + col);
+    const float4_t b1 = *reinterpret_cast<const float4_t*>(colvec + BN + col + 4);
+    float* const out32 = a.out_img[m0 >> 12];
+#pragma unroll
+    for (int i = 0; i < NI; ++i)
+#pragma unroll
+        for (int kk = 0; kk < 2; ++kk) {
+            const int r = row_base + i * 16 + kk * 8 + rd_row;
+            float s1 = 0.f;
+#pragma unroll
+            for (int g = 0; g < 4; ++g) s1 += rowpart[r * 4 + g][0];
+            const float mean = s1 * (1.0f / (float)BN);
+            float m2 = 0.f;
+#pragma unroll
+            for (int g = 0; g < 4; ++g) {
+                const float dm = rowpart[r * 4 + g][0] * (1.0f / 64.0f) - mean;
+                m2 += rowpart[r * 4 + g][1] + 64.0f * dm * dm;
+            }
+            const float rstd = 1.0f / sqrtf(m2 * (1.0f / (float)BN) + a.ln_eps);
+            if (a.nonfinite && wc == 0 && (lane & 7) == 0 && !(fabsf(mean) < INFINITY && fabsf(rstd) < INFINITY)) *a.nonfinite = 1;
+            const float4_t y0 = (v[i][kk][0] - mean) * rstd * g0 + b0, y1 = (v[i][kk][1] - mean) * rstd * g1 + b1;
+            const size_t m = (size_t)(m0 + r);
+            if (out32) {
+                store16_result(out32 + (m & 4095) * BN + col, y0);
+                store16_result(out32 + (m & 4095) * BN + col + 4, y1);
+            }
+            if (a.out_h) {
+                const half8_t h = {(half_t)y0[0], (half_t)y0[1], (half_t)y0[2], (half_t)y0[3],
+                                   (half_t)y1[0], (half_t)y1[1], (half_t)y1[2], (half_t)y1[3]};
+                store16_result(a.out_h + m * a.ldc16 + col, h);
+            }
+        }
+}
+
 template <int NI, int ACT, int EPI, bool PRE = false>
 DLIMG_DEVICE void pp_epilogue(const k::GemmArgs& a, float4v (&acc)[NI][4], char* smem, const float* rowstat, const float* colvec,
                               float2_t* rowpart, int m0, int n0, int row_base, int wc, int wave, int lane,
                               float4_t (*pre)[4] = nullptr) {
     constexpr int BN = 256;
+    if constexpr (EPI == EPI_LN2D) {
+        pp_epilogue_ln2d<NI>(a, acc, smem, colvec, rowpart, m0, row_base, wc, wave, lane);
+        return;
+    }
     const int l15 = lane & 15, quad = lane >> 4;
     const int col_base = wc * 64 + quad * 4;
     float4_t bias4[4], csum4[4];
@@ -613,9 +695,10 @@
 constexpr int pp128_lds(int bm) { return pp128_operands(bm) + pp_aux_bytes(bm); }
 static_assert(pp128_lds(128) <= 160 * 1024 && pp128_lds(64) <= 160 * 1024, "gemm_pp128_kernel: LDS");
 
-template <int BM, int ACT, int EPI>
+template <int BM, int ACT, int EPI, bool CONV3 = false>
 __global__ __launch_bounds__(512, 2) void gemm_pp128_kernel(k::GemmArgs a) {
     static_assert(BM == 128 || BM == 64, "128 or 64 rows per tile");
+    static_assert((EPI != EPI_LN2D && !CONV3) || BM == 64, "the neck flavours exist for 64-row tiles");
     constexpr int BN = 256;
     constexpr int NI = BM / 32;
     constexpr int APIECES = BM / 64;
@@ -657,8 +740,25 @@
         src_a[q] = a.A + (size_t)(m0 + row) * a.lda + chunk * 8;
     }
     const size_t w_half = (size_t)128 * a.ldw;
+    unsigned tap_ok = 0;
+    const half_t* zero_src = nullptr;
+    if (CONV3) {
+        const int token = m0 + wave * 8 + (lane >> 3);
+        const int y = (token >> 6) & 63, x = token & 63;
+#pragma unroll
+        for (int tap = 0; tap < 9; ++tap)
+            if ((unsigned)(y + tap / 3 - 1) < 64u && (unsigned)(x + tap % 3 - 1) < 64u) tap_ok |= 1u << tap;
+        zero_src = a.zeros + (lane & 7) * 8;
+    }
     auto stage_a = [&](int t, int abuf) {
         char* dst = smem + abuf * pp128_a_bytes(BM) + wave * (APIECES * 1024);
+        if (CONV3) {
+            const int tap = t >> 2;
+            const int shift = ((tap / 3 - 1) * 64 + (tap % 3 - 1)) * 256 + (t & 3) * 64;
+            const int ok = -(int)((tap_ok >> tap) & 1u);
+            glds16((ok ? src_a[0] : zero_src) + (shift & ok), dst);
+            return;
+        }
 #pragma unroll
         for (int q = 0; q < APIECES; ++q) glds16(src_a[q] + (size_t)t * 64, dst + q * 1024);
     };
@@ -851,6 +951,17 @@
     launch_tile<TILE>(kernels, attr_once, a, s, t);
 }
 
+template <bool CONV3>
+void launch_neck(const k::GemmArgs& a, hipStream_t s, Timing t) {
+    static k::LdsOptIn attr_once;
+    const GemmKernel kernel = gemm_pp128_kernel<64, k::ACT_NONE, EPI_LN2D, CONV3>;
+    attr_once.ensure((const void*)kernel, pp128_lds(64), "neck convolution: the device refuses the LDS size of its tile");
+    if (t.start || t.stop)
+        hipExtLaunchKernelGGL(kernel, dim3(a.M / 64), dim3(512), pp128_lds(64), s, t.start, t.stop, 0, a);
+    else
+        hipLaunchKernelGGL(kernel, dim3(a.M / 64), dim3(512), pp128_lds(64), s, a);
+}
+
 template <int TILE, int BM>
 void launch_pp128(const k::GemmArgs& a, hipStream_t s, Timing t) {
     static_assert(tile_row_is<TILE>(BM, 256, 512, pp128_lds(BM), k::TileFamily::pingpong, kPPStatGroups), "gemm_pp128_kernel: the kernel and its row of k::kGemmTiles disagree");
@@ -882,5 +993,47 @@
     kLaunchers[tile](a, s, Timing{start, stop});
 }
 
-}
-}
+namespace {
+template <bool CONV3>
+void neck_launches(GemmArgs g, int B, const NeckOutputs& out, hipStream_t s, hipEvent_t start, hipEvent_t stop) {
+    const half_t* in = g.A;
+    for (int base = 0; base < B; base += 8) {
+        const int n = B - base < 8 ? B - base : 8;
+        g.A = in + (size_t)base * 4096 * g.lda;
+        g.M = n * 4096;
+        g.out_h = out.out_h ? out.out_h + (size_t)base * 4096 * 256 : nullptr;
+        for (int i = 0; i < 8; ++i) g.out_img[i] = (out.out_f32 && i < n) ? out.out_f32[base + i] : nullptr;
+        launch_neck<CONV3>(g, s, Timing{base == 0 ? start : nullptr, base + 8 >= B ? stop : nullptr});
+    }
+}
+GemmArgs neck_args(const char* who, const half_t* in, int B, int K, const half_t* w, const float* gamma, const float* beta,
+                   float eps, const NeckOutputs& out) {
+    if (B <= 0 || K < 64 || K % 64) throw_error((std::string(who) + ": needs at least one image and K a multiple of 64").c_str());
+    if (!in || !w || !gamma || !beta) throw_error((std::string(who) + ": null operand").c_str());
+    uintptr_t bits = (uintptr_t)in | (uintptr_t)w | (uintptr_t)gamma | (uintptr_t)beta | (uintptr_t)out.out_h;
+    for (int i = 0; out.out_f32 && i < B; ++i) bits |= (uintptr_t)out.out_f32[i];
+    if (bits & 15) throw_error((std::string(who) + ": operands and results must be 16-byte aligned").c_str());
+    GemmArgs g;
+    g.A = in; g.W = w; g.ldw = K; g.N = 256; g.K = K; g.ldc16 = 256;
+    g.ln2d_w = gamma; g.ln2d_b = beta; g.ln_eps = eps; g.nonfinite = out.nonfinite;
+    return g;
+}
+}
+
+void neck_conv1x1_ln(const half_t* in, int B, int K, const half_t* w, const float* gamma, const float* beta, float eps,
+                     const NeckOutputs& out, hipStream_t s, hipEvent_t start, hipEvent_t stop) {
+    GemmArgs g = neck_args("neck_conv1x1_ln", in, B, K, w, gamma, beta, eps, out);
+    g.lda = K;
+    neck_launches<false>(g, B, out, s, start, stop);
+}
+
+void neck_conv3x3_ln(const half_t* in, int B, const half_t* w, const half_t* zeros, const float* gamma, const float* beta,
+                     float eps, const NeckOutputs& out, hipStream_t s, hipEvent_t start, hipEvent_t stop) {
+    GemmArgs g = neck_args("neck_conv3x3_ln", in, B, 9 * 256, w, gamma, beta, eps, out);
+    if (!zeros || ((uintptr_t)zeros & 15)) throw_error("neck_conv3x3_ln: needs a 16-byte aligned line of zeros");
+    g.lda = 256; g.zeros = zeros;
+    neck_launches<true>(g, B, out, s, start, stop);
+}
+
+}
+}
diff --git a/dlimgedit_amd/csrc/kernels/kernels.hpp b/dlimgedit_amd/csrc/kernels/kernels.hpp
--- a/dlimgedit_amd/csrc/kernels/kernels.hpp
+++ b/dlimgedit_amd/csrc/kernels/kernels.hpp
@@ -53,12 +53,27 @@
     int tile = -1;
     int unit_rows = 0;
     unsigned long long* stamps = nullptr;
+    const float* ln2d_w = nullptr;
+    const float* ln2d_b = nullptr;
+    float* out_img[8] = {};
+    int* nonfinite = nullptr;
+    const half_t* zeros = nullptr;
 };
 const char* gemm_check(const GemmArgs&);
 bool gemm_tile_fits(const GemmArgs&, int tile);
 int gemm_pick_tile(const GemmArgs&);
 int gemm_choose_tile(GemmArgs&);
 void gemm(const GemmArgs&, hipStream_t, hipEvent_t start = nullptr, hipEvent_t stop = nullptr);
+
+struct NeckOutputs {
+    half_t* out_h = nullptr;
+    float* const* out_f32 = nullptr;
+    int* nonfinite = nullptr;
+};
+void neck_conv1x1_ln(const half_t* in, int B, int K, const half_t* w, const float* gamma, const float* beta, float eps,
+                     const NeckOutputs& out, hipStream_t, hipEvent_t start = nullptr, hipEvent_t stop = nullptr);
+void neck_conv3x3_ln(const half_t* in, int B, const half_t* w, const half_t* zeros, const float* gamma, const float* beta,
+                     float eps, const NeckOutputs& out, hipStream_t, hipEvent_t start = nullptr, hipEvent_t stop = nullptr);
 
 void layernorm(const float* x, const float* w, const float* b, float eps, int rows, int D, int act,
                float* out_f32, half_t* out_h, hipStream_t, int* nonfinite = nullptr);
diff --git a/dlimgedit_amd/csrc/neck_test_hooks.cpp b/dlimgedit_amd/csrc/neck_test_hooks.cpp
--- /dev/null
+++ b/dlimgedit_amd/csrc/neck_test_hooks.cpp
@@ -0,0 +1,62 @@
+#include "ext_common.hpp"
+
+#include <vector>
+
+namespace dlimg {
+namespace {
+
+using namespace extapi;
+
+template <typename F>
+void run_neck_hook(int B, float* const* out_f32, float* workspace, int* out_flag, F&& launch) {
+    require_gpu();
+    DLIMG_ASSERT(B > 0 && out_flag != nullptr);
+    std::vector<float*> dst(B, nullptr);
+    bool any = false;
+    for (int i = 0; i < B; ++i) {
+        dst[i] = (out_f32 && out_f32[i]) ? out_f32[i] : (workspace ? workspace + (size_t)i * kTokens * kEmbedDim : nullptr);
+        any = any || dst[i];
+    }
+    int* flag = nullptr;
+    HIP_CHECK(hipHostMalloc(reinterpret_cast<void**>(&flag), sizeof(int), hipHostMallocDefault));
+    *flag = 0;
+    struct FreeFlag { int* p; ~FreeFlag() { (void)hipHostFree(p); } } free_flag{flag};
+    k::NeckOutputs out;
+    out.out_f32 = any ? dst.data() : nullptr;
+    out.nonfinite = flag;
+    launch(out);
+    HIP_CHECK(hipDeviceSynchronize());
+    *out_flag = *const_cast<volatile int*>(flag);
+}
+
+}
+}
+
+using namespace dlimg;
+
+extern "C" {
+
+DLIMG_API int dlimg_amd_test_neck_conv1x1_ln(void const* in, int B, int K, void const* w, float const* gamma, float const* beta,
+                                             float eps, void* out_f16, float* const* out_f32, float* workspace, int* out_flag) {
+    return guarded([&] {
+        run_neck_hook(B, out_f32, workspace, out_flag, [&](k::NeckOutputs& out) {
+            out.out_h = static_cast<half_t*>(out_f16);
+            k::neck_conv1x1_ln(static_cast<half_t const*>(in), B, K, static_cast<half_t const*>(w), gamma, beta, eps, out, nullptr);
+        });
+    });
+}
+
+DLIMG_API int dlimg_amd_test_neck_conv3x3_ln(void const* in, int B, void const* w, float const* gamma, float const* beta, float eps,
+                                             void* out_f16, float* const* out_f32, float* workspace, int* out_flag) {
+    return guarded([&] {
+        DeviceBuffer<half_t> zeros(64);
+        HIP_CHECK(hipMemset(zeros.get(), 0, 64 * sizeof(half_t)));
+        run_neck_hook(B, out_f32, workspace, out_flag, [&](k::NeckOutputs& out) {
+            out.out_h = static_cast<half_t*>(out_f16);
+            k::neck_conv3x3_ln(static_cast<half_t const*>(in), B, static_cast<half_t const*>(w), zeros.get(), gamma, beta, eps, out,
+                               nullptr);
+        });
+    });
+}
+
+}
diff --git a/dlimgedit_amd/csrc/sam_model.cpp b/dlimgedit_amd/csrc/sam_model.cpp
--- a/dlimgedit_amd/csrc/sam_model.cpp
+++ b/dlimgedit_amd/csrc/sam_model.cpp
@@ -67,6 +67,16 @@
     const Stage flavour = a.stats_out ? ST_GEMM_STATS : a.ln_stats ? (a.act == k::ACT_GELU ? ST_GEMM_NORM_GELU : ST_GEMM_NORM) : ST_GEMM_OTHER;
     const StageClock::Pending p = clock_.event_pair(ST_GEMM, 2.0 * a.M * a.N * a.K, flavour, shape);
     k::gemm(a, stream_, p.a, p.b);
+    clock_.add(p);
+}
+
+template <typename F> void SamModel::neck_launch(double flops, F&& launch) {
+    if (!clock_.profiling()) {
+        launch(nullptr, nullptr);
+        return;
+    }
+    const StageClock::Pending p = clock_.event_pair(ST_GEMM, flops, ST_GEMM_OTHER);
+    launch(p.a, p.b);
     clock_.add(p);
 }
 
@@ -111,7 +121,7 @@
     qkv_.reserve(M * 3 * D);
     att_.reserve(M * std::max<size_t>(D, kEmbedDim));
     hid_.reserve(M * wide);
-    neck_f32_.reserve(M * kEmbedDim);
+    if (!W.fused_ln_) neck_f32_.reserve(M * kEmbedDim);
     emb_.reserve(M * kEmbedDim);
     if (W.has_hq()) {
         hq_a_.reserve(M * 4 * kEmbedDim);
@@ -429,27 +439,6 @@
         ++layer_index;
     }
 
-    if (!fused) {
-        clock_.timed(ST_ENC_OTHER, (double)M * D * 6, [&] {
-            k::add_cast(x_.get(), nullptr, 0, (size_t)M * D, nullptr, xn_.get(), stream_);
-        });
-    }
-    g = k::GemmArgs{};
-    g.A = xn_.get(); g.lda = D; g.W = W.neck1_.w.get(); g.ldw = D;
-    g.out_f32 = neck_f32_.get(); g.ldc32 = kEmbedDim; g.M = M; g.N = kEmbedDim; g.K = D;
-    gemm(g);
-    clock_.timed(ST_LAYERNORM, (double)M * kEmbedDim * 6, [&] {
-        k::layernorm(neck_f32_.get(), W.neck_ln1_.w.get(), W.neck_ln1_.b.get(), kLnEps, M, kEmbedDim, k::ACT_NONE, nullptr,
-                     att_.get(), stream_);
-    });
-    clock_.timed(ST_ENC_OTHER, (double)M * kEmbedDim * 2 * 10, [&] {
-        k::im2col3x3(att_.get(), batch, kEmbedDim, hid_.get(), stream_);
-    });
-    g = k::GemmArgs{};
-    g.A = hid_.get(); g.lda = 9 * kEmbedDim; g.W = W.neck2_.w.get(); g.ldw = 9 * kEmbedDim;
-    g.out_f32 = neck_f32_.get(); g.ldc32 = kEmbedDim; g.M = M; g.N = kEmbedDim; g.K = 9 * kEmbedDim;
-    gemm(g);
-    float* direct = (emb_dst && batch == 1 && emb_dst[0]) ? emb_dst[0] : nullptr;
     if (!pass_flags_) {
         HIP_CHECK(hipHostMalloc(reinterpret_cast<void**>(&pass_flags_), kPassFlags * sizeof(int), hipHostMallocDefault));
         std::memset(pass_flags_, 0, kPassFlags * sizeof(int));
@@ -461,10 +450,46 @@
     }
     pass_flag_ = pass_flags_ + flag_slot;
     *pass_flag_ = 0;
-    clock_.timed(ST_LAYERNORM, (double)M * kEmbedDim * 8, [&] {
-        k::layernorm(neck_f32_.get(), W.neck_ln2_.w.get(), W.neck_ln2_.b.get(), kLnEps, M, kEmbedDim, k::ACT_NONE,
-                     direct ? direct : emb_.get(), W.has_hq() ? emb_h_.get() : nullptr, stream_, pass_flag_);
-    });
+    float* direct = (emb_dst && batch == 1 && emb_dst[0]) ? emb_dst[0] : nullptr;
+    if (fused) {
+        std::vector<float*> dst(batch);
+        for (int i = 0; i < batch; ++i)
+            dst[i] = (emb_dst && emb_dst[i]) ? emb_dst[i] : emb_.get() + (size_t)i * kEmbeddingFloats;
+        k::NeckOutputs map, emb;
+        map.out_h = att_.get();
+        emb.out_f32 = dst.data(); emb.out_h = W.has_hq() ? emb_h_.get() : nullptr; emb.nonfinite = pass_flag_;
+        neck_launch(2.0 * M * kEmbedDim * D, [&](hipEvent_t a, hipEvent_t b) {
+            k::neck_conv1x1_ln(xn_.get(), batch, D, W.neck1_.w.get(), W.neck_ln1_.w.get(), W.neck_ln1_.b.get(), kLnEps, map,
+                               stream_, a, b);
+        });
+        neck_launch(2.0 * M * kEmbedDim * 9 * kEmbedDim, [&](hipEvent_t a, hipEvent_t b) {
+            k::neck_conv3x3_ln(att_.get(), batch, W.neck2_.w.get(), W.zero_line_.get(), W.neck_ln2_.w.get(), W.neck_ln2_.b.get(),
+                               kLnEps, emb, stream_, a, b);
+        });
+    } else {
+        clock_.timed(ST_ENC_OTHER, (double)M * D * 6, [&] {
+            k::add_cast(x_.get(), nullptr, 0, (size_t)M * D, nullptr, xn_.get(), stream_);
+        });
+        g = k::GemmArgs{};
+        g.A = xn_.get(); g.lda = D; g.W = W.neck1_.w.get(); g.ldw = D;
+        g.out_f32 = neck_f32_.get(); g.ldc32 = kEmbedDim; g.M = M; g.N = kEmbedDim; g.K = D;
+        gemm(g);
+        clock_.timed(ST_LAYERNORM, (double)M * kEmbedDim * 6, [&] {
+            k::layernorm(neck_f32_.get(), W.neck_ln1_.w.get(), W.neck_ln1_.b.get(), kLnEps, M, kEmbedDim, k::ACT_NONE, nullptr,
+                         att_.get(), stream_);
+        });
+        clock_.timed(ST_ENC_OTHER, (double)M * kEmbedDim * 2 * 10, [&] {
+            k::im2col3x3(att_.get(), batch, kEmbedDim, hid_.get(), stream_);
+        });
+        g = k::GemmArgs{};
+        g.A = hid_.get(); g.lda = 9 * kEmbedDim; g.W = W.neck2_.w.get(); g.ldw = 9 * kEmbedDim;
+        g.out_f32 = neck_f32_.get(); g.ldc32 = kEmbedDim; g.M = M; g.N = kEmbedDim; g.K = 9 * kEmbedDim;
+        gemm(g);
+        clock_.timed(ST_LAYERNORM, (double)M * kEmbedDim * 8, [&] {
+            k::layernorm(neck_f32_.get(), W.neck_ln2_.w.get(), W.neck_ln2_.b.get(), kLnEps, M, kEmbedDim, k::ACT_NONE,
+                         direct ? direct : emb_.get(), W.has_hq() ? emb_h_.get() : nullptr, stream_, pass_flag_);
+        });
+    }
     if (W.has_hq()) {
         hq_gemm_pair(emb_h_.get(), kEmbedDim, W.hq_emb1_, W.hq_emb_ln_, W.hq_emb2_, M, hq_embf_.get());
         clock_.timed(ST_ENC_OTHER, (double)batch * kHqFeatureFloats * 12, [&] {
@@ -475,7 +500,7 @@
             }
         });
     }
-    if (emb_dst && !direct) {
+    if (emb_dst && !direct && !fused) {
         const size_t n = (size_t)kTokens * kEmbedDim;
         for (int i = 0; i < batch; ++i)
             if (emb_dst[i])
diff --git a/dlimgedit_amd/csrc/sam_model.hpp b/dlimgedit_amd/csrc/sam_model.hpp
--- a/dlimgedit_amd/csrc/sam_model.hpp
+++ b/dlimgedit_amd/csrc/sam_model.hpp
@@ -75,6 +75,7 @@
     std::vector<EncoderLayer> layers_;
     LinearH neck1_, neck2_;
     NormW neck_ln1_, neck_ln2_;
+    DeviceBuffer<half_t> zero_line_;
     DeviceBuffer<float> pe_gauss_, pe_point_, pe_not_a_point_, pe_no_mask_;
     k::PromptEncoderWeights prompt_encoder() const {
         return k::PromptEncoderWeights{pe_gauss_.get(), pe_point_.get(), pe_not_a_point_.get(), iou_token_.get(), mask_tokens_.get()};
@@ -197,6 +198,7 @@
                       k::MaskSource const* mask_input);
     void hq_gemm_pair(half_t const* a, int K, LinearH const& conv1, NormW const& ln, LinearH const& conv2, int M, float* out);
     void gemm(k::GemmArgs const& a, Stage shape = ST_COUNT);
+    template <typename F> void neck_launch(double flops, F&& launch);
 
     int device_ = 0;
     bool shared_gpu_ = false;
@@ -220,7 +222,8 @@
     bool caller_copy_pending_ = false;
     uint8_t* stage_rows(uint8_t const* pixels, size_t row_bytes, int rows, int stride, hipEvent_t* copied);
     DeviceBuffer<half_t> patches_, xn_, xlo_, qkv_, att_, hid_;
-    DeviceBuffer<float> x_, xstat_, neck_f32_, emb_;
+    DeviceBuffer<float> x_, xstat_, emb_;
+    DeviceBuffer<float> neck_f32_;
     DeviceBuffer<float> hq_a_, hq_vit_, hq_embf_, hq_feat_;
     DeviceBuffer<half_t> hq_h_, emb_h_;
     bool split_stream_ = false;
diff --git a/dlimgedit_amd/csrc/sam_weights.cpp b/dlimgedit_amd/csrc/sam_weights.cpp
--- a/dlimgedit_amd/csrc/sam_weights.cpp
+++ b/dlimgedit_amd/csrc/sam_weights.cpp
@@ -205,6 +205,8 @@
         neck2_.in = 9 * kEmbedDim;
     }
     ld.norm("enc.neck.ln2", kEmbedDim, neck_ln2_);
+    zero_line_.reserve(64);
+    HIP_CHECK(hipMemsetAsync(zero_line_.get(), 0, 64 * sizeof(half_t), stream_));
 
     DeviceBuffer<half_t> pe_h;
     ld.f32("pe.gauss", {2, 128}, pe_gauss_);
```

Result: faster. 909.6 images/s, median of 6 (+1.0%).
